# wuwuz/Pacmann

Hardware: AMD Instinct MI355X
Metric: private queries/sec + PIR-scan HBM GB/s, SIFT1M d=128 at 1/2/4/8 GPUs (higher is better)
Workload: dtype u64

## Files before the change

pacmann_amd/csrc/pm_ctx.cpp:

```cpp
#include "pm_host.h"

static thread_local std::string g_err;
namespace pmh {
int fail(int code, const std::string& msg) { g_err = msg; return code; }
}

extern "C" const char* pm_last_error(void) { return g_err.c_str(); }

static constexpr AesTables kAes{};
extern "C" int pm_expand_key(const uint8_t key[16], uint32_t rk[44]) {
  uint8_t w[176];
  memcpy(w, key, 16);
  uint8_t rcon = 1;
  for (int i = 16; i < 176; i += 4) {
    uint8_t t[4] = {w[i - 4], w[i - 3], w[i - 2], w[i - 1]};
    if (i % 16 == 0) {
      uint8_t u = t[0];
      t[0] = kAes.sbox[t[1]] ^ rcon; t[1] = kAes.sbox[t[2]]; t[2] = kAes.sbox[t[3]]; t[3] = kAes.sbox[u];
      rcon = AesTables::gmul(rcon, 2);
    }
    for (int k = 0; k < 4; ++k) w[i + k] = w[i - 16 + k] ^ t[k];
  }
  memcpy(rk, w, 176);
  return 0;
}


extern "C" int pm_ctx_create(int device, pm_ctx** out) {
  if (!out) return fail(PM_EINVAL, "out is NULL");
  int n = 0;
  HIPCHK(hipGetDeviceCount(&n));
  if (device < 0 || device >= n) return fail(PM_EINVAL, "no such HIP device " + std::to_string(device));
  HIPCHK(hipSetDevice(device));
  (void)hipSetDeviceFlags(hipDeviceScheduleSpin);
  (void)hipGetLastError();
  pm_ctx* c = new pm_ctx();
  c->device = device;
  const char* dbg = getenv("PM_DEBUG_SYNC");
  c->debug_sync = dbg && dbg[0] == '1';
  const char* nf = getenv("PM_NO_FUSE");
  c->no_fuse = nf && nf[0] == '1';
  const char* ns = getenv("PM_NO_SPLIT");
  c->no_split = ns && ns[0] == '1';
  const char* ls = getenv("PM_LOG_STEPS");
  c->log_steps = ls && ls[0] == '1';
  const char* dc = getenv("PM_DEBUG_CACHE");
  c->debug_cache = dc && dc[0] == '1';
  const char* vr = getenv("PM_VERIFY_ROWS");
  c->verify_rows = vr && vr[0] == '1';
  if (const char* rc = getenv("PM_ROWS_CHECK")) c->rows_check = atoi(rc);
  c->hash_mult.resize(pmk::step_max_e());
  for (size_t w = 0; w < c->hash_mult.size(); ++w) c->hash_mult[w] = row_hash_mult(w);
  if (const char* pw = getenv("PM_PUBLISH_WAIT")) c->publish_wait = pw[0] != '0';
  if (c->publish_wait) {
    for (auto& e : c->done_ring)
      if (hipEventCreateWithFlags(&e, hipEventDisableTiming | hipEventReleaseToSystem) != hipSuccess) {
        delete c;
        return fail(PM_EHIP, "hipEventCreateWithFlags(step completion) failed");
      }
    c->done_ev = c->done_ring[0];
  }
  if (const char* rs = getenv("PM_REPL_SIDE")) c->repl_side = rs[0] != '0';
  const char* ng = getenv("PM_NO_GUESS");
  c->no_guess = ng && ng[0] == '1';
  const char* sr = getenv("PM_STEP_SPEC");
  c->step_spec = sr && sr[0] == '1';
  hipError_t e = hipStreamCreateWithFlags(&c->stream, hipStreamNonBlocking);
  if (e != hipSuccess) { delete c; return fail(PM_EHIP, hipGetErrorString(e)); }
  *out = c;
  return 0;
}
extern "C" void pm_ctx_destroy(pm_ctx* c) { if (c) { (void)hipSetDevice(c->device); delete c; } }
extern "C" int pm_ctx_sync(pm_ctx* c) { HIPCHK(hipStreamSynchronize(c->stream)); HIPCHK(hipGetLastError()); return 0; }
extern "C" int pm_ctx_mem_info(pm_ctx* c, uint64_t* free_b, uint64_t* total_b) {
  if (!c) return fail(PM_EINVAL, "ctx is NULL");
  HIPCHK(hipSetDevice(c->device));
  size_t f = 0, t = 0;
  HIPCHK(hipMemGetInfo(&f, &t));
  if (free_b) *free_b = f;
  if (total_b) *total_b = t;
  return 0;
}
static std::mutex g_tl_mu;
static hipEvent_t g_tl_base = nullptr;
extern "C" int pm_timing_enable(pm_ctx* c, int on) {
  c->timing = on;
  if (on >= 2) {
    std::lock_guard<std::mutex> lk(g_tl_mu);
    if (!g_tl_base) {
      HIPCHK(hipEventCreate(&g_tl_base));
      HIPCHK(hipEventRecord(g_tl_base, c->stream));
    }
  }
  return 0;
}
extern "C" int pm_timing_timeline(pm_ctx* c, const char* path) {
  if (!c || !path) return fail(PM_EINVAL, "NULL argument");
  HIPCHK(hipStreamSynchronize(c->stream));
  std::lock_guard<std::mutex> lk(g_tl_mu);
  if (!g_tl_base) return fail(PM_EINVAL, "no timeline (kernel timing level 2 never enabled)");
  FILE* f = fopen(path, "a");
  if (!f) return fail(PM_EINVAL, std::string("cannot open ") + path);
  for (auto& t : c->launches) {
    float a = 0, b = 0;
    if (hipEventElapsedTime(&a, g_tl_base, t.a) != hipSuccess || hipEventElapsedTime(&b, g_tl_base, t.b) != hipSuccess)
      continue;
    fprintf(f, "%s,%.3f,%.3f,%p\n", t.name.c_str(), a * 1e3, b * 1e3, (void*)c);
  }
  fclose(f);
  return 0;
}
namespace pmh {
std::atomic<int> g_verify_records{0};
std::atomic<int> g_device_loop{-1};
std::atomic<int> g_rccl_timeout_s{-1};
std::atomic<int> g_fault_drl_query{-1};
}
extern "C" int pm_set_option(const char* name, int value) {
  if (!name) return fail(PM_EINVAL, "NULL argument");
  if (!strcmp(name, "verify_records")) { g_verify_records.store(value < 0 ? 0 : value); return 0; }
  if (!strcmp(name, "rccl_timeout_s")) { g_rccl_timeout_s.store(value); return 0; }
  if (!strcmp(name, "device_loop")) { g_device_loop.store(value < 0 ? -1 : value); return 0; }
  if (!strcmp(name, "fault_drl_query")) { g_fault_drl_query.store(value); return 0; }
  if (!strcmp(name, "stream_upload_only")) { g_stream_upload_only.store(value > 0 ? 1 : 0); return 0; }
  if (!strcmp(name, "aes_bs")) { pmk::set_aes_bs(value); return 0; }
  if (!strcmp(name, "fold_rot")) {
    if (value < -1 || value > 1) return fail(PM_EINVAL, "fold_rot takes 1, 0 or -1");
    pmk::set_fold_rot(value);
    return 0;
  }
  if (!strcmp(name, "fold_pack")) {
    if (value < -1 || value > 1) return fail(PM_EINVAL, "fold_pack takes 1, 0 or -1");
    pmk::set_fold_pack(value);
    return 0;
  }
  if (!strcmp(name, "answer_pack")) {
    if (value < -1 || value > 1) return fail(PM_EINVAL, "answer_pack takes 1, 0 or -1");
    pmk::set_answer_pack(value);
    return 0;
  }
  if (!strcmp(name, "step_help") && value != -2 && (value < 0 || value > 3))
    return fail(PM_EINVAL, "step_help takes 0..3 or -2");
  if (!strcmp(name, "step_help_spoil") && value != -2 && (value < 0 || value > 7))
    return fail(PM_EINVAL, "step_help_spoil takes a mask 0..7 or -2");
  if (pmk::set_option(name, value)) return fail(PM_EINVAL, std::string("unknown option ") + name);
  return 0;
}
extern "C" int pm_step_plan(const pm_step_shape* in, pm_step_forms* out) {
  if (!in || !out) return fail(PM_EINVAL, "NULL argument");
  if (in->kind > (uint32_t)pmk::STEP_DEVICE || in->nsub == 0 || in->np == 0) return fail(PM_EINVAL, "bad step shape");
  pmk::StepShape s{};
  s.np = in->np; s.nsub = in->nsub; s.np_live = in->np_live; s.max_per_part = in->max_per_part;
  s.maxPH = in->maxPH; s.maxSS = in->maxSS; s.E = in->E; s.ph8 = in->ph8 != 0;
  s.of_caller((int)in->kind, true);
  s.unfused = in->no_fuse != 0; s.no_split = in->no_split != 0; s.no_guess = in->no_guess != 0;
  const pmk::StepPlan p = pmk::step_plan(s, pmk::step_opts());
  static_assert(sizeof out->counter / sizeof out->counter[0] == pmk::STAGE_COUNT, "one slot per launch of a plan");
  *out = pm_step_forms{};
  for (int i = 0; i < pmk::STAGE_COUNT; ++i) {
    const pmk::StepLaunch& l = p.at[i];
    if (l.form < 0) continue;
    out->counter[i] = kHostTimerName[pm_ctx::step_counter(i, l.form)];
    out->grid_x[i] = l.gx; out->grid_y[i] = l.gy; out->block[i] = l.block;
  }
  out->nhelp = p.nhelp; out->nsplit = p.nsplit; out->qw = p.qw; out->np_live = p.np_live; out->cblk = p.cblk;
  out->no_guess = p.no_guess; out->qset = p.qset; out->args_valid = s.args_valid;
  return 0;
}
extern "C" int pm_fold_image_map(uint32_t cs, uint32_t ss, uint32_t E, uint32_t dim, int packed, uint64_t x0,
                                 uint64_t n, uint64_t* row, uint32_t* word, uint8_t* is_packed, uint64_t* nitems,
                                 uint32_t* npk_out) {
  if ((n && (!row || !word || !is_packed)) || !nitems || !npk_out) return fail(PM_EINVAL, "NULL argument");
  if ((cs != 512 && cs != 1024) || ss == 0 || ss % 4 || E < 4 || E % 2) return fail(PM_EINVAL, "not a fold image shape");
  const uint32_t npk = packed ? pmk::fold_pack_shape(E, dim) : 0;
  if (packed && (!npk || cs != 512)) return fail(PM_EINVAL, "these entries have no packed fold image");
  *nitems = pmk::fold_image_words(ss, E, cs, npk) / 2;
  *npk_out = npk;
  if (x0 > *nitems || n > *nitems - x0) return fail(PM_EINVAL, "items past the image");
  pmk::fold_image_map(cs, ss, npk, x0, n, row, word, is_packed);
  return 0;
}
extern "C" int pm_timing_reset(pm_ctx* c) {
  HIPCHK(hipStreamSynchronize(c->stream));
  for (auto& t : c->launches) { c->pool.push_back(t.a); c->pool.push_back(t.b); }
  c->launches.clear();
  for (int i = 0; i < HT_COUNT; ++i) { c->host_n[i] = 0; c->host_ms[i] = 0; }
  return 0;
}
extern "C" int pm_timing_get(pm_ctx* c, const char* name, uint64_t* launches, double* total_ms,
                             double* bytes) {
  HIPCHK(hipStreamSynchronize(c->stream));
  uint64_t n = 0; double ms = 0, by = 0;
  if (strncmp(name, "host_", 5) == 0) {
    for (int i = 0; i < HT_COUNT; ++i)
      if (strcmp(name, kHostTimerName[i]) == 0) { n = c->host_n[i]; ms = c->host_ms[i]; }
    if (launches) *launches = n;
    if (total_ms) *total_ms = ms;
    if (bytes) *bytes = 0;
    return 0;
  }
  for (auto& t : c->launches) {
    if (t.name != name) continue;
    float x = 0;
    HIPCHK(hipEventElapsedTime(&x, t.a, t.b));
    ++n; ms += x; by += t.bytes;
  }
  if (launches) *launches = n;
  if (total_ms) *total_ms = ms;
  if (bytes) *bytes = by;
  return 0;
}

#if defined(PM_STEP_STAMPS) || defined(PM_MR_STAMPS) || defined(PM_ANSWER_STAMPS)
namespace pmh {
int dump_stamps(hipStream_t st, const char* path, const void* hdr, size_t hdr_bytes, const DevBuf& buf, uint64_t count) {
  HIPCHK(hipStreamSynchronize(st));
  std::vector<uint64_t> t(count);
  HIPCHK(hipMemcpy(t.data(), buf.p, count * 8, hipMemcpyDeviceToHost));
  static std::mutex mu;
  std::lock_guard<std::mutex> lk(mu);
  if (FILE* f = fopen(path, "ab")) {
    fwrite(hdr, 1, hdr_bytes, f);
    fwrite(t.data(), 8, count, f);
    fclose(f);
  }
  return 0;
}
}
#endif

extern "C" int pm_prf_batch(pm_ctx* c, const uint32_t rk[44], const uint64_t* tags, const uint64_t* xs,
                            uint64_t n, uint64_t* out) {
  if (n == 0) return 0;
  DevBuf drk, dt, dx, dout;
  CHK(drk.reserve(176)); CHK(dt.reserve(n * 8)); CHK(dx.reserve(n * 8)); CHK(dout.reserve(n * 8));
  hipStream_t st = c->stream;
  HIPCHK(hipMemcpyAsync(drk.p, rk, 176, hipMemcpyHostToDevice, st));
  HIPCHK(hipMemcpyAsync(dt.p, tags, n * 8, hipMemcpyHostToDevice, st));
  HIPCHK(hipMemcpyAsync(dx.p, xs, n * 8, hipMemcpyHostToDevice, st));
  c->timed("prf", (double)n, [&] { pmk::prf_batch(st, drk.as<uint32_t>(), dt.as<uint64_t>(), dx.as<uint64_t>(), n, dout.as<uint64_t>()); });
  HIPCHK(hipGetLastError());
  HIPCHK(hipMemcpyAsync(out, dout.p, n * 8, hipMemcpyDeviceToHost, st));
  HIPCHK(hipStreamSynchronize(st));
  return 0;
}
extern "C" int pm_l2_batch(pm_ctx* c, const float* q, const float* rows, uint64_t nrows, uint64_t dim,
                           float* out) {
  if (nrows == 0) return 0;
  if (dim == 0) return fail(PM_EINVAL, "dim must be > 0");
  DevBuf dq, dr, dout;
  CHK(dq.reserve(dim * 4)); CHK(dr.reserve(nrows * dim * 4)); CHK(dout.reserve(nrows * 4));
  hipStream_t st = c->stream;
  HIPCHK(hipMemcpyAsync(dq.p, q, dim * 4, hipMemcpyHostToDevice, st));
  HIPCHK(hipMemcpyAsync(dr.p, rows, nrows * dim * 4, hipMemcpyHostToDevice, st));
  c->timed("l2_rows", (double)nrows * dim * 4, [&] {
    pmk::l2_rows(st, dr.as<float>(), dim, nrows, nullptr, dq.as<float>(), (uint32_t)dim, dout.as<float>());
  });
  HIPCHK(hipGetLastError());
  HIPCHK(hipMemcpyAsync(out, dout.p, nrows * 4, hipMemcpyDeviceToHost, st));
  HIPCHK(hipStreamSynchronize(st));
  return 0;
}
extern "C" int pm_ip_batch(pm_ctx* c, const uint32_t* q, const uint32_t* rows, uint64_t nrows, uint64_t dim,
                           uint32_t* per_row, uint32_t* sum) {
  if (dim == 0) return fail(PM_EINVAL, "dim must be > 0");
  DevBuf dq, dr, dpr, ds;
  CHK(dq.reserve(dim * 4)); CHK(dr.reserve(std::max<uint64_t>(1, nrows * dim * 4)));
  CHK(dpr.reserve(std::max<uint64_t>(4, nrows * 4))); CHK(ds.reserve(4));
  hipStream_t st = c->stream;
  HIPCHK(hipMemcpyAsync(dq.p, q, dim * 4, hipMemcpyHostToDevice, st));
  if (nrows) HIPCHK(hipMemcpyAsync(dr.p, rows, nrows * dim * 4, hipMemcpyHostToDevice, st));
  HIPCHK(hipMemsetAsync(ds.p, 0, 4, st));
  c->timed("ip_scan", (double)nrows * dim * 4, [&] {
    pmk::ip_rows(st, dr.as<uint32_t>(), nrows, dq.as<uint32_t>(), (uint32_t)dim, per_row ? dpr.as<uint32_t>() : nullptr,
                 ds.as<uint32_t>());
  });
  HIPCHK(hipGetLastError());
  if (per_row && nrows) HIPCHK(hipMemcpyAsync(per_row, dpr.p, nrows * 4, hipMemcpyDeviceToHost, st));
  uint32_t s = 0;
  HIPCHK(hipMemcpyAsync(&s, ds.p, 4, hipMemcpyDeviceToHost, st));
  HIPCHK(hipStreamSynchronize(st));
  if (sum) *sum = s;
  return 0;
}
extern "C" int pm_ip_bench(pm_ctx* c, uint64_t N, uint64_t D, uint32_t* sum, double* scan_ms) {
  return pm_ip_bench_shard(c, N, D, 0, N, sum, scan_ms);
}
extern "C" int pm_ip_bench_shard(pm_ctx* c, uint64_t Ntot, uint64_t D, uint64_t r0, uint64_t N, uint32_t* sum,
                                 double* scan_ms) {
  if (!c) return fail(PM_EINVAL, "NULL context");
  if (D == 0 || D % 4 || D > 4096) return fail(PM_EINVAL, "D must be a multiple of 4 and <= 4096");
  if (r0 > Ntot || N > Ntot - r0) return fail(PM_EINVAL, "shard rows past the fill's N");
  if (N == 0) {
    if (sum) *sum = 0;
    if (scan_ms) *scan_ms = 0.0;
    return 0;
  }
  DevBuf dv, dq, ds;
  CHK(dv.reserve(N * D * 4)); CHK(dq.reserve(D * 4)); CHK(ds.reserve(4));
  std::vector<uint32_t> q(D);
  for (uint64_t j = 0; j < D; ++j) q[j] = (uint32_t)j;
  hipStream_t st = c->stream;
  HIPCHK(hipMemcpyAsync(dq.p, q.data(), D * 4, hipMemcpyHostToDevice, st));
  HIPCHK(hipMemsetAsync(ds.p, 0, 4, st));
  pmk::ip_fill(st, dv.as<uint32_t>(), N, (uint32_t)D, r0);
  hipEvent_t a, b;
  HIPCHK(hipEventCreate(&a)); HIPCHK(hipEventCreate(&b));
  HIPCHK(hipEventRecord(a, st));
  c->timed("ip_scan", (double)N * D * 4, [&] { pmk::ip_rows(st, dv.as<uint32_t>(), N, dq.as<uint32_t>(), (uint32_t)D, nullptr, ds.as<uint32_t>()); });
  HIPCHK(hipEventRecord(b, st));
  HIPCHK(hipGetLastError());
  uint32_t s = 0;
  HIPCHK(hipMemcpyAsync(&s, ds.p, 4, hipMemcpyDeviceToHost, st));
  HIPCHK(hipStreamSynchronize(st));
  float ms = 0;
  HIPCHK(hipEventElapsedTime(&ms, a, b));
  (void)hipEventDestroy(a); (void)hipEventDestroy(b);
  if (sum) *sum = s;
  if (scan_ms) *scan_ms = ms;
  return 0;
}
```

pacmann_amd/csrc/pm_engine.cpp:

```cpp
#include "pm_engine.h"

static void derive_key(uint64_t seed, uint64_t part, uint64_t epoch, uint8_t key[16]) {
  uint64_t r1 = hash4(seed, DOM_KEY, part, epoch, 0), r2 = hash4(seed, DOM_KEY, part, epoch, 1);
  memcpy(key, &r1, 8);
  memcpy(key + 8, &r2, 8);
}

static void part_params(PartHost& ph, uint64_t N, uint64_t F) {
  uint64_t target = (uint64_t)(2 * std::sqrt((double)N));
  uint64_t cs = 1;
  while (cs < target) cs *= 2;
  uint64_t ss = (uint64_t)std::ceil((double)N / (double)cs);
  ss = (ss + 3) / 4 * 4;
  const uint64_t thr = 8;
  uint64_t maxq = (uint64_t)(std::sqrt((double)N) * std::log((double)N));
  uint64_t k = (uint64_t)std::ceil(std::log(2.0) * (double)(F + 1));
  uint64_t phn = (k * cs + thr - 1) / thr * thr;
  uint64_t qpc = 3 * (uint64_t)((double)maxq / (double)ss);
  qpc = (qpc + thr - 1) / thr * thr;
  ph.d.N = N;
  ph.d.CS = (uint32_t)cs;
  uint32_t lg = 0; while ((1ull << lg) < cs) ++lg;
  ph.d.log2CS = lg;
  ph.d.SS = (uint32_t)ss;
  ph.d.PH = (uint32_t)phn;
  ph.d.Qpc = (uint32_t)qpc;
  ph.d.H = (uint32_t)(phn + ss * qpc);
  ph.maxq64 = maxq;
  ph.d.MaxQ = (uint32_t)std::min<uint64_t>(maxq, 0xffffffffu);
}

static double part_storage(const PartHost& p, uint64_t Ebytes) {
  double s = 0;
  s = s + (double)p.d.PH * 8;
  s = s + (double)p.d.PH * (double)Ebytes;
  s = s + (double)p.d.PH * 8;
  double tb = (double)p.d.SS * (double)p.d.Qpc;
  s = s + tb * 8;
  s = s + tb * (double)Ebytes;
  s = s + tb * 8;
  s = s + tb * (double)Ebytes;
  return s;
}
static double part_comm(const PartHost& p, uint64_t E) { return (double)((uint64_t)p.d.SS * 4 + E * 8); }

namespace pmh {
int engine_create(pm_ctx* ctx, Engine* g, uint64_t N, uint64_t Ebytes, uint64_t B,
                         const uint64_t* rawDB, uint64_t F, uint64_t seed, bool batch,
                         uint32_t shard, uint32_t nshards, const Engine* server,
                         const DbGen* gen, uint32_t coord_words, bool remote) {
  if (nshards == 0 || shard >= nshards) return fail(PM_EINVAL, "shard must be < nshards");
  if (!ctx) return fail(PM_EINVAL, "ctx is NULL");
  if (!rawDB && N && !server && !gen && !remote) return fail(PM_EINVAL, "rawDB is NULL");
  if (gen && gen->kind == 1 && (uint64_t)(gen->dim + gen->m) * 4 != Ebytes)
    return fail(PM_EINVAL, "graph entry size must be 4 * (dim + m)");
  if (server && server->ctx->device != ctx->device) return fail(PM_EINVAL, "a client shares the server DB of its own device only");
  if (N == 0) return fail(PM_EINVAL, "DBSize must be > 0");
  if (Ebytes < 8) return fail(PM_EINVAL, "DBEntryByteNum must be >= 8");
  HIPCHK(hipSetDevice(ctx->device));
  g->ctx = ctx; g->is_batch = batch;
  g->N = N; g->Ebytes = Ebytes; g->E = Ebytes / 8; g->F = F; g->seed = seed;
  g->remote = remote;
  if (batch) {
    g->B = B;
    g->P = B / 2;
    if (g->P == 0) return fail(PM_EINVAL, "BatchSize must be >= 2");
    g->PS = (N + g->P - 1) / g->P;
    if (g->PS > 1 && g->PS < (1ull << 32)) g->ps_magic = ~0ull / g->PS + 1;
  } else {
    g->P = 1; g->PS = N;
  }
  g->parts.resize(g->P);
  if (g->E > pmk::step_max_e()) return fail(PM_EINVAL, "DBEntrySize above the step kernel's LDS limit");
  g->shard = shard; g->nshards = nshards;
  uint64_t off_tag = 0, off_pp = 0, off_par = 0, off_ridx = 0, off_rval = 0, off_hist = 0, off_ar = 0,
           off_tab = 0, off_tabT = 0, off_cur = 0, off_db = 0;
  for (uint64_t i = 0; i < g->P; ++i) {
    PartHost& ph = g->parts[i];
    uint64_t start = i * g->PS, end = std::min((i + 1) * g->PS, N);
    if (end <= start) return fail(PM_EINVAL, "empty partition (DBSize too small for BatchSize)");
    part_params(ph, end - start, F);
    ph.owned = i % nshards == shard;
    if (!ph.owned) {
      ph.d.seed = seed; ph.d.idx = i;
      continue;
    }
    g->owned_list.push_back((uint32_t)i);
    if (ph.d.CS > 32768) return fail(PM_EINVAL, "ChunkSize > 32768 unsupported (16-bit prep offsets)");
    if (ph.d.SS > pmk::step_max_ss()) return fail(PM_EINVAL, "SetSize above the step kernel's LDS limit");
    if ((uint64_t)ph.d.H >= (1ull << 29)) return fail(PM_EINVAL, "tag space >= 2^29 (util.go:161)");
    ph.d.row0 = off_db; off_db += end - start;
    ph.d.seed = seed; ph.d.idx = i;
    g->maxH = std::max(g->maxH, ph.d.H);
    g->maxCS = std::max(g->maxCS, ph.d.CS);
    g->minCS = std::min(g->minCS, ph.d.CS);
    g->maxPH = std::max(g->maxPH, ph.d.PH);
    g->ph8 = g->ph8 && ph.d.PH % 8 == 0;
    g->maxSS = std::max(g->maxSS, ph.d.SS);
    g->maxRepl = std::max(g->maxRepl, ph.d.SS * ph.d.Qpc);
    ph.d.tag = (uint32_t*)(uintptr_t)off_tag; off_tag += ph.d.H;
    ph.d.pp = (uint32_t*)(uintptr_t)off_pp; off_pp += ph.d.PH;
    ph.d.parity = (uint64_t*)(uintptr_t)off_par; off_par += (uint64_t)ph.d.H * g->E;
    ph.d.ridx = (uint32_t*)(uintptr_t)off_ridx; off_ridx += (uint64_t)ph.d.SS * ph.d.Qpc;
    ph.d.rval = (uint64_t*)(uintptr_t)off_rval; off_rval += (uint64_t)ph.d.SS * ph.d.Qpc * g->E;
    ph.d.hist = (uint32_t*)(uintptr_t)off_hist; off_hist += ph.d.SS;
    ph.d.arena = (uint64_t*)(uintptr_t)off_ar; off_ar += (uint64_t)ph.d.MaxQ * g->E;
    ph.d.tab = (uint16_t*)(uintptr_t)off_tab; off_tab += (uint64_t)ph.d.H * ph.d.SS;
    ph.d.curk = cur_k(ph.d.PH, ph.d.SS);
    ph.d.cur = (uint16_t*)(uintptr_t)off_cur; off_cur += cur_words(ph.d.PH, ph.d.SS, ph.d.curk);
    ph.d.tabT = (uint16_t*)(uintptr_t)off_tabT; off_tabT += tabT_words(ph.d.H, ph.d.SS);
    ph.cache.reserve(ph.d.MaxQ);
  }
  CHK(g->zero16.reserve(64));
  HIPCHK(hipMemset(g->zero16.p, 0, 64));
  if (server) g->db = server->db;
  else if (!remote) CHK(g->db->reserve(std::max<uint64_t>(8, off_db * g->E * 8)));
  for (uint32_t i : server || remote ? std::vector<uint32_t>{} : g->owned_list) {
    const uint64_t start = (uint64_t)i * g->PS, rows = g->parts[i].d.N;
    uint64_t* dst = g->db->as<uint64_t>() + g->parts[i].d.row0 * g->E;
    if (gen && gen->kind == 0)
      pmk::db_synth(ctx->stream, dst, start, rows, (uint32_t)g->E, gen->seed);
    else if (gen)
      pmk::graph_synth(ctx->stream, dst, start, rows, N, gen->dim, gen->m, gen->seed);
    else
      HIPCHK(hipMemcpy(dst, rawDB + start * g->E, rows * g->E * 8, hipMemcpyHostToDevice));
  }
  if (gen) {
    HIPCHK(hipGetLastError());
    HIPCHK(hipStreamSynchronize(ctx->stream));
  }
  uint64_t off_img = 0;
  const bool fold_img = !remote && !g->owned_list.empty() && pmk::fold_image_ok(g->minCS, g->maxCS, (uint32_t)g->E);
  const uint32_t want_npk = !server && fold_img ? pmk::fold_pack_slices(g->minCS, g->maxCS, (uint32_t)g->E, coord_words) : 0;
  const uint32_t want_apk = !server && !remote && !g->owned_list.empty() ? pmk::answer_pack_segs((uint32_t)g->E, coord_words) : 0;
  bool low_zero = false;
  if (want_npk || want_apk) {
    DevBuf flag;
    CHK(flag.reserve(64));
    low_zero = pmk::coord_low_zero(ctx->stream, g->db->as<uint64_t>(), off_db, (uint32_t)g->E, coord_words, flag.as<uint32_t>());
    HIPCHK(hipGetLastError());
  }
  if (fold_img) {
    if (server) g->img_npk = server->img_npk;
    else if (low_zero) g->img_npk = want_npk;
    for (uint32_t i : g->owned_list) {
      PmPart& d = g->parts[i].d;
      d.img = (const uint64_t*)(uintptr_t)off_img;
      off_img += pmk::fold_image_words(d.SS, (uint32_t)g->E, (uint32_t)g->maxCS, g->img_npk);
    }
    size_t free_b = 0, total_b = 0;
    if (!server && hipMemGetInfo(&free_b, &total_b) == hipSuccess && off_img * 8 > free_b / 4) {
      for (uint32_t i : g->owned_list) g->parts[i].d.img = nullptr;
      off_img = 0;
    } else if (server && !server->img->p) {
      for (uint32_t i : g->owned_list) g->parts[i].d.img = nullptr;
      off_img = 0;
    }
    if (!off_img) g->img_npk = 0;
  }
  if (off_img) {
    if (server) {
      g->img = server->img;
    } else {
      CHK(g->img->reserve(off_img * 8));
      for (uint32_t i : g->owned_list) {
        const PmPart& d = g->parts[i].d;
        pmk::fold_image(ctx->stream, g->img->as<uint64_t>() + (uintptr_t)d.img, g->db->as<uint64_t>() + d.row0 * g->E,
                        d.N, d.SS, (uint32_t)g->E, (uint32_t)g->maxCS, g->img_npk);
      }
      HIPCHK(hipGetLastError());
      HIPCHK(hipStreamSynchronize(ctx->stream));
    }
  }
  if (server) {
    g->apk = server->apk; g->apk_nseg = server->apk_nseg; g->apk_cseg = server->apk_cseg;
  } else if (want_apk && low_zero) {
    const uint64_t bytes = off_db * want_apk * 16;
    size_t free_b = 0, total_b = 0;
    if (hipMemGetInfo(&free_b, &total_b) != hipSuccess || bytes <= free_b / 4) {
      CHK(g->apk->reserve(bytes));
      pmk::answer_pack_image(ctx->stream, g->apk->as<uint64_t>(), g->db->as<uint64_t>(), off_db, (uint32_t)g->E, coord_words);
      HIPCHK(hipGetLastError());
      HIPCHK(hipStreamSynchronize(ctx->stream));
      g->apk_nseg = want_apk; g->apk_cseg = coord_words / 8;
    }
  }
  CHK(g->tag.reserve(off_tag * 4));
  CHK(g->pp.reserve(off_pp * 4));
  CHK(g->parity.reserve(off_par * 8));
  CHK(g->ridx.reserve(off_ridx * 4));
  CHK(g->rval.reserve(off_rval * 8));
  CHK(g->hist.reserve(off_hist * 4));
  CHK(g->fqn.reserve(g->P * 4));
  CHK(g->arena.reserve(std::max<uint64_t>(8, off_ar * 8)));
  const bool need_tab = !remote && pmk::fold_needs_tab(g->minCS, g->maxCS, (uint32_t)g->E, off_img != 0);
  if (need_tab) CHK(g->tab.reserve(off_tab * 2));
  CHK(g->tabT.reserve(off_tabT * 2));
  CHK(g->cur.reserve(std::max<uint64_t>(2, off_cur * 2)));
  CHK(g->done.reserve(4 * (3 + 16 * 4096)));
  {
    const uint32_t init[3] = {1u << 31, 0, 0};
    HIPCHK(hipMemcpy(g->done.p, init, sizeof init, hipMemcpyHostToDevice));
  }
  {
    g->gran_words = (g->maxPH + 63) / 64;
    const size_t n = (size_t)kArgSubs * (8 + 64 + 2 * g->gran_words + 8) * 8;
    CHK(g->gran.reserve(n));
    HIPCHK(hipMemset(g->gran.p, 0, n));
    CHK(g->err_h.reserve(64));
    memset(g->err_h.p, 0, 64);
  }
  CHK(g->parts_d.reserve(g->P * sizeof(PmPart)));
  CHK(g->owned_d.reserve(std::max<size_t>(1, g->owned_list.size()) * sizeof(PmPart)));
  CHK(g->parts_stage.reserve((g->P + g->owned_list.size()) * sizeof(PmPart)));
  for (uint64_t i = 0; i < g->P; ++i) {
    PmPart& d = g->parts[i].d;
    if (!g->parts[i].owned) continue;
    d.tag = g->tag.as<uint32_t>() + (uintptr_t)d.tag;
    d.pp = g->pp.as<uint32_t>() + (uintptr_t)d.pp;
    d.parity = g->parity.as<uint64_t>() + (uintptr_t)d.parity;
    d.ridx = g->ridx.as<uint32_t>() + (uintptr_t)d.ridx;
    d.rval = g->rval.as<uint64_t>() + (uintptr_t)d.rval;
    d.hist = g->hist.as<uint32_t>() + (uintptr_t)d.hist;
    d.fqn = g->fqn.as<uint32_t>() + i;
    d.arena = g->arena.as<uint64_t>() + (uintptr_t)d.arena;
    d.tabT = g->tabT.as<uint16_t>() + (uintptr_t)d.tabT;
    d.tab = need_tab ? g->tab.as<uint16_t>() + (uintptr_t)d.tab : nullptr;
    d.cur = g->cur.as<uint16_t>() + (uintptr_t)d.cur;
    d.img = off_img ? g->img->as<uint64_t>() + (uintptr_t)d.img : nullptr;
  }
  HIPCHK(hipMemsetAsync(g->fqn.p, 0, g->P * 4, ctx->stream));
  HIPCHK(hipMemsetAsync(g->hist.p, 0, off_hist * 4, ctx->stream));
  HIPCHK(hipStreamSynchronize(ctx->stream));
  return 0;
}
}

static int upload_parts(Engine* g) {
  std::vector<PmPart> v(g->P), w;
  for (uint64_t i = 0; i < g->P; ++i) v[i] = g->parts[i].d;
  for (uint32_t i : g->owned_list) w.push_back(g->parts[i].d);
  HIPCHK(hipMemcpyAsync(g->parts_d.p, v.data(), g->P * sizeof(PmPart), hipMemcpyHostToDevice,
                        g->ctx->stream));
  if (!w.empty())
    HIPCHK(hipMemcpyAsync(g->owned_d.p, w.data(), w.size() * sizeof(PmPart), hipMemcpyHostToDevice,
                          g->ctx->stream));
  HIPCHK(hipStreamSynchronize(g->ctx->stream));
  return 0;
}

static int upload_parts_async(Engine* g, hipStream_t st) {
  if (g->ctx->stream != st && hipStreamQuery(g->ctx->stream) != hipSuccess) {
    if (!g->order_ev) HIPCHK(hipEventCreateWithFlags(&g->order_ev, hipEventDisableTiming));
    HIPCHK(hipEventRecord(g->order_ev, g->ctx->stream));
    HIPCHK(hipStreamWaitEvent(st, g->order_ev, 0));
  }
  const size_t no = g->owned_list.size();
  if (g->stage_ev) HIPCHK(hipEventSynchronize(g->stage_ev));
  else HIPCHK(hipEventCreateWithFlags(&g->stage_ev, hipEventDisableTiming));
  CHK(g->parts_stage.reserve((g->P + no) * sizeof(PmPart)));
  PmPart* h = g->parts_stage.as<PmPart>();
  for (uint64_t i = 0; i < g->P; ++i) h[i] = g->parts[i].d;
  for (size_t i = 0; i < no; ++i) h[g->P + i] = g->parts[g->owned_list[i]].d;
  HIPCHK(hipMemcpyAsync(g->parts_d.p, h, g->P * sizeof(PmPart), hipMemcpyHostToDevice, st));
  if (no) HIPCHK(hipMemcpyAsync(g->owned_d.p, h + g->P, no * sizeof(PmPart), hipMemcpyHostToDevice, st));
  HIPCHK(hipEventRecord(g->stage_ev, st));
  return 0;
}

namespace pmh {
int ensure_host_cache(Engine* g) {
  if (!g->cache_on_dev) return 0;
  const uint64_t cap = (uint64_t)g->dcache_cmask + 1;
  std::vector<uint64_t> t(g->P * cap);
  HIPCHK(hipSetDevice(g->ctx->device));
  HIPCHK(hipMemcpy(t.data(), g->dcache.p, t.size() * 8, hipMemcpyDeviceToHost));
  for (uint64_t p = 0; p < g->P; ++p) {
    FlatMap& c = g->parts[p].cache;
    c.clear();
    for (uint64_t i = 0; i < cap; ++i)
      if (const uint64_t e = t[p * cap + i]) c.put((uint32_t)e - 1u, (uint32_t)(e >> 32));
  }
  g->cache_on_dev = false;
  g->dcache_valid = false;
  return 0;
}

int engine_prep_host(Engine* g, uint64_t p0, uint64_t p1, std::vector<uint64_t>& todo,
                            hipStream_t st) {
  if (p1 - p0 > 1 && !(p0 == 0 && p1 == g->P)) return fail(PM_EINVAL, "engine_prep: unsupported range");
  const bool all = p0 == 0 && p1 == g->P;
  if (g->cache_on_dev && !all) CHK(ensure_host_cache(g));
  if (all) { g->cache_on_dev = false; g->dcache_valid = false; }
  todo.clear();
  for (uint64_t i = p0; i < p1; ++i)
    if (g->parts[i].owned) todo.push_back(i);
  if (todo.empty()) return 0;
  for (uint64_t i : todo) {
    PartHost& ph = g->parts[i];
    uint8_t key[16];
    derive_key(g->seed, i, ph.epoch_ctr, key);
    ph.d.epoch = ph.epoch_ctr++;
    pm_expand_key(key, ph.d.rk);
    ph.fqn = 0;
    ph.cache.clear();
    ph.shadow.clear();
  }
  CHK(st ? upload_parts_async(g, st) : upload_parts(g));
  g->prep_gen++;
  return 0;
}
int engine_prep_launch(pm_ctx* c, const Engine* g, const PmPart* dp, int np, const PmPart* host_parts,
                              uint32_t clients, bool sync) {
  hipStream_t st = c->stream;
  c->timed("prep_init", 0, [&] { pmk::prep_init(st, dp, np, g->maxH, g->maxRepl, (uint32_t)g->E, g->skipPrep); });
  double aes = 0, fold = 0, repl = 0;
  uint32_t minH = ~0u;
  for (int i = 0; i < np; ++i) {
    const PmPart& d = host_parts[i];
    minH = std::min(minH, d.H);
    aes += (double)d.H * d.SS;
    fold += ((double)d.PH + (double)(d.SS - 1) * d.Qpc) * d.SS * (double)g->E * 8;
    repl += (double)d.SS * d.Qpc * g->E * 8 * 2;
  }
  const bool side = !g->skipPrep && c->repl_side && !c->timing && !c->debug_sync;
  std::unique_lock<std::mutex> side_lk(c->side_mu, std::defer_lock);
  if (side) {
    side_lk.lock();
    if (!c->side) {
      HIPCHK(hipStreamCreateWithFlags(&c->side, hipStreamNonBlocking));
      for (auto& e : c->side_ev) HIPCHK(hipEventCreateWithFlags(&e, hipEventDisableTiming));
    }
    HIPCHK(hipEventRecord(c->side_ev[0], st));
    HIPCHK(hipStreamWaitEvent(c->side, c->side_ev[0], 0));
    pmk::prep_repl(c->side, dp, np, g->maxRepl, g->db->as<uint64_t>(), (uint32_t)g->E);
    HIPCHK(hipEventRecord(c->side_ev[1], c->side));
  }
  c->timed("prep_offsets", aes, [&] { pmk::prep_offsets(st, dp, np, g->maxH, g->maxSS); });
  if (g->skipPrep) {
    for (int i = 0; i < np; ++i) {
      const PmPart& d = host_parts[i];
      HIPCHK(hipMemsetAsync(d.parity, 0, (uint64_t)d.H * g->E * 8, st));
      HIPCHK(hipMemsetAsync(d.rval, 0, (uint64_t)d.SS * d.Qpc * g->E * 8, st));
    }
  } else {
    int kind = pmk::FOLD_GATHER;
    c->timed("prep_fold", fold, [&] { kind = pmk::prep_fold(st, dp, np, g->maxH, g->db->as<uint64_t>(), (uint32_t)g->E, g->minCS,
                                                      g->maxCS, g->zero16.as<uint64_t>(), clients, g->img->p != nullptr, minH,
                                                      g->img_npk); });
    if (kind == pmk::FOLD_ROT512 || kind == pmk::FOLD_ROT512P || kind == pmk::FOLD_ROT1024) {
      c->host_add(kind == pmk::FOLD_ROT512 ? HT_FOLD_ROT512 : kind == pmk::FOLD_ROT512P ? HT_FOLD_ROT512P : HT_FOLD_ROT1024, 0.0);
    } else {
      c->host_add(HT_FOLD_OTHER, 0.0);
      c->host_add(kind == pmk::FOLD_PIPE ? HT_FOLD_PIPE : kind == pmk::FOLD_BLK ? HT_FOLD_BLK : HT_FOLD_GATHER, 0.0);
    }
    if (side) HIPCHK(hipStreamWaitEvent(st, c->side_ev[1], 0));
    else c->timed("prep_repl", repl, [&] { pmk::prep_repl(st, dp, np, g->maxRepl, g->db->as<uint64_t>(), (uint32_t)g->E); });
  }
  HIPCHK(hipGetLastError());
  if (sync) HIPCHK(hipStreamSynchronize(st));
  return 0;
}
}
static int engine_prep(Engine* g, uint64_t p0, uint64_t p1) {
  std::vector<uint64_t> todo;
  CHK(engine_prep_host(g, p0, p1, todo));
  if (todo.empty()) return 0;
  const PmPart* dp = p1 - p0 == 1 ? g->parts_d.as<PmPart>() + p0 : g->owned_d.as<PmPart>();
  std::vector<PmPart> hp;
  for (uint64_t i : todo) hp.push_back(g->parts[i].d);
  return engine_prep_launch(g->ctx, g, dp, (int)todo.size(), hp.data());
}


namespace pmh {
int wait_done(pm_ctx* sc, uint64_t seq) {
  if (sc->done_seen.load(std::memory_order_acquire) >= seq) return 0;
  auto t0 = Clock::now();
  for (uint64_t spin = 0;; ++spin) {
    if (sc->done_seen.load(std::memory_order_acquire) >= seq) return 0;
    if (sc->done_mu.try_lock()) {
      std::lock_guard<std::mutex> lk(sc->done_mu, std::adopt_lock);
      if (sc->done_seen.load(std::memory_order_acquire) >= seq) return 0;
      const uint64_t rec = seq;
      if (sc->done_rec.load(std::memory_order_acquire) < seq)
        return fail(PM_EHIP, "step completion: waited for a step that was not recorded");
      for (uint64_t k = 0;; ++k) {
        const hipError_t e = hipEventQuery(sc->done_ring[seq % pm_ctx::kDoneRing]);
        if (e == hipSuccess) break;
        if (e != hipErrorNotReady) return fail(PM_EHIP, std::string("step completion: ") + hipGetErrorString(e));
        if ((k & 0xfff) == 0xfff && ms_since(t0) > 5000.0) {
          HIPCHK(hipStreamSynchronize(sc->stream));
          HIPCHK(hipGetLastError());
          break;
        }
      }
      uint64_t prev = sc->done_seen.load(std::memory_order_relaxed);
      while (prev < rec && !sc->done_seen.compare_exchange_weak(prev, rec, std::memory_order_release)) {}
      return 0;
    }
    if ((spin & 0xffff) == 0xffff && ms_since(t0) > 10000.0) return fail(PM_EHIP, "step completion wait timed out");
  }
}

int poll_done(pm_ctx* sc, uint64_t seq, bool* ready) {
  *ready = !(sc->publish_wait && sc->done_ev && seq) || sc->done_seen.load(std::memory_order_acquire) >= seq;
  if (*ready || !sc->done_mu.try_lock()) return 0;
  std::lock_guard<std::mutex> lk(sc->done_mu, std::adopt_lock);
  if (sc->done_seen.load(std::memory_order_acquire) >= seq) { *ready = true; return 0; }
  if (sc->done_rec.load(std::memory_order_acquire) < seq)
    return fail(PM_EHIP, "step completion: polled a step that was not recorded");
  const hipError_t e = hipEventQuery(sc->done_ring[seq % pm_ctx::kDoneRing]);
  if (e == hipErrorNotReady) return 0;
  if (e != hipSuccess) return fail(PM_EHIP, std::string("step completion: ") + hipGetErrorString(e));
  uint64_t prev = sc->done_seen.load(std::memory_order_relaxed);
  while (prev < seq && !sc->done_seen.compare_exchange_weak(prev, seq, std::memory_order_release)) {}
  *ready = true;
  return 0;
}

int wait_step(pm_ctx* c, const PmOutHdr* hdr, uint32_t nsub, uint32_t token, const char* rows,
                     size_t row_bytes, size_t pf_off, size_t pf_len, uint64_t seq, pm_ctx* sc) {
  if (!sc) sc = c;
  hipStream_t stream = sc->stream;
  const bool ordered = sc->publish_wait && sc->done_ev && seq;
  const size_t w0 = pf_off / 8, w1 = (pf_off + pf_len + 7) / 8;
  auto row_hash = [&](uint32_t s) {
    const volatile uint64_t* rw = (const volatile uint64_t*)(rows + s * row_bytes);
    uint64_t x = token * kCsumMix;
    for (size_t w = w0; w < w1; ++w) x += rw[w] * c->hash_mult[w];
    return x;
  };
  if (c->debug_sync) {
    HIPCHK(hipStreamSynchronize(stream));
  } else if (ordered && !c->timing) {
    for (uint32_t s = 0; s < nsub; ++s) {
      __builtin_prefetch(&hdr[s]);
      if (c->rows_check)
        for (size_t w = w0; w < w1; w += 8) __builtin_prefetch(rows + s * row_bytes + w * 8);
    }
    CHK(wait_done(sc, seq));
    std::atomic_thread_fence(std::memory_order_acquire);
  } else {
    const volatile uint32_t* tok = &hdr[0].token;
    const size_t stride = sizeof(PmOutHdr) / sizeof(uint32_t);
    for (uint32_t s = 0; s < nsub; ++s) {
      __builtin_prefetch(&hdr[s]);
      if (c->rows_check)
        for (size_t w = w0; w < w1; w += 8) __builtin_prefetch(rows + s * row_bytes + w * 8);
    }
    auto t0 = Clock::now();
    uint32_t s = 0;
    bool first_look = true;
    for (uint64_t spin = 0; s < nsub; ++spin) {
      if (tok[s * stride] == token) {
        if (c->timing && s == 0 && first_look) c->host_add(HT_WAIT_FIRST, ms_since(t0));
        std::atomic_thread_fence(std::memory_order_acquire);
        if (c->rows_check) {
          const bool match = row_hash(s) == *(const volatile uint64_t*)&hdr[s].csum;
          if (first_look) {
            c->host_add(HT_ROWS_SEEN, 0);
            if (!match) c->host_add(HT_ROWS_TORN, 0);
          }
          if (!match && !ordered) {
            first_look = false;
            if (c->rows_check == 1)
              return fail(PM_EHIP, "step result row " + std::to_string(s) + " does not match its header checksum");
            if ((spin & 0xffff) == 0xffff && ms_since(t0) > 5000.0)
              return fail(PM_EHIP, "step results incomplete (sub-query " + std::to_string(s) + ")");
            continue;
          }
        }
        if (c->timing && s + 1 == nsub) c->host_add(HT_WAIT_ALL, ms_since(t0));
        ++s;
        first_look = true;
        continue;
      }
      if ((spin & 0xffff) == 0xffff && ms_since(t0) > 5000.0) {
        HIPCHK(hipStreamSynchronize(stream));
        HIPCHK(hipGetLastError());
        break;
      }
    }
    if (ordered) {
      auto td = Clock::now();
      CHK(wait_done(sc, seq));
      if (c->timing) c->host_add(HT_WAIT_DONE, ms_since(td));
    }
    std::atomic_thread_fence(std::memory_order_acquire);
  }
  for (uint32_t s = 0; s < nsub; ++s)
    if (hdr[s].token != token) return fail(PM_EHIP, "step results not published (sub-query " + std::to_string(s) + ")");
  if (ordered && c->rows_check)
    for (uint32_t s = 0; s < nsub; ++s)
      if (row_hash(s) != hdr[s].csum)
        return fail(PM_EHIP, "step result row " + std::to_string(s) + " does not match its header after completion");
  return 0;
}
}

static int wait_and_post(Engine* g, const PmStep& S, uint32_t nsub, Clock::time_point) {
  pm_ctx* c = g->ctx;
  const uint64_t E = g->E;
  auto t_wait = Clock::now();
  CHK(wait_step(c, S.hdr_h, nsub, S.token, (const char*)S.rows_h, E * 8, (size_t)S.pf_w0 * 8,
                (size_t)(S.pf_w1 - S.pf_w0) * 8, g->step_seq));
  c->host_add(HT_STEP_WAIT, ms_since(t_wait));

  if (c->verify_rows) {
    std::vector<uint64_t> seen((const uint64_t*)S.rows_h, (const uint64_t*)S.rows_h + (uint64_t)nsub * E);
    std::vector<PmOutHdr> hseen(S.hdr_h, S.hdr_h + nsub);
    HIPCHK(hipStreamSynchronize(c->stream));
    for (uint32_t s = 0; s < nsub; ++s) {
      const bool rd = memcmp(seen.data() + (uint64_t)s * E, (const uint64_t*)S.rows_h + (uint64_t)s * E, E * 8) != 0;
      const bool hd = memcmp(&hseen[s], &S.hdr_h[s], sizeof(PmOutHdr)) != 0;
      if (rd || hd)
        fprintf(stderr, "[pm] verify: token %u sub %u status %u: %s%s changed after the token was seen\n", S.token, s,
                S.hdr_h[s].status, rd ? "row " : "", hd ? "header " : "");
    }
  }
  auto t_post = Clock::now();
  post_results(g, S.hdr_h, S.rows_h, nsub, 0, S.token);
  c->host_add(HT_STEP_POST, ms_since(t_post));
  return 0;
}

namespace pmh {
void post_results(Engine* g, PmOutHdr* hdr, uint64_t* rows, uint32_t nsub, uint32_t base,
                         uint32_t token) {
  pm_ctx* c = g->ctx;
  const uint64_t E = g->E;
  g->hdr = hdr + base;
  g->rows = rows + (uint64_t)base * E;
  PmStep S{};
  S.token = token;
  if (c->log_steps) {
    for (uint32_t s = 0; s < nsub; ++s)
      fprintf(stderr, "[pm] step %p tok %u s %u part %u kind %u idx %lu -> st %u ref %u row0 %016lx\n", (void*)g,
              S.token, s, g->subs[s].part, g->subs[s].kind, (unsigned long)g->subs[s].idx, g->hdr[s].status,
              g->hdr[s].ref, (unsigned long)g->rows[(uint64_t)s * E]);
  }
  if (c->debug_cache) {
    for (uint32_t s = 0; s < nsub; ++s) {
      const PmOutHdr& h = g->hdr[s];
      PartHost& ph = g->parts[g->subs[s].part];
      const uint64_t* row = g->rows + (uint64_t)s * E;
      if (h.status == ST_OK) ph.shadow[h.ref].assign(row, row + E);
      if (h.status == ST_CACHED) {
        auto it = ph.shadow.find(h.ref);
        if (it == ph.shadow.end() || memcmp(it->second.data(), row, E * 8) != 0) {
          (void)hipStreamSynchronize(c->stream);
          std::vector<uint64_t> dev(E);
          (void)hipMemcpy(dev.data(), ph.d.arena + (uint64_t)h.ref * E, E * 8, hipMemcpyDeviceToHost);
          const bool dev_ok = it != ph.shadow.end() && memcmp(it->second.data(), dev.data(), E * 8) == 0;
          fprintf(stderr, "[pm] cache: token %u sub %u part %u idx %lu slot %u: row differs from the slot's answer%s; "
                  "device arena now %s the slot's answer; row[0] %016lx shadow[0] %016lx arena[0] %016lx\n",
                  S.token, s, g->subs[s].part, (unsigned long)g->subs[s].idx, h.ref,
                  it == ph.shadow.end() ? " (no answer recorded)" : "", dev_ok ? "equals" : "differs from",
                  (unsigned long)row[0], (unsigned long)(it == ph.shadow.end() ? 0 : it->second[0]), (unsigned long)dev[0]);
        }
      }
    }
  }
  for (uint32_t s = 0; s < nsub; ++s) {
    const PmOutHdr& h = g->hdr[s];
    if (h.status == ST_OK) {
      PartHost& ph = g->parts[g->subs[s].part];
      ph.fqn++;
      ph.cache.put(g->subs[s].idx, h.ref);
    } else if (h.status == ST_DUP) {
      const uint32_t r = h.ref - base;
      memcpy(g->rows + (uint64_t)s * E, g->rows + (uint64_t)r * E, E * 8);
      g->hdr[s].dist = g->hdr[r].dist;
    }
  }
#ifdef PM_STAMPS
  {
    std::vector<uint64_t> t(64);
    (void)hipMemcpy(t.data(), g->buf.stamps.p, 64 * 8, hipMemcpyDeviceToHost);
    g->stamp_sum.resize(64, 0.0);
    for (int i = 1; i < 64; ++i)
    {
      const uint64_t base = i >= 48 ? t[48] : i >= 41 ? t[41] : t[0];
      if (t[i] && base && i != 41 && i != 48) g->stamp_sum[i] += (double)(t[i] - base);
    }
    g->stamp_n++;
  }
#endif
}

#if defined(PM_STEP_STAMPS) || defined(PM_MR_STAMPS) || defined(PM_ANSWER_STAMPS)
struct LaunchStamps {
  const char* file = nullptr;
  uint64_t words = 0;
  int begin(const char* f, std::atomic<int>* first, hipStream_t st, StepBufs& B, PmStep& S, uint64_t n) {
    if (!f || (first && first->fetch_add(1) >= 40)) return 0;
    CHK(B.stamps.reserve(n * 8));
    HIPCHK(hipMemsetAsync(B.stamps.p, 0, n * 8, st));
    S.stamps = B.stamps.as<uint64_t>();
    file = f; words = n;
    return 0;
  }
  int end(hipStream_t st, const StepBufs& B, PmStep& S, const void* hdr, size_t hdr_bytes) {
    if (!file) return 0;
    S.stamps = nullptr;
    return dump_stamps(st, file, hdr, hdr_bytes, B.stamps, words);
  }
};
#endif

int step_chain(pm_ctx* c, StepBufs& B, PmStep& S, const pmk::StepShape& shape, uint32_t nreal, double ans_bytes,
               const std::function<int()>& after_resolve) {
  hipStream_t st = c->stream;
  if (shape.desc_shared != (S.subs == S.subs_h && S.sb == S.sb_h))
    return fail(PM_EINVAL, "step_chain: the descriptor is not where the step's shape says");
  const pmk::StepPlan plan = pmk::step_plan(shape, pmk::step_opts());
  S.args_valid = shape.args_valid ? 1u : 0u;
  S.nsplit = plan.nsplit; S.qw = plan.qw; S.np_live = plan.np_live; S.cblk = plan.cblk; S.nhelp = plan.nhelp; S.no_guess = plan.no_guess;
  S.help_spoil = plan.help_spoil;
  const uint32_t nsub = S.nsub;
  if (plan.qset) {
    CHK(B.qset.reserve((uint64_t)nsub * plan.qw * 2));
    S.qset = B.qset.as<uint16_t>();
  }
  if (plan.nsplit > 1) {
    CHK(B.part_x.reserve((uint64_t)nsub * plan.nsplit * (S.E & ~3u) * 8));
    S.part_x = B.part_x.as<uint64_t>();
  }
  const bool fused = plan.at[pmk::STAGE_FUSED].form >= 0;
  if (fused) {
    if (plan.nhelp && !B.helpg.p) {
      const size_t nh = (size_t)kArgSubs * kStepHelpMax * kHelpGran * 8;
      CHK(B.helpg.reserve(nh));
      HIPCHK(hipMemsetAsync(B.helpg.p, 0, nh, st));
    }
    S.helpg = B.helpg.as<uint64_t>();
  }
  B.spec_nsub = 0;
  if (fused && c->step_spec) {
    CHK(B.specrec.reserve(kArgSubs * 4));
    HIPCHK(hipMemsetAsync(B.specrec.p, 0, kArgSubs * 4, st));
    S.specrec = B.specrec.as<uint32_t>();
    B.spec_nsub = nsub;
  }
  auto run = [&](int stage, const char* name, double bytes) {
    const int form = plan.at[stage].form;
    if (form < 0) return;
    c->timed_ext(name, bytes, [&](pmk::PmEvents ev) { pmk::step_launch(st, S, plan, stage, ev); }, 2);
    c->host_add(pm_ctx::step_counter(stage, form), stage == pmk::STAGE_FUSED ? plan.nhelp : 0.0);
    if (pmk::step_answer_packed(S, plan, stage)) c->host_add(HT_ANSWER_PACKED, 0.0);
  };
#ifdef PM_STEP_STAMPS
  LaunchStamps ss;
  const uint32_t sh[4] = {plan.at[pmk::STAGE_FUSED].gx, nsub, pmk::step_match_blocks(shape.maxPH), S.np};
// ... 800 lines not shown
```

pacmann_amd/csrc/pm_engine.h:

```cpp
#pragma once
#include "pm_host.h"

#include <functional>

struct DbGen;
struct Engine;
struct pm_graph;
struct StepGroup;
struct StepBufs;
struct ShardComb;

namespace pmh {
int engine_create(pm_ctx* ctx, Engine* g, uint64_t N, uint64_t Ebytes, uint64_t B,
                  const uint64_t* rawDB, uint64_t F, uint64_t seed, bool batch,
                  uint32_t shard = 0, uint32_t nshards = 1, const Engine* server = nullptr,
                  const DbGen* gen = nullptr, uint32_t coord_words = 0, bool remote = false);
int ensure_host_cache(Engine* g);
int engine_prep_host(Engine* g, uint64_t p0, uint64_t p1, std::vector<uint64_t>& todo,
                     hipStream_t st = nullptr);
int engine_prep_launch(pm_ctx* c, const Engine* g, const PmPart* dp, int np, const PmPart* host_parts,
                       uint32_t clients = 1, bool sync = true);
int wait_done(pm_ctx* sc, uint64_t seq);
int poll_done(pm_ctx* sc, uint64_t seq, bool* ready);
int wait_step(pm_ctx* c, const PmOutHdr* hdr, uint32_t nsub, uint32_t token, const char* rows,
              size_t row_bytes, size_t pf_off, size_t pf_len, uint64_t seq, pm_ctx* sc = nullptr);
void post_results(Engine* g, PmOutHdr* hdr, uint64_t* rows, uint32_t nsub, uint32_t base,
                  uint32_t token);
constexpr int kChainStop = 1 << 30;
int step_chain(pm_ctx* c, StepBufs& B, PmStep& S, const pmk::StepShape& shape, uint32_t nreal, double ans_bytes,
               const std::function<int()>& after_resolve = {});
int engine_step(Engine* g, const float* q_dev, uint32_t dim);
int client_guard(const Engine* g);
int db_guard(const Engine* g);
void print_stamps(const Engine& e);
void record_stats(Engine* g, double t);
int batch_prep(Engine* g);
int batch_query(Engine* g, const uint64_t* idx, uint64_t n, uint64_t* out, const float* q_dev,
                uint32_t dim, float* dist_out, const uint64_t** rows_out = nullptr,
                uint8_t* ok = nullptr);
int bq_prepare(Engine* g, const uint64_t* idx, uint64_t n, bool* fast);
void bq_emit_fast(Engine* g, const uint64_t* idx, uint64_t n, uint64_t* out, float* dist_out,
                  const uint64_t** rows_out, uint8_t* ok);
int bq_tail(Engine* g, uint64_t n);
int batch_query_impl(Engine* g, const uint64_t* idx, uint64_t n, uint64_t* out, const float* q_dev,
                     uint32_t dim, float* dist_out, const uint64_t** rows_out, uint8_t* ok);
int check_session(const pm_graph* g);
int graph_start_set(pm_graph* g);
int gvi_pre(pm_graph* g, bool with_q, bool* fast);
int gvi_post(pm_graph* g, bool with_q, bool fast);
void knn_reset(pm_graph* g);
void knn_begin_finish(pm_graph* g, int parallel, int benchmarking, const float* sdh = nullptr);
void knn_batch(pm_graph* g, int parallel, int benchmarking);
void knn_update(pm_graph* g, int step);
void knn_end(pm_graph* g, int k, int64_t* ids_out, int64_t* steps_out);
int group_step_launch(StepGroup& G, PmStep& S, int kind, uint32_t max_per_part, uint32_t nreal, double ans_bytes);
int prep_clients(pm_ctx* c, DevBuf& pbuf, const std::vector<uint32_t>& lp, const std::vector<Engine*>& who,
                 const std::vector<double*>* mt, HostBuf* stage = nullptr, hipEvent_t* stage_ev = nullptr);
int team_init(StepGroup& G, pm_graph** gs, uint32_t S);
void team_release(pm_graph** gs, uint32_t S);
int run_batched_team(pm_graph** gs, uint32_t S, const float* queries, uint64_t q, int k, int step,
                     int parallel, uint32_t T, int64_t* answers, double* mt_out, ShardComb* comb = nullptr,
                     uint32_t team = 0);
hipStream_t team_stream(int dev, uint32_t t);
int run_batched_pool(pm_graph** gs, uint32_t S, const float* queries, uint64_t q, int k, int step, int parallel,
                     uint32_t NG, uint32_t T, int64_t* answers, double* mt_out);
int check_loop_sessions(pm_graph** gs, uint32_t S, bool sharded);
using TeamFn = std::function<int(uint32_t g, uint32_t s0, uint32_t s1, uint32_t Tg)>;
int run_teams(pm_graph** gs, uint32_t S, uint32_t NG, uint32_t TT, const TeamFn& fn);
}

struct FlatMap {
  struct Slot { uint64_t key; uint32_t val, gen; };
  std::vector<Slot> slot;
  uint32_t cur = 1, count = 0, mask = 0;
  explicit FlatMap(uint32_t cap_pow2 = 256) { rehash(cap_pow2); }
  static uint64_t mix(uint64_t x) { x ^= x >> 33; x *= 0xff51afd7ed558ccdULL; x ^= x >> 33; return x; }
  void rehash(uint32_t cap) {
    std::vector<Slot> s0;
    s0.swap(slot);
    slot.assign(cap, Slot{0, 0, 0});
    mask = cap - 1; count = 0;
    const uint32_t old = cur; cur = 1;
    for (const Slot& x : s0) if (x.gen == old) put(x.key, x.val);
  }
  void clear() { if (++cur == 0) { for (Slot& x : slot) x.gen = 0; cur = 1; } count = 0; }
  void reserve(uint32_t n) { uint32_t c = (uint32_t)slot.size(); while (c < 2 * n) c *= 2; if (c != slot.size()) rehash(c); }
  void prefetch(uint64_t k) const { __builtin_prefetch(&slot[(uint32_t)mix(k) & mask]); }
  uint32_t* find(uint64_t k) {
    for (uint32_t i = (uint32_t)mix(k) & mask;; i = (i + 1) & mask) {
      Slot& x = slot[i];
      if (x.gen != cur) return nullptr;
      if (x.key == k) return &x.val;
    }
  }
  void put(uint64_t k, uint32_t v) {
    if (2 * (count + 1) > slot.size()) rehash((uint32_t)slot.size() * 2);
    for (uint32_t i = (uint32_t)mix(k) & mask;; i = (i + 1) & mask) {
      Slot& x = slot[i];
      if (x.gen != cur) { x.gen = cur; x.key = k; x.val = v; ++count; return; }
      if (x.key == k) { x.val = v; return; }
    }
  }
  bool emplace(uint64_t k, uint32_t v) {
    if (find(k)) return false;
    put(k, v);
    return true;
  }
  template <class F> void for_each(F&& f) const {
    for (const Slot& x : slot) if (x.gen == cur) f(x.key, x.val);
  }
};

struct StepBufs {
  DevBuf subs_d, sb_d, bits, cand, meta, spec, res_d, ans, part_x, stamps;
  DevBuf qset;
  DevBuf helpg;
  DevBuf specrec;
  uint32_t spec_nsub = 0;
  HostBuf desc_h, out_h;
  int reserve(uint32_t nsub, uint32_t np, uint32_t words, uint32_t cblk, uint64_t E) {
    CHK(subs_d.reserve(nsub * sizeof(PmSub)));
    CHK(sb_d.reserve((np + 1) * 4));
    CHK(bits.reserve((uint64_t)nsub * words * 8));
    CHK(cand.reserve((uint64_t)nsub * cblk * 6 * 4));
    CHK(meta.reserve((uint64_t)nsub * 2 * 4));
    CHK(spec.reserve((uint64_t)nsub * 64 * 4));
    CHK(res_d.reserve(nsub * sizeof(PmRes)));
    CHK(ans.reserve((uint64_t)nsub * E * 8));
    return 0;
  }
  void fill(PmStep& S, uint32_t words, uint32_t cblk) const {
    S.subs = subs_d.as<PmSub>();
    S.sb = sb_d.as<uint32_t>();
    S.bits = bits.as<uint64_t>();
    S.cand = cand.as<uint32_t>();
    S.meta = meta.as<uint32_t>();
    S.spec = spec.as<uint32_t>();
    S.res = res_d.as<PmRes>();
    S.ans = ans.as<uint64_t>();
    S.words = words;
    S.cblk = cblk;
  }
};
static inline size_t step_out_bytes(uint32_t nsub, uint64_t E) { return nsub * sizeof(PmOutHdr) + (size_t)nsub * E * 8; }
static inline void step_out(PmStep& S, void* out, uint32_t nsub) {
  S.hdr_h = (PmOutHdr*)out;
  S.rows_h = (uint64_t*)((char*)out + nsub * sizeof(PmOutHdr));
}
static inline uint32_t next_token(uint32_t& token) {
  if (++token == 0) ++token;
  return token;
}
static inline void step_read_window(PmStep& S, size_t pf_off, size_t pf_len, uint64_t E) {
  const size_t off = std::min<size_t>(pf_off, E * 8);
  const size_t end = std::min<size_t>(E * 8, off + std::min<size_t>(pf_len, E * 8));
  S.pf_w0 = (uint32_t)(off / 8);
  S.pf_w1 = (uint32_t)((end + 7) / 8);
}
static inline uint32_t host_rows_partial(const pm_ctx* c, bool partial) {
  return partial && !c->verify_rows && !c->debug_cache ? 1u : 0u;
}
struct PartHost {
  PmPart d{};
  bool owned = true;
  uint64_t epoch_ctr = 0, fqn = 0, dummy_ctr = 0;
  uint64_t maxq64 = 0;
  FlatMap cache;
  std::unordered_map<uint64_t, std::vector<uint64_t>> shadow;
};

struct Engine {
  pm_ctx* ctx = nullptr;
  static uint64_t next_uid() { static std::atomic<uint64_t> n{0}; return ++n; }
  const uint64_t uid = next_uid();
  bool is_batch = false;
  uint64_t N = 0, E = 0, Ebytes = 0, F = 0, seed = 0;
  uint64_t B = 0, P = 1, PS = 0;
  uint64_t ps_magic = 0;
  uint64_t part_of(uint64_t id) const {
    return ps_magic && id < (1ull << 32) ? (uint64_t)(((unsigned __int128)id * ps_magic) >> 64) : id / PS;
  }
  uint32_t shard = 0, nshards = 1;
  bool skipPrep = false;
  uint64_t FBN = 0, QMIP = 0, Support = 0, prepCount = 0;
  double prepTime = 0, storage = 0, commOn = 0, commOff = 0;

  std::shared_ptr<DevBuf> db = std::make_shared<DevBuf>();
  std::shared_ptr<DevBuf> img = std::make_shared<DevBuf>();
  uint32_t img_npk = 0;
  std::shared_ptr<DevBuf> apk = std::make_shared<DevBuf>();
  uint32_t apk_nseg = 0, apk_cseg = 0;
  void step_db(PmStep& S) const {
    S.db = db->as<uint64_t>();
    S.dbp = apk_nseg ? apk->as<uint64_t>() : nullptr;
    S.pk_nseg = apk_nseg; S.pk_cseg = apk_cseg;
  }
  DevBuf zero16, parts_d, owned_d, tag, pp, parity, ridx, rval, hist, fqn, arena, tab, tabT, cur, done, gran;
  HostBuf parts_stage;
  hipEvent_t stage_ev = nullptr;
  hipEvent_t order_ev = nullptr;
  uint32_t gran_words = 0;
  std::vector<uint32_t> owned_list;
  DevBuf qoffs, ans_srv;
  DevBuf srv_parts;
  bool srv_parts_up = false;
  struct SplitQuery {
    bool open = false;
    PmStep S{};
    uint64_t nq = 0;
    std::vector<uint64_t> ids;
    std::vector<uint32_t> map;
    DevBuf sets_d, ans_d, map_d;
    HostBuf sets_h;
  } split;
  bool remote = false, prepared = false, prep_due = false;
  struct PrepStream {
    bool open = false;
    std::vector<std::vector<char>> got;
    uint64_t missing = 0;
    HostBuf stage[2];
    DevBuf win[2];
    hipEvent_t ev[2] = {};
    bool busy[2] = {};
    uint64_t slot_bytes = 0;
    uint32_t next = 0;
    std::chrono::steady_clock::time_point t0;
  } pstream;
  StepBufs buf;
  std::vector<double> stamp_sum;
  uint64_t stamp_n = 0;
  uint32_t step_token = 0;
  uint64_t step_seq = 0;
  size_t pf_off = 0, pf_len = ~size_t(0);
  bool rows_partial = false;
  HostBuf err_h, src_h;
  HostBuf stage_h;
  hipEvent_t dev_ev = nullptr;
  ~Engine() {
    if (dev_ev) (void)hipEventDestroy(dev_ev);
    if (stage_ev) (void)hipEventDestroy(stage_ev);
    if (order_ev) (void)hipEventDestroy(order_ev);
    for (hipEvent_t e : pstream.ev) if (e) (void)hipEventDestroy(e);
  }
  std::vector<PartHost> parts;
  uint32_t maxH = 0, maxPH = 0, maxSS = 0, maxRepl = 0, maxCS = 0, minCS = ~0u;
  bool ph8 = true;

  std::vector<PmSub> subs;
  std::vector<uint32_t> sb;
  std::vector<uint64_t> sub_gid;
  PmOutHdr* hdr = nullptr;
  uint64_t* rows = nullptr;
  std::vector<std::vector<uint64_t>> pq;
  FlatMap resp_map;
  std::vector<uint64_t> resp_rows;
  std::vector<float> resp_dist;
  std::vector<uint8_t> resp_ok;
  std::vector<char> slow;
  uint64_t qn = 0;
  uint64_t prep_gen = 0;
  std::vector<uint64_t> zero_row;
  DevBuf dcache;
  uint32_t dcache_cmask = 0;
  bool cache_on_dev = false, dcache_valid = false;
};

static inline double answer_bytes(const PmPart& d, uint64_t E) {
  const double rows = std::min((double)d.SS, (double)d.N / (double)d.CS);
  return rows * (double)E * 8 + 4.0 * d.SS + 8.0 * E;
}

struct DbGen { int kind; uint64_t seed; uint32_t dim, m; };

struct pm_batchpir { Engine e; ~pm_batchpir() { print_stamps(e); } };

struct SplitMix {
  uint64_t s;
  uint64_t next() { s += 0x9e3779b97f4a7c15ULL; uint64_t z = s;
    z = (z ^ (z >> 30)) * 0xbf58476d1ce4e5b9ULL; z = (z ^ (z >> 27)) * 0x94d049bb133111ebULL;
    return z ^ (z >> 31); }
  uint64_t intn(uint64_t n) { return next() % n; }
};
struct VD { float dist; int64_t id; };

struct pm_graph {
  pm_ctx* ctx = nullptr;
  uint64_t n = 0, dim = 0, m = 0;
  bool nonprivate = false, skipPrep = false;
  uint64_t pir_seed = 0;
  SplitMix rng{0};
  std::shared_ptr<const std::vector<float>> vec_own;
  std::shared_ptr<const std::vector<uint32_t>> graph_own;
  const float* vectors = nullptr;
  const uint32_t* graph = nullptr;
  std::shared_ptr<DevBuf> dvec = std::make_shared<DevBuf>();
  std::shared_ptr<DevBuf> dgraph = std::make_shared<DevBuf>();
  uint32_t shard = 0, nshards = 1;
  bool synth = false;
  uint64_t data_seed = 0;
  DevBuf dstartvec;
  std::vector<uint8_t> okv;
  const uint32_t* true_nb(uint64_t id, uint32_t* tmp) const {
    if (!synth) return graph + id * m;
    const uint64_t kg = sm64(data_seed + DOM_SYNTH_NB);
    for (uint32_t k = 0; k < m; ++k) tmp[k] = graph_synth_nb(kg, n, id, (uint32_t)m, k);
    return tmp;
  }
  pm_batchpir* server = nullptr;
  DevBuf dq, dids, ddist;
  float* q_shared = nullptr;
  float* qdev() { return q_shared ? q_shared : dq.as<float>(); }
  HostBuf stage_h;
  pm_batchpir* pir = nullptr;
  std::vector<uint64_t> start;
  DevBuf dstart;
  uint64_t total = 0, succ = 0;
  std::vector<int64_t> batch;
  std::vector<uint64_t> qids;
  std::vector<const uint64_t*> rowp;
  std::vector<float> dist, start_d;
  std::vector<uint32_t> nb;
  FlatMap known;
  std::vector<uint32_t> known_nb;
  std::vector<float> known_dist;
  std::vector<int64_t> known_id, known_reach;
  std::vector<VD> heap, all;
  std::vector<std::pair<VD, uint32_t>> fs;
  Clock::time_point t_init;
  DevBuf kb_q, kb_ids, kb_steps, kb_flags;
  int graph_ids_ok = -1;
  std::string lost;
  ~pm_graph() { delete pir; }
};

struct ShardComb;
struct StepGroup {
  pm_ctx* c = nullptr;
  uint32_t S = 0, P = 0, maxPH = 0, maxSS = 0, E = 0, dim = 0;
  std::vector<uint32_t> lp;
  uint32_t Pl = 0;
  bool ph8 = false;
  StepBufs buf;
  DevBuf parts_d, done, prep_parts, desc_d;
  uint32_t token = 0, pf_w0 = 0, pf_w1 = 0;
  uint64_t seq = 0;
  std::vector<PmSub> subs;
  std::vector<uint32_t> sb, base;
  uint32_t nsub = 0;
  struct alignas(64) SessStage {
    uint64_t step = ~0ull;
    uint32_t n = 0, nreal = 0, maxpp = 0, live = 0;
    double bytes = 0;
    bool ok = false;
    std::vector<uint32_t> pc;
  };
  bool stage_on = false;
  uint32_t stride = 0;
  uint64_t nstep = 0;
  HostBuf stage_h;
  std::vector<SessStage> stg;
  std::vector<uint64_t> gen;
  std::vector<Engine*> es;
  std::vector<const float*> qv;
  bool rows_partial = false;
  uint32_t ns = 0;
  DevBuf qbuf, start_ids, start_dist, start_vec;
  HostBuf qstage;
  ShardComb* comb = nullptr;
  uint32_t team = 0;
  uint64_t round = 0;
  std::vector<pm_graph*> gs;
  uint32_t npos = 0, W = 0, w0 = 0, nb_off = 0;
  DevBuf out_d, map_d, ids_d, rec_own;
  uint64_t* rec_d = nullptr;
  std::atomic<bool> peer_failed{false};
  uint32_t verify_every = 0;
  bool combine_dead = false;
  DevBuf st_d;
  HostBuf map_h, ids_h, slow_h, rec_h;
  std::vector<char> slow;
};

struct StreamSwap {
  pm_ctx* c = nullptr;
  hipStream_t old = nullptr;
  void swap_in(pm_ctx* ctx, hipStream_t st) {
    if (!st) return;
    c = ctx; old = ctx->stream;
    (void)hipStreamSynchronize(old);
    ctx->stream = st;
  }
  ~StreamSwap() {
    if (!c) return;
    (void)hipStreamSynchronize(c->stream);
    c->stream = old;
  }
};
```

pacmann_amd/csrc/pm_host.h:

```cpp
#define PM_HOST_TU 1
#pragma once
#include "pm_internal.h"
#include "pm_aes.h"
#include "../../include/pacmann.h"

#include <dlfcn.h>
#include <hip/hip_runtime.h>
#include <rccl/rccl.h>

#include <algorithm>
#include <atomic>
#include <cstdio>
#include <cstdlib>
#include <chrono>
#include <condition_variable>
#include <cmath>
#include <cstring>
#include <memory>
#include <string>
#include <mutex>
#include <thread>
#include <unordered_map>
#include <vector>

using namespace pm;

struct DevBuf;

namespace pmh {
int fail(int code, const std::string& msg);
extern std::atomic<int> g_verify_records;
extern std::atomic<int> g_device_loop;
extern std::atomic<int> g_rccl_timeout_s;
extern std::atomic<int> g_fault_drl_query;
extern std::atomic<int> g_stream_upload_only;
int dump_stamps(hipStream_t st, const char* path, const void* hdr, size_t hdr_bytes, const DevBuf& buf, uint64_t count);
}
using namespace pmh;

#define HIPCHK(x)                                                                         \
  do {                                                                                    \
    hipError_t e_ = (x);                                                                  \
    if (e_ != hipSuccess)                                                                 \
      return fail(PM_EHIP, std::string(#x) + ": " + hipGetErrorString(e_));               \
  } while (0)
#define CHK(x)            \
  do {                    \
    int r_ = (x);         \
    if (r_ != 0) return r_; \
  } while (0)

struct DevBuf {
  void* p = nullptr;
  size_t n = 0;
  ~DevBuf() { if (p) (void)hipFree(p); }
  int reserve(size_t bytes) {
    if (bytes <= n) return 0;
    if (p) { (void)hipFree(p); p = nullptr; n = 0; }
    if (bytes == 0) return 0;
    hipError_t e = hipMalloc(&p, bytes);
    if (e != hipSuccess) return fail(PM_ENOMEM, "hipMalloc(" + std::to_string(bytes) + "): " + hipGetErrorString(e));
    n = bytes;
    return 0;
  }
  template <class T> T* as() const { return (T*)p; }
};
struct HostBuf {
  void* p = nullptr;
  size_t n = 0;
  ~HostBuf() { if (p) (void)hipHostFree(p); }
  int reserve(size_t bytes) {
    if (bytes <= n) return 0;
    if (p) { (void)hipHostFree(p); p = nullptr; n = 0; }
    hipError_t e = hipHostMalloc(&p, bytes, hipHostMallocCoherent | hipHostMallocMapped);
    if (e != hipSuccess) return fail(PM_ENOMEM, std::string("hipHostMalloc: ") + hipGetErrorString(e));
    memset(p, 0, bytes);
    n = bytes;
    return 0;
  }
  template <class T> T* as() const { return (T*)p; }
};

enum HostTimer : int { HT_STEP_LAUNCH, HT_STEP_WAIT, HT_STEP_POST, HT_BATCH_QUERY, HT_GVI_PARSE, HT_SEARCH_KNN, HT_KNN_INIT, HT_KNN_BATCH, HT_KNN_UPDATE, HT_KNN_FINAL, HT_WAIT_FIRST, HT_WAIT_ALL, HT_ROWS_SEEN, HT_ROWS_TORN, HT_WAIT_DONE, HT_COMBINE, HT_COMBINE_TURN, HT_PATH_MATCH, HT_PATH_MATCH_PART, HT_PATH_MATCH_PART8, HT_PREP_SETS, HT_REC_VERIFIED, HT_REC_BAD, HT_REC_DROPPED, HT_REC_FAILED, HT_REC_PEER, HT_REC_UNEXPLAINED, HT_FOLD_ROT512, HT_FOLD_ROT1024, HT_FOLD_OTHER, HT_FOLD_PIPE, HT_FOLD_BLK, HT_FOLD_GATHER, HT_FOLD_ROT512P, HT_DEV_STEPS, HT_DEV_QUERIES, HT_KNN_BATCH_FALLBACK, HT_PATH_STEP, HT_PATH_RESOLVE_LDS, HT_PATH_RESOLVE_G, HT_PATH_MR_S2, HT_PATH_MR_S4, HT_PATH_MR_GENERAL, HT_PATH_GATHER, HT_PATH_ANSWER_P5, HT_PATH_ANSWER_P, HT_PATH_ANSWER_S, HT_PATH_ANSWER_G, HT_ANSWER_PACKED, HT_GVI_GROUP, HT_GVI_GROUP_STEPS, HT_SERVER_ANSWER_PACKED, HT_CLIENT_BEGIN, HT_CLIENT_FINISH, HT_PREP_STREAM, HT_PREP_STREAM_WINDOWS, HT_COUNT };
static const char* const kHostTimerName[HT_COUNT] = {"host_step_launch", "host_step_wait", "host_step_post", "host_batch_query", "host_gvi_parse", "host_search_knn", "host_knn_init", "host_knn_batch", "host_knn_update", "host_knn_final", "host_wait_first_token", "host_wait_all_tokens", "host_rows_seen", "host_rows_torn", "host_wait_done", "host_combine", "host_combine_turn", "host_path_match", "host_path_match_part", "host_path_match_part8", "host_prep_sets", "host_records_verified", "host_records_bad", "host_records_dropped", "host_records_failed", "host_records_peer", "host_records_unexplained", "host_fold_rot512", "host_fold_rot1024", "host_fold_other", "host_fold_pipe", "host_fold_blk", "host_fold_gather", "host_fold_rot512p", "host_dev_steps", "host_dev_queries", "host_knn_batch_fallback", "host_path_step", "host_path_resolve_lds", "host_path_resolve_g", "host_path_mr_s2", "host_path_mr_s4", "host_path_mr_general", "host_path_gather", "host_path_answer_p5", "host_path_answer_p", "host_path_answer_s", "host_path_answer_g", "host_answer_packed", "host_gvi_group", "host_gvi_group_steps", "host_server_answer_packed", "host_client_begin", "host_client_finish", "host_prep_stream", "host_prep_stream_windows"};
static_assert(HT_PATH_ANSWER_G - HT_PATH_STEP + 1 == pmk::FORM_COUNT, "one counter per step form, in the order of pmk::FORM_*");

struct TimedLaunch { std::string name; hipEvent_t a, b; double bytes; };

struct pm_ctx {
  int device = 0;
  hipStream_t stream = nullptr;
  int timing = 0;
  bool sample_now = true;
  uint64_t sample_ctr = 0;
  bool no_fuse = false;
  bool no_split = false;
  bool no_guess = false;
  bool step_spec = false;
  bool verify_rows = false;
  bool debug_cache = false;
  bool log_steps = false;
  bool debug_sync = false;
  bool repl_side = true;
  hipStream_t side = nullptr;
  hipEvent_t side_ev[2] = {};
  std::mutex side_mu;
  int rows_check = 2;
  std::vector<uint64_t> hash_mult;
  bool publish_wait = true;
  static constexpr uint32_t kDoneRing = 64;
  hipEvent_t done_ev = nullptr;
  hipEvent_t done_ring[kDoneRing] = {};
  std::atomic<uint64_t> done_rec{0}, done_seen{0};
  std::mutex done_mu, rec_mu;
  uint64_t record_done(hipStream_t st) {
    if (!publish_wait) return 0;
    std::lock_guard<std::mutex> lk(rec_mu);
    const uint64_t seq = done_rec.load(std::memory_order_relaxed) + 1;
    (void)hipEventRecord(done_ring[seq % kDoneRing], st);
    done_rec.store(seq, std::memory_order_release);
    return seq;
  }
  std::string last_kernel;
  uint64_t host_n[HT_COUNT] = {};
  double host_ms[HT_COUNT] = {};
  void host_add(HostTimer t, double ms) { host_n[t]++; host_ms[t] += ms; }
  static HostTimer step_counter(int stage, int form) {
    if (stage != pmk::STAGE_MATCH) return (HostTimer)(HT_PATH_STEP + form);
    return form == pmk::MATCH_PART8 ? HT_PATH_MATCH_PART8 : form == pmk::MATCH_PART ? HT_PATH_MATCH_PART : HT_PATH_MATCH;
  }
  std::vector<TimedLaunch> launches;
  std::vector<hipEvent_t> pool;
  hipEvent_t ev() {
    if (!pool.empty()) { hipEvent_t e = pool.back(); pool.pop_back(); return e; }
    hipEvent_t e; (void)hipEventCreate(&e); return e;
  }
  template <class F> void timed(const char* name, double bytes, F&& f, int level = 1) {
    last_kernel = name;
    if (debug_sync) {
      f();
      hipError_t e = hipStreamSynchronize(stream);
      if (e != hipSuccess) fprintf(stderr, "[pm] kernel %s failed: %s\n", name, hipGetErrorString(e));
      return;
    }
    if (timing < level) { f(); return; }
    TimedLaunch t{name, ev(), ev(), bytes};
    (void)hipEventRecord(t.a, stream);
    f();
    (void)hipEventRecord(t.b, stream);
    launches.push_back(t);
  }
  template <class F> void timed_ext(const char* name, double bytes, F&& f, int level) {
    last_kernel = name;
    if (debug_sync) { timed(name, bytes, [&] { f(pmk::PmEvents{}); }, level); return; }
    if (timing < level || (timing == 3 && level == 2 && !sample_now)) { f(pmk::PmEvents{}); return; }
    TimedLaunch t{name, ev(), ev(), bytes};
    f(pmk::PmEvents{t.a, t.b});
    launches.push_back(t);
  }
  ~pm_ctx() {
    for (auto& t : launches) { (void)hipEventDestroy(t.a); (void)hipEventDestroy(t.b); }
    for (auto e : pool) (void)hipEventDestroy(e);
    for (auto e : done_ring) if (e) (void)hipEventDestroy(e);
    for (auto e : side_ev) if (e) (void)hipEventDestroy(e);
    if (side) (void)hipStreamDestroy(side);
    if (stream) (void)hipStreamDestroy(stream);
  }
};
struct KnnDev {
  DevBuf x, xb, xl, xn, mx;
  uint32_t dp = 0;
};
struct KnnOut {
  DevBuf cand, out, dist, len, tau, list, nlist, pref, eps;
  bool stages = false;
  uint64_t nl = 0;
};
extern const char* const kWideDimText;
bool wide_dim_ok(uint64_t dim);
int knn_upload(pm_ctx* c, const float* v, uint64_t n, uint32_t dim, KnnDev& d, bool exact, bool wide = false,
               hipMemcpyKind kind = hipMemcpyHostToDevice);
int knn_device(pm_ctx* c, const KnnDev& B, uint64_t n, const KnnDev& Q, uint64_t nq, uint32_t dim, uint32_t K,
               bool self_base, bool want_dist, bool exact, KnnOut& o, uint64_t* fallback,
               uint32_t top = pmk::knn_top());

using Clock = std::chrono::steady_clock;
static inline double ms_since(Clock::time_point t) {
  return std::chrono::duration<double, std::milli>(Clock::now() - t).count();
}
```

pacmann_amd/csrc/pm_internal.h:

```cpp
#pragma once
#include <hip/hip_runtime.h>
#include <stdint.h>

#include <string>

#if defined(__HIP_DEVICE_COMPILE__) && !defined(PM_HOST_TU)
#define PM_G __attribute__((address_space(1)))
#else
#define PM_G
#endif

namespace pm {

constexpr uint32_t kDefaultProgramPoint = 0x7fffffffu;
constexpr uint64_t kDefaultValue = 0xdeadbeefULL;
constexpr uint16_t kSkip = 0xffffu;
constexpr int kBlock = 256;

enum : uint64_t { DOM_KEY = 1, DOM_REPL = 2, DOM_DUMMY = 3, DOM_SYNTH_DB = 9, DOM_SYNTH_VEC = 10, DOM_SYNTH_NB = 11 };
__host__ __device__ inline uint64_t sm64(uint64_t x) {
  uint64_t z = x + 0x9e3779b97f4a7c15ULL;
  z = (z ^ (z >> 30)) * 0xbf58476d1ce4e5b9ULL;
  z = (z ^ (z >> 27)) * 0x94d049bb133111ebULL;
  return z ^ (z >> 31);
}
__host__ __device__ inline uint64_t hash4(uint64_t seed, uint64_t dom, uint64_t a, uint64_t b,
                                          uint64_t c) {
  uint64_t h = sm64(seed + dom);
  h = sm64(h ^ a);
  h = sm64(h ^ b);
  return sm64(h ^ c);
}

__host__ __device__ inline float graph_synth_vec(uint64_t kv, uint64_t v, uint32_t dim, uint32_t j) {
  return (float)(sm64(kv ^ (v * dim + j)) >> 40) * 0x1.0p-24f;
}
__host__ __device__ inline uint32_t graph_synth_nb(uint64_t kg, uint64_t n, uint64_t v, uint32_t m, uint32_t k) {
  const uint64_t c = v * m + k;
  uint64_t x = sm64(kg ^ c) % n;
  for (uint64_t a = 1; x == v; ++a) x = sm64(kg ^ c ^ (a << 56)) % n;
  return (uint32_t)x;
}
__host__ __device__ inline uint32_t graph_synth_elem(uint64_t kv, uint64_t kg, uint64_t n, uint32_t dim, uint32_t m,
                                                     uint64_t v, uint32_t e) {
  if (e < dim) return __builtin_bit_cast(uint32_t, graph_synth_vec(kv, v, dim, e));
  return graph_synth_nb(kg, n, v, m, e - dim);
}

struct PmPart {
  uint64_t N;
  uint64_t row0;
  uint64_t seed;
  uint64_t epoch;
  uint64_t idx;
  uint32_t CS, log2CS, SS, PH, Qpc, H, MaxQ, curk;
  uint32_t rk[44];
  PM_G uint32_t* tag;
  PM_G uint32_t* pp;
  PM_G uint64_t* parity;
  PM_G uint32_t* ridx;
  PM_G uint64_t* rval;
  PM_G uint32_t* hist;
  PM_G uint32_t* fqn;
  PM_G uint64_t* arena;
  PM_G uint16_t* tab;
  PM_G uint16_t* tabT;
  PM_G uint16_t* cur;
  const PM_G float* qv;
  const PM_G uint64_t* img;
};
struct PmSrvPart {
  uint64_t N;
  uint64_t row0;
  uint32_t CS, SS;
};

__host__ __device__ inline uint64_t tabT_index(uint32_t H, uint32_t t, uint32_t c) {
  return ((uint64_t)(c >> 3) * H + t) * 8 + (c & 7);
}
struct FoldImageSrc { uint64_t row; uint32_t word; bool packed; };
__host__ __device__ inline uint64_t tabT_words(uint32_t H, uint32_t SS) { return (uint64_t)((SS + 7) / 8) * 8 * H; }

#ifndef PM_CUR_K
#define PM_CUR_K 0
#endif
__host__ __device__ inline uint32_t cur_k(uint32_t PH, uint32_t SS) {
  return PM_CUR_K ? PM_CUR_K : ((uint64_t)PH * 2 > (uint64_t)SS * 128 ? 1u : 2u);
}
__host__ __device__ inline uint32_t cur_blocks(uint32_t PH) { return (PH + 7) >> 3; }
__host__ __device__ inline uint64_t cur_index(uint32_t PH, uint32_t K, uint32_t c, uint32_t h) {
  return K == 2 ? (((uint64_t)(c >> 1) * cur_blocks(PH) + (h >> 3)) * 2 + (c & 1)) * 8 + (h & 7)
                : (((uint64_t)(c / K) * cur_blocks(PH) + (h >> 3)) * K + (c % K)) * 8 + (h & 7);
}
__host__ __device__ inline uint64_t cur_row(uint32_t PH, uint32_t K, uint32_t c) { return cur_index(PH, K, c, 0); }
__host__ __device__ inline uint32_t cur_row_off(uint32_t K, uint32_t h) { return (h >> 3) * 8 * K + (h & 7); }
__host__ __device__ inline uint64_t cur_words(uint32_t PH, uint32_t SS, uint32_t K) {
  return (uint64_t)((SS + K - 1) / K) * cur_blocks(PH) * 8 * K;
}

enum : uint32_t { SUB_NONE = 0, SUB_REAL = 1, SUB_DUMMY = 2, SUB_HOSTCACHE = 3 };
enum : uint32_t {
  ST_OK = 0, ST_EBUDGET = 1, ST_ECHUNK = 2, ST_ENOHIT = 3, ST_ERANGE = 4,
  ST_DUMMY = 8, ST_CACHED = 9, ST_DUP = 10, ST_SKIP = 11
};
struct PmSub {
  uint32_t part, kind;
  uint64_t idx;
};
struct PmRes {
  uint32_t status, hit, chunk, ing;
  uint32_t tag, pp;
  uint32_t slot;
  uint32_t flags;
};
constexpr uint64_t kCsumMix = 0x9E3779B97F4A7C15ull;
__host__ __device__ inline uint64_t row_hash_mult(uint64_t w) { return sm64(w ^ 0x5851F42D4C957F2Dull) | 1ull; }
struct alignas(16) PmOutHdr {
  uint32_t status, ref;
  float dist;
  uint32_t token;
  uint64_t csum, pad;
};
#ifndef PM_KARG_SUBS
#define PM_KARG_SUBS 112
#endif
constexpr uint32_t kArgSubs = PM_KARG_SUBS, kArgParts = PM_KARG_SUBS > 1 ? 32 : 1;
constexpr uint32_t kStepHelpMax = 3, kHelpWords = 256, kHelpGran = 2 * kHelpWords + 8;
struct PmStep {
  const PM_G PmPart* parts;
  const PM_G PmSub* subs_h;
  const PM_G uint32_t* sb_h;
  PM_G PmSub* subs;
  PM_G uint32_t* sb;
  PM_G uint64_t* bits;
  PM_G uint32_t* cand;
  PM_G PmRes* res;
  PM_G uint64_t* ans;
  PM_G uint32_t* done;
  const PM_G uint64_t* db;
  const PM_G uint64_t* dbp;
  uint32_t pk_nseg, pk_cseg;
  const PM_G float* q;
  PM_G PmOutHdr* hdr_h;
  PM_G uint64_t* rows_h;
  PM_G uint64_t* stamps;
  PM_G uint32_t* meta;
  PM_G uint32_t* spec;
  PM_G uint64_t* recg;
  PM_G uint64_t* specg;
  PM_G uint64_t* bitsg;
  PM_G uint64_t* resg;
  PM_G uint64_t* helpg;
  uint32_t nhelp;
  uint32_t help_spoil;
  PM_G uint32_t* specrec;
  PM_G uint32_t* err_h;
  uint32_t words, E, dim, nsub, np, cblk;
  uint32_t np_live;
  uint32_t pf_w0, pf_w1;
  uint32_t rows_partial;
  uint32_t no_guess;
  uint32_t nsplit;
  PM_G uint64_t* part_x;
  PM_G uint16_t* qset;
  uint32_t qw;
  uint32_t args_valid;
  uint32_t token;
  uint32_t sb_a[kArgParts + 1];
  PmSub subs_a[kArgSubs];
};

__host__ __device__ inline uint32_t step_spec_word(uint32_t gmode, bool helped, bool help_ok, bool kept, bool redo,
                                                   uint32_t mode) {
  return (gmode & 7u) | (helped ? 8u : 0u) | (help_ok ? 16u : 0u) | (kept ? 32u : 0u) | (redo ? 64u : 0u) |
         ((mode & 7u) << 8) | 0x80000000u;
}

__host__ __device__ inline uint32_t drl_hash(uint32_t k) {
  uint64_t x = k;
  x ^= x >> 33; x *= 0xff51afd7ed558ccdULL; x ^= x >> 33;
  return (uint32_t)x;
}
struct DrlSess {
  uint64_t rng;
  uint64_t succ;
  uint32_t nknown, nheap;
  uint32_t pad0, pad1;
};
enum : uint32_t { DRL_BEGIN = 0, DRL_MID = 1, DRL_END = 2 };
struct DrlArgs {
  uint32_t S, P, qn, n, m, parallel, k, E, dim, kcap, cmask, ns, mode, q, qi, seq;
  uint32_t vec16;
  uint64_t N, PS;
  const PmOutHdr* hdr;
  const uint64_t* rows;
  PmSub* subs;
  uint64_t* gid;
  const uint32_t* graph;
  const float* start_dist;
  const uint32_t* start_ids;
  DrlSess* sess;
  uint64_t* dummy;
  uint32_t* batch;
  uint64_t* heap;
  uint64_t* ktab;
  uint32_t* knb;
  float* kdist;
  uint32_t* kid;
  uint64_t* const* ctab;
  int64_t* answers;
  const double* part_bytes;
  double* step_bytes;
  uint32_t* step_real;
  uint64_t* stamps;
};

struct KnbArgs {
  const float* vec;
  const uint32_t* graph;
  const uint32_t* start;
  const float* queries;
  uint32_t nq, ns, dim, m, k, max_step, parallel, kcap;
  int64_t* ids;
  int64_t* steps;
  uint32_t* needs_host;
};

}

namespace pmk {
using namespace pm;
void prep_init(hipStream_t st, const PmPart* dparts, int nparts, uint32_t maxH, uint32_t maxRepl,
               uint32_t E, bool zero_state);
void prep_offsets(hipStream_t st, const PmPart* dparts, int nparts, uint32_t maxH, uint32_t maxSS);
void set_aes_bs(int v);
enum : int { FOLD_GATHER = 0, FOLD_ROT512 = 1, FOLD_ROT1024 = 2, FOLD_PIPE = 3, FOLD_BLK = 4, FOLD_ROT512P = 5 };
int fold_form(uint32_t minCS, uint32_t maxCS, uint32_t E, bool have_img, uint32_t npk = 0);
void set_fold_rot(int v);
int prep_fold(hipStream_t st, const PmPart* dparts, int nparts, uint32_t maxH, const uint64_t* db,
              uint32_t E, uint32_t minCS, uint32_t maxCS, const uint64_t* zero16, uint32_t clients = 1,
              bool have_img = false, uint32_t minH = 0, uint32_t npk = 0);
void prep_repl(hipStream_t st, const PmPart* dparts, int nparts, uint32_t maxRepl,
               const uint64_t* db, uint32_t E);
void stream_fold(hipStream_t st, const PmPart* parts, uint32_t part, uint32_t H, const uint64_t* win, uint32_t c0,
                 uint32_t nc, uint32_t nrows, uint32_t E);
void stream_repl(hipStream_t st, const PmPart* parts, uint32_t part, uint32_t Qpc, const uint64_t* win, uint32_t c0,
                 uint32_t nc, uint32_t nrows, uint32_t E);
bool fold_image_ok(uint32_t minCS, uint32_t maxCS, uint32_t E);
bool fold_needs_tab(uint32_t minCS, uint32_t maxCS, uint32_t E, bool have_img);
uint64_t fold_image_words(uint32_t SS, uint32_t E, uint32_t CS, uint32_t npk = 0);
void fold_image(hipStream_t st, uint64_t* img, const uint64_t* part_rows, uint64_t N, uint32_t SS, uint32_t E,
                uint32_t CS, uint32_t npk = 0);
void set_fold_pack(int v);
uint32_t fold_pack_shape(uint32_t E, uint32_t dim);
uint32_t fold_pack_slices(uint32_t minCS, uint32_t maxCS, uint32_t E, uint32_t dim);
bool coord_low_zero(hipStream_t st, const uint64_t* rows, uint64_t nrows, uint32_t E, uint32_t dim, uint32_t* flag);
void set_answer_pack(int v);
uint32_t answer_pack_shape(uint32_t E, uint32_t dim);
uint32_t answer_pack_segs(uint32_t E, uint32_t dim);
void answer_pack_image(hipStream_t st, uint64_t* img, const uint64_t* rows, uint64_t nrows, uint32_t E, uint32_t dim);
void fold_image_map(uint32_t CS, uint32_t SS, uint32_t npk, uint64_t x0, uint64_t n, uint64_t* row, uint32_t* word,
                    uint8_t* packed);
struct PmEvents { hipEvent_t a = nullptr, b = nullptr; };
int set_option(const char* name, int value);
struct StepOpts { int match_part, match_part8, match_resolve, answer_waves, answer_nt, answer_pair, gather_split, step_help, step_help_spoil; };
StepOpts step_opts();
uint32_t step_match_blocks(uint32_t maxPH);
enum : int { STEP_ENGINE = 0, STEP_SHARED = 1, STEP_DEVICE = 2 };
inline bool step_args_fit(uint32_t nsub, uint32_t np) { return nsub <= kArgSubs && np <= kArgParts; }
struct StepShape {
  uint32_t np, nsub, np_live, max_per_part, maxPH, maxSS, E;
  bool ph8;
  bool args_valid;
  bool desc_shared;
  bool granules;
  bool unfused;
  bool no_split, no_guess;
  void of_caller(int kind, bool have_granules) {
    args_valid = kind != STEP_DEVICE && step_args_fit(nsub, np);
    desc_shared = kind == STEP_DEVICE || (kind == STEP_SHARED && !args_valid);
    granules = kind == STEP_ENGINE && have_granules;
  }
};
enum : int { MATCH_SUB = 0, MATCH_PART = 1, MATCH_PART8 = 2 };
enum : int { FORM_STEP = 0, FORM_RESOLVE_LDS, FORM_RESOLVE_G, FORM_MR_S2, FORM_MR_S4, FORM_MR_GENERAL,
             FORM_GATHER, FORM_ANSWER_P5, FORM_ANSWER_P, FORM_ANSWER_S, FORM_ANSWER_G, FORM_COUNT };
enum : int { STAGE_FUSED = 0, STAGE_MR, STAGE_MATCH, STAGE_RESOLVE, STAGE_GATHER, STAGE_ANSWER, STAGE_COUNT };
struct StepLaunch { int form = -1; uint32_t gx = 0, gy = 1, block = 0; };
struct StepPlan {
  StepLaunch at[STAGE_COUNT];
  uint32_t nhelp, nsplit, qw, np_live, cblk, no_guess;
  uint32_t help_spoil;
  bool qset;
};
StepPlan step_plan(const StepShape& s, const StepOpts& O);
void step_launch(hipStream_t st, const PmStep& S, const StepPlan& plan, int stage, PmEvents ev = {});
inline bool step_answer_packed(const PmStep& S, const StepPlan& plan, int stage) {
  const int form = plan.at[stage].form;
  return stage == STAGE_ANSWER && (form == FORM_ANSWER_P5 || form == FORM_ANSWER_P) && S.dbp != nullptr;
}
uint32_t step_max_sub_per_part();
uint32_t step_max_ss();
uint32_t step_max_e();
void client_sets(hipStream_t st, const PmStep& S, uint32_t* sets, uint32_t* modes, uint32_t qw);
void client_finish(hipStream_t st, const PmStep& S, const uint64_t* answers, const uint32_t* map);
bool client_mode_sends(uint32_t mode);
bool client_mode_reads(uint32_t mode);
uint32_t client_max_ss();
uint32_t client_max_e();
void server_answer(hipStream_t st, const PmPart* dpart, const uint32_t* offs, uint32_t nq,
                   uint32_t SS, const uint64_t* db, uint32_t E, uint64_t* out);
void server_answer_parts(hipStream_t st, const PmSrvPart* sp, const uint32_t* qpart, const uint32_t* offs,
                         uint32_t nq, uint32_t stride, const uint64_t* db, const uint64_t* dbp, uint32_t pk_nseg,
                         uint32_t pk_cseg, uint32_t E, uint64_t* out);
void l2_rows(hipStream_t st, const float* rows, uint64_t row_stride_floats, uint64_t nrows,
             const uint32_t* row_ids, const float* q, uint32_t dim, float* out, uint64_t seglen = 0);
void ip_rows(hipStream_t st, const uint32_t* rows, uint64_t nrows, const uint32_t* q, uint32_t dim,
             uint32_t* per_row, uint32_t* sum);
void ip_fill(hipStream_t st, uint32_t* rows, uint64_t N, uint32_t D, uint64_t r0 = 0);
void db_synth(hipStream_t st, uint64_t* dst, uint64_t r0, uint64_t rows, uint32_t E, uint64_t db_seed);
void gather_rows(hipStream_t st, const uint64_t* const* src, uint64_t n, uint32_t E, uint64_t* out);
void graph_synth(hipStream_t st, uint64_t* dst, uint64_t r0, uint64_t rows, uint64_t n, uint32_t dim, uint32_t m,
                 uint64_t seed);
void graph_synth_vecs(hipStream_t st, const uint64_t* ids, uint64_t nids, uint32_t dim, uint64_t seed, float* out);
void pack_records(hipStream_t st, const int32_t* map, uint32_t nrec, const PmOutHdr* hdr, const uint64_t* rows,
                  uint32_t E, uint32_t w0, uint32_t W, uint64_t* rec, uint32_t nsub, uint32_t* st2, uint64_t errw);
void synth_records(hipStream_t st, const int32_t* map, const uint64_t* ids, uint32_t nrec, uint32_t npos,
                   const float* qbuf, uint32_t dim, uint32_t m, uint64_t n, uint64_t seed, uint32_t w0, uint32_t W,
                   uint64_t* rec);
void prf_batch(hipStream_t st, const uint32_t* rk, const uint64_t* tags, const uint64_t* xs,
               uint64_t n, uint64_t* out);
void team_round(hipStream_t st, const DrlArgs& A, PmEvents ev = {});
uint32_t team_round_lds(uint32_t kcap, uint32_t n, uint32_t m);
constexpr uint32_t kDrlMaxKcap = 4096, kDrlMaxN = 256, kDrlMaxNM = 8192, kDrlMaxParallel = 8;
constexpr uint32_t kKnbMaxBatch = 256, kKnbMaxM = 64, kKnbMaxLds = 160 * 1024 - 512;
uint32_t knn_batch_kcap(uint64_t parallel, uint64_t max_step, uint64_t m);
uint64_t knn_batch_lds(uint32_t kcap, uint32_t dim, uint32_t nb, uint32_t ns);
bool knn_batch_ok(uint64_t dim, uint64_t m, uint64_t ns, uint64_t max_step, uint64_t parallel);
void knn_batch(hipStream_t st, const KnbArgs& A);
inline unsigned gcdiv(uint64_t a, uint64_t b) { return (unsigned)((a + b - 1) / b); }
inline unsigned gclamp(uint64_t blocks) { return (unsigned)(blocks < (1u << 20) ? blocks : (1u << 20)); }
uint32_t knn_pad_dim(uint32_t dim);
uint32_t knn_pad_dim_wide(uint32_t dim);
bool knn_wide(uint32_t width);
uint32_t knn_top();
uint32_t knn_top_k128();
uint32_t prune_max_list();
uint32_t prune_max_dim();
uint32_t prune_max_m();
void to_bf16(hipStream_t st, const float* rows, uint64_t n, uint32_t dim, uint32_t dp, void* out, float* norms);
void knn_prefilter(hipStream_t st, const void* X, const float* xn, uint64_t N, const void* Q, const float* qn,
                   uint64_t M, uint32_t dp, uint32_t* out, uint32_t* out_hi = nullptr);
void knn_rerank(hipStream_t st, const float* X, uint64_t N, uint32_t dim, const float* Q, uint64_t M,
                const uint32_t* cand, uint32_t K, bool self_base, uint32_t* out, float* dist, uint32_t* len);
void to_bf16x2(hipStream_t st, const float* rows, uint64_t n, uint32_t dim, uint32_t dp, void* hi, void* lo,
               float* norms, uint32_t* maxnorm);
void knn_prefilter_x3(hipStream_t st, const void* Xh, const void* Xl, const float* xn, uint64_t N, const void* Qh,
                      const void* Ql, const float* qn, uint64_t M, uint32_t dp, uint32_t top, uint32_t* out,
                      float* tau, uint32_t* out_hi = nullptr);
float knn_cert_rel(uint32_t dp);
void knn_rerank_cert(hipStream_t st, const float* X, uint64_t N, uint32_t dim, const float* Q, uint64_t M,
                     const uint32_t* cand, uint32_t K, bool self_base, uint32_t* out, float* dist, uint32_t* len,
                     const float* qn, const float* tau, const uint32_t* maxnorm, uint32_t dp, uint32_t top,
                     uint64_t* list, uint64_t* nlist, float* eps_out = nullptr);
void knn_brute(hipStream_t st, const float* X, uint64_t N, uint32_t dim, uint32_t top, const float* Q,
               const uint64_t* list, uint64_t nlist, uint32_t K, bool self_base, uint32_t* out, float* dist,
               uint32_t* len);
void prune(hipStream_t st, const float* X, uint32_t dim, bool wide, const uint32_t* verts, uint64_t nverts,
           const uint64_t* offs, uint64_t stride, const uint32_t* lens, const uint32_t* ids, uint32_t m,
           float alpha, uint32_t* out, uint32_t* out_len, uint32_t* err, const uint32_t* sorted_pos = nullptr,
           const float* dist_g = nullptr);
void cand_dist(hipStream_t st, const float* X, uint32_t dim, const uint32_t* verts, uint64_t nverts,
               const uint64_t* offs, const uint32_t* lens, const uint32_t* ids, float* dist_g);
uint32_t knn_u8_max_dim();
uint32_t knn_u8_pad_dim(uint32_t dim);
void u8_bias(hipStream_t st, const uint8_t* rows, uint64_t n, uint32_t dim, uint32_t dp, void* out, int32_t* cst);
void u8_to_f32(hipStream_t st, const uint8_t* rows, uint64_t count, float* out);
void knn_i8(hipStream_t st, const void* X, const int32_t* xc, uint64_t N, const void* Q, const int32_t* qc, uint64_t M,
            uint32_t dp, uint32_t K, bool self_base, uint32_t* out, float* dist, uint32_t* len);
struct ScanWork {
  uint64_t r0, r1;
  uint32_t q, pad;
};
constexpr uint32_t kKmeansPartials = 16;
size_t cluster_sort_temp(uint64_t n, uint64_t nc);
hipError_t cluster_sort(hipStream_t st, void* temp, size_t temp_bytes, const uint32_t* labels, uint64_t n, uint64_t nc,
                        uint64_t* keys, uint64_t* keys_out, uint32_t* order, uint64_t* offs);
void kmeans_update(hipStream_t st, const float* rows, uint32_t dim, const uint32_t* order, const uint64_t* offs,
                   uint64_t nc, float* centroids);
void kmeans_moved(hipStream_t st, const uint32_t* cur, const uint32_t* prev, uint64_t n, uint64_t* count);
void cluster_gather(hipStream_t st, const float* rows, uint64_t n, uint32_t dim, const uint32_t* order, float* out);
void cluster_scan(hipStream_t st, const float* S, const uint32_t* order, uint32_t dim, const float* Q,
                  const ScanWork* work, uint64_t nwork, uint32_t K, uint64_t* lists);
void cluster_merge(hipStream_t st, const uint64_t* lists, const uint64_t* woff, uint64_t nq, uint32_t K, uint32_t* out,
                   float* dist, uint32_t* len);
}
```

pacmann_amd/csrc/pm_kernels.hip:

```cpp
#include <atomic>
#include "pm_aes.h"
#include "pm_aes_bs.h"
#include "pm_internal.h"

namespace pm {
#ifndef PM_PREP_NT
#define PM_PREP_NT 0
#endif


__device__ __forceinline__ uint32_t xor3(uint32_t a, uint32_t b, uint32_t c) {
  return __builtin_amdgcn_bitop3_b32(a, b, c, 0x96);
}
__device__ __forceinline__ uint4 xor4(uint4 a, uint4 b) {
  return make_uint4(a.x ^ b.x, a.y ^ b.y, a.z ^ b.z, a.w ^ b.w);
}

#ifndef PM_OFFS_CHUNKS
#define PM_OFFS_CHUNKS 8
#endif
constexpr int kOffsChunksPerBlock = PM_OFFS_CHUNKS;
constexpr int kOffsBlock = 1024;

#ifndef PM_OFFS_TILES
// ... 159 lines not shown
    } else {
      if ((q & 1) == 0) continue;
#pragma unroll
      for (int j = 0; j < 32; ++j) T[j] = 0xffffffffu;
    }
    uint32_t* tt = reinterpret_cast<uint32_t*>(P.tabT + tabT_index(H, h0, c));
    if (h0 + 32 <= H) {
#pragma unroll
      for (int j = 0; j < 32; ++j) tt[4 * j] = T[j];
    } else {
#pragma unroll
      for (int j = 0; j < 32; ++j)
        if (h0 + j < H) tt[4 * j] = T[j];
    }
    if (c >= SS) continue;
#pragma unroll
    for (int jb = 0; jb < 4; ++jb) {
      const uint32_t hb = h0 + 8 * jb;
      uint4 wlo, whi;
      wlo.x = __builtin_amdgcn_perm(T[8 * jb + 1], T[8 * jb + 0], 0x05040100u);
      wlo.y = __builtin_amdgcn_perm(T[8 * jb + 3], T[8 * jb + 2], 0x05040100u);
      wlo.z = __builtin_amdgcn_perm(T[8 * jb + 5], T[8 * jb + 4], 0x05040100u);
      wlo.w = __builtin_amdgcn_perm(T[8 * jb + 7], T[8 * jb + 6], 0x05040100u);
      whi.x = __builtin_amdgcn_perm(T[8 * jb + 1], T[8 * jb + 0], 0x07060302u);
      whi.y = __builtin_amdgcn_perm(T[8 * jb + 3], T[8 * jb + 2], 0x07060302u);
      whi.z = __builtin_amdgcn_perm(T[8 * jb + 5], T[8 * jb + 4], 0x07060302u);
      whi.w = __builtin_amdgcn_perm(T[8 * jb + 7], T[8 * jb + 6], 0x07060302u);
      if (hb < PH) {
        *reinterpret_cast<uint4*>(P.cur + cur_index(PH, P.curk, c, hb)) = wlo;
        *reinterpret_cast<uint4*>(P.cur + cur_index(PH, P.curk, c + 1, hb)) = whi;
      }
      if (P.tab && hb < H) {
        *reinterpret_cast<uint4*>(P.tab + (uint64_t)c * H + hb) = wlo;
        *reinterpret_cast<uint4*>(P.tab + (uint64_t)(c + 1) * H + hb) = whi;
      }
    }
  }
}

#ifndef PM_FOLD_NT
#define PM_FOLD_NT 1
#endif
template <int W>
__global__ void __launch_bounds__(kBlock) k_prep_fold(const PmPart* __restrict__ parts,
                                                      const uint64_t* __restrict__ db, uint32_t E) {
  const PmPart& P = parts[blockIdx.y];
  const uint32_t EX = E & ~3u, NSEG = EX / W;
  const uint64_t e = (uint64_t)blockIdx.x * kBlock + threadIdx.x;
  const uint32_t H = P.H;
  if (NSEG == 0) {
    if (e < (uint64_t)H * E) P.parity[e] = 0;
    return;
  }
  const uint32_t h = (uint32_t)(e / NSEG), seg = (uint32_t)(e % NSEG);
  if (h >= H) return;
  const uint64_t* base = db + (P.row0 * E) + (uint64_t)seg * W;
  const uint32_t CS = P.CS, SS = P.SS;
  const uint64_t N = P.N;
  uint64_t a0 = 0, a1 = 0;
  uint32_t c = 0;
  for (; c + 4 <= SS; c += 4) {
    const uint64_t t4 = *reinterpret_cast<const uint64_t*>(P.tabT + tabT_index(H, h, c));
    uint16_t v[4];
#pragma unroll
    for (int u = 0; u < 4; ++u) v[u] = (uint16_t)(t4 >> (16 * u));
#pragma unroll
    for (int u = 0; u < 4; ++u) {
      const uint64_t r = (uint64_t)(c + u) * CS + v[u];
      if (v[u] != kSkip && r < N) {
        const uint64_t* p = base + r * E;
        if (W == 2) {
          typedef uint32_t u32x4 __attribute__((ext_vector_type(4)));
          const u32x4 x = PM_FOLD_NT ? __builtin_nontemporal_load(reinterpret_cast<const u32x4*>(p))
                                     : *reinterpret_cast<const u32x4*>(p);
          a0 ^= ((uint64_t)x.y << 32) | x.x;
          a1 ^= ((uint64_t)x.w << 32) | x.z;
        } else {
          a0 ^= PM_FOLD_NT ? __builtin_nontemporal_load(p) : *p;
        }
      }
    }
  }
  for (; c < SS; ++c) {
    uint16_t v = P.tabT[tabT_index(H, h, c)];
    const uint64_t r = (uint64_t)c * CS + v;
    if (v != kSkip && r < N) {
      const uint64_t* p = base + r * E;
      a0 ^= p[0];
      if (W == 2) a1 ^= p[1];
    }
  }
  uint64_t* dst = P.parity + (uint64_t)h * E + (uint64_t)seg * W;
  dst[0] = a0;
  if (W == 2) dst[1] = a1;
  if (seg == 0)
    for (uint32_t w = EX; w < E; ++w) P.parity[(uint64_t)h * E + w] = 0;
}

constexpr int kFoldThreads = 1024, kFoldHPT = 7;
constexpr int kFoldHPTBlk = 4;
constexpr uint32_t kFoldMaxItems = 4;
typedef __attribute__((address_space(3))) void lds_void_t;
typedef __attribute__((address_space(1))) const void g_cvoid_t;

__device__ __forceinline__ void lds_dma16(const void* src, const void* lds_wave_base) {
  const uint32_t m = __builtin_amdgcn_readfirstlane((uint32_t)(uintptr_t)(lds_void_t*)lds_wave_base);
  asm volatile("s_nop 0\n\tglobal_load_lds_dwordx4 %0, off" ::"v"(src), "{m0}"(m) : "memory");
}

template <int SW>
__global__ void __launch_bounds__(kFoldThreads) k_prep_fold_blk(const PmPart* __restrict__ parts,
                                                                const uint64_t* __restrict__ db,
                                                                const uint64_t* __restrict__ zero16,
                                                                uint32_t E, uint32_t w0) {
  extern __shared__ __attribute__((aligned(16))) uint64_t fold_lds[];
  typedef uint64_t u64x2 __attribute__((ext_vector_type(2)));
  constexpr uint32_t IPE = SW / 2;
  const PmPart& P = parts[blockIdx.z];
  const uint32_t H = P.H, CS = P.CS, SS = P.SS, tid = threadIdx.x;
  const uint32_t ng = (H + kFoldThreads * kFoldHPTBlk - 1) / (kFoldThreads * kFoldHPTBlk);
  if (blockIdx.x >= ng) return;
  const uint32_t hb = (H + ng - 1) / ng, h0 = blockIdx.x * hb, h1 = min(H, h0 + hb);
  const uint32_t w = w0 + blockIdx.y * SW;
  const uint64_t N = P.N;
  const PM_G uint64_t* base = (const PM_G uint64_t*)db + P.row0 * E + w;
  const PM_G uint16_t* tab = P.tab;
  const uint32_t rowWords = (CS + 1) * SW, items = CS * IPE;
  const uint32_t wave_item0 = tid & ~63u;
  uint32_t hk[kFoldHPTBlk];
  uint64_t acc[kFoldHPTBlk][SW];
#pragma unroll
  for (int k = 0; k < kFoldHPTBlk; ++k) {
    hk[k] = h0 + tid + k * kFoldThreads;
#pragma unroll
    for (int x = 0; x < SW; ++x) acc[k][x] = 0;
  }
  uint32_t v[kFoldHPTBlk], nv[kFoldHPTBlk];
  auto stage = [&](uint32_t c, uint32_t buf) {
    uint64_t* L = fold_lds + buf * rowWords;
#pragma unroll
    for (uint32_t i = 0; i < kFoldMaxItems; ++i) {
      const uint32_t it = tid + i * kFoldThreads;
      if (i * kFoldThreads + wave_item0 < items && it < items) {
        const uint64_t r = (uint64_t)c * CS + it / IPE;
        const PM_G uint64_t* src = r < N ? base + r * E + (it % IPE) * 2 : (const PM_G uint64_t*)zero16;
        __builtin_amdgcn_global_load_lds((g_cvoid_t*)src, (lds_void_t*)(L + (i * kFoldThreads + wave_item0) * 2),
                                         16, 0, 0);
      }
    }
  };
  auto load_tab = [&](uint32_t c, uint32_t* out) {
#pragma unroll
    for (int k = 0; k < kFoldHPTBlk; ++k) out[k] = hk[k] < h1 ? tab[(uint64_t)c * H + hk[k]] : kSkip;
  };
  stage(0, 0);
  load_tab(0, v);
  for (uint32_t x = tid; x < 2 * SW; x += kFoldThreads) fold_lds[(x / SW) * rowWords + CS * SW + x % SW] = 0;
  asm volatile("s_waitcnt vmcnt(0)" ::: "memory");
  __syncthreads();
  for (uint32_t c = 0; c < SS; ++c) {
    const bool more = c + 1 < SS;
    if (more) { stage(c + 1, (c + 1) & 1); load_tab(c + 1, nv); }
    const uint64_t* L = fold_lds + (c & 1) * rowWords;
#pragma unroll
    for (int k = 0; k < kFoldHPTBlk; ++k) {
      const uint32_t o = v[k] == kSkip ? CS : v[k];
      const uint64_t* row = L + o * SW;
#pragma unroll
      for (int x = 0; x < SW; x += 2) {
        const u64x2 y = *reinterpret_cast<const u64x2*>(row + x);
        acc[k][x] ^= y.x;
        acc[k][x + 1] ^= y.y;
      }
    }
    asm volatile("s_waitcnt vmcnt(0)" ::: "memory");
    __syncthreads();
#pragma unroll
    for (int k = 0; k < kFoldHPTBlk; ++k) v[k] = nv[k];
  }
#pragma unroll
  for (int k = 0; k < kFoldHPTBlk; ++k) {
    if (hk[k] >= h1) continue;
    PM_G uint64_t* dst = P.parity + (uint64_t)hk[k] * E + w;
#pragma unroll
    for (int x = 0; x < SW; x += 2) *reinterpret_cast<PM_G u64x2*>(dst + x) = u64x2{acc[k][x], acc[k][x + 1]};
    if (w == 0)
      for (uint32_t t = E & ~3u; t < E; ++t) P.parity[(uint64_t)hk[k] * E + t] = 0;
  }
}

constexpr uint32_t kPipeTabWords = kFoldThreads * kFoldHPT / 4;

__device__ __forceinline__ void wait_vmcnt(uint32_t n) {
  switch (__builtin_amdgcn_readfirstlane(n)) {
#define PM_VMC(i) case i: asm volatile("s_waitcnt vmcnt(" #i ")" ::: "memory"); break;
    PM_VMC(1) PM_VMC(2) PM_VMC(3) PM_VMC(4) PM_VMC(5) PM_VMC(6) PM_VMC(7) PM_VMC(8)
    PM_VMC(9) PM_VMC(10) PM_VMC(11) PM_VMC(12) PM_VMC(13) PM_VMC(14) PM_VMC(15)
#undef PM_VMC
    default: asm volatile("s_waitcnt vmcnt(0)" ::: "memory");
  }
}

template <int SW, int G, int NB, int D = 1>
__global__ void __launch_bounds__(kFoldThreads) k_prep_fold_pipe(const PmPart* __restrict__ parts,
                                                                 const uint64_t* __restrict__ db,
                                                                 const uint64_t* __restrict__ zero16,
                                                                 uint32_t E, uint32_t ngmax, uint32_t nsl,
                                                                 uint32_t npg, uint32_t K) {
  extern __shared__ __attribute__((aligned(16))) uint64_t fold_lds[];
  typedef uint64_t u64x2 __attribute__((ext_vector_type(2)));
  constexpr uint32_t IPE = SW / 2, CS = G * kFoldThreads / IPE;
  constexpr uint32_t LW = 16 / SW;
  const uint32_t ngl = (nsl + LW - 1) / LW, per_pg = K * ngl * LW;
  const uint32_t xcd = blockIdx.x % 8, k = blockIdx.x / 8;
  const uint32_t pg = xcd + 8 * (k / per_pg), r = k % per_pg;
  const uint32_t client = (r / LW) % K, slice = (r / (K * LW)) * LW + r % LW;
  if (pg >= npg || slice >= nsl) return;
  const PmPart& P = parts[(pg / ngmax) * K + client];
  const uint32_t H = P.H, SS = P.SS, tid = threadIdx.x;
  const uint32_t ng = (H + kFoldThreads * kFoldHPT - 1) / (kFoldThreads * kFoldHPT);
  const uint32_t grp = pg % ngmax;
  if (grp >= ng) return;
  const uint32_t hb = (((H + ng - 1) / ng) + 7) & ~7u, h0 = grp * hb, h1 = min(H, h0 + hb);
  const uint32_t w = slice * SW;
  const uint64_t N = P.N;
  const PM_G uint64_t* base = (const PM_G uint64_t*)db + P.row0 * E + w;
  const PM_G uint16_t* tab = P.tab;
  constexpr uint32_t TABW = (CS + 1) * SW, BUFW = TABW + kPipeTabWords;
  const uint32_t wave_item0 = tid & ~63u;
  const bool tab_wave = tid < kPipeTabWords / 2;
  uint32_t hk[kFoldHPT];
  uint64_t acc[kFoldHPT][SW];
#pragma unroll
  for (int k = 0; k < kFoldHPT; ++k) {
    hk[k] = h0 + tid + k * kFoldThreads;
#pragma unroll
    for (int x = 0; x < SW; ++x) acc[k][x] = 0;
  }
  auto stage = [&](uint32_t c, uint32_t buf) {
    uint64_t* L = fold_lds + buf * BUFW;
#pragma unroll
    for (uint32_t i = 0; i < (uint32_t)G; ++i) {
      const uint32_t it = tid + i * kFoldThreads;
      const uint64_t r = (uint64_t)c * CS + it / IPE;
      const PM_G uint64_t* src = r < N ? base + r * E + (it % IPE) * 2 : (const PM_G uint64_t*)zero16;
      __builtin_amdgcn_global_load_lds((g_cvoid_t*)src, (lds_void_t*)(L + (i * kFoldThreads + wave_item0) * 2),
                                       16, 0, 0);
    }
    if (tab_wave) {
      const uint32_t hh = h0 + tid * 8;
      const PM_G uint64_t* src = hh < h1 ? (const PM_G uint64_t*)(tab + (uint64_t)c * H + hh)
                                         : (const PM_G uint64_t*)zero16;
      __builtin_amdgcn_global_load_lds((g_cvoid_t*)src, (lds_void_t*)(L + TABW + wave_item0 * 2), 16, 0, 0);
    }
  };
  for (uint32_t x = tid; x < NB * SW; x += kFoldThreads) fold_lds[(x / SW) * BUFW + CS * SW + x % SW] = 0;
  static_assert(NB > D, "fold pipeline: more buffers than chunks per barrier");
  for (uint32_t c = 0; c + D < (uint32_t)NB && c < SS; ++c) stage(c, c);
  const uint32_t ops = G + (tab_wave ? 1 : 0);
  auto wait_chunks = [&](uint32_t next, uint32_t issued) {
    const uint32_t need = min(SS, next + D);
    wait_vmcnt(issued > need ? (issued - need) * ops : 0);
    asm volatile("s_waitcnt lgkmcnt(0)" ::: "memory");
    __builtin_amdgcn_s_barrier();
  };
  wait_chunks(0, min(SS, (uint32_t)(NB - D)));
  const uint32_t fl = SW == 4 ? ((tid & 1u) << 1) : 0u;
  for (uint32_t c0 = 0; c0 < SS; c0 += D) {
#pragma unroll
    for (int j = 0; j < D; ++j)
      if (c0 + NB - D + j < SS) stage(c0 + NB - D + j, (c0 + NB - D + j) % NB);
#pragma unroll
    for (int j = 0; j < D; ++j) {
    const uint32_t c = c0 + j;
    if (D > 1 && c >= SS) break;
    const uint64_t* L = fold_lds + (c % NB) * BUFW;
    const uint16_t* T = reinterpret_cast<const uint16_t*>(L + TABW);
#pragma unroll
    for (int k = 0; k < kFoldHPT; ++k) {
      const uint32_t t = hk[k] < h1 ? T[hk[k] - h0] : kSkip;
      const uint64_t* row = L + (t == kSkip ? CS : t) * SW;
#pragma unroll
      for (int x = 0; x < SW; x += 2) {
        const u64x2 y = *reinterpret_cast<const u64x2*>(row + (x ^ fl));
        acc[k][x] ^= y.x;
        acc[k][x + 1] ^= y.y;
      }
    }
    }
    if (c0 + D < SS) wait_chunks(c0 + D, min(SS, c0 + NB));
  }
#pragma unroll
  for (int k = 0; k < kFoldHPT; ++k) {
    if (hk[k] >= h1) continue;
    PM_G uint64_t* dst = P.parity + (uint64_t)hk[k] * E + w;
#pragma unroll
    for (int x = 0; x < SW; x += 2)
      *reinterpret_cast<PM_G u64x2*>(dst + (x ^ fl)) = u64x2{acc[k][x], acc[k][x + 1]};
    if (w == 0)
      for (uint32_t t = E & ~3u; t < E; ++t) P.parity[(uint64_t)hk[k] * E + t] = 0;
  }
}

#ifndef PM_ROT_HPL
#define PM_ROT_HPL 5
#endif
#ifndef PM_ROT_GB
#define PM_ROT_GB 4
#endif
#ifndef PM_ROT_SB
#define PM_ROT_SB 8
#endif
#ifndef PM_ROT_HPL2
#define PM_ROT_HPL2 7
#endif
constexpr int kRotHPL = PM_ROT_HPL;
__host__ __device__ constexpr int rot_hpl(uint32_t cs) { return cs == 512 ? kRotHPL : PM_ROT_HPL2; }
constexpr uint32_t kRotBufBytes = 512 * 128;
__host__ __device__ constexpr uint32_t rot_nch(uint32_t cs) { return cs == 512 ? 4 : 2; }
template <int CS>
__global__ void __launch_bounds__(kFoldThreads) k_prep_fold_rot(const PmPart* __restrict__ parts, uint32_t E,
                                                                uint32_t nvg, uint32_t nsl, uint32_t npv,
                                                                uint32_t npk_arg, uint32_t K, uint32_t ngc) {
  constexpr uint32_t NCH = rot_nch(CS), LINE = NCH * 8, BUFW = (CS + 1) * LINE;
  constexpr int HPL = rot_hpl(CS);
  static_assert(CS == 512 || CS == 1024, "4 chunks of 512 rows or 2 of 1,024 per block");
  static_assert(CS * LINE * 4 == kRotBufBytes, "64 KB blocks");
  __shared__ __attribute__((aligned(16))) uint32_t rot_lds[2 * BUFW];
  constexpr uint32_t ITEMS = CS * NCH * 2;
  static_assert(ITEMS % kFoldThreads == 0, "whole staging items per thread");
  constexpr uint32_t G = ITEMS / kFoldThreads;
  constexpr uint32_t HB = kFoldThreads * HPL;
  const uint32_t npk = CS == 512 ? npk_arg : 0u;
  const uint32_t xcd = blockIdx.x % 8, kq = blockIdx.x / 8;
  constexpr uint32_t GB = PM_ROT_GB, SB = PM_ROT_SB;
  const uint32_t nsb = (nsl + SB - 1) / SB, ngb = (npv + GB - 1) / GB;
  const uint32_t T = (kq / (GB * SB)) * 8 + xcd, wt = kq % (GB * SB);
  if (T >= ngb * nsb) return;
  const uint32_t gsup = T / (8 * nsb), m = min(8u, ngb - gsup * 8), r = T - gsup * 8 * nsb;
  const uint32_t pgv = (gsup * 8 + r % m) * GB + wt % GB;
  const uint32_t slice = (r / m) * SB + wt / GB;
  if (pgv >= npv || slice >= nsl) return;
  const uint32_t part = pgv / nvg, vg = pgv % nvg;
  const PmPart& P = parts[part * K];
  const uint32_t H = P.H, SS = P.SS, tid = threadIdx.x;
  const uint32_t vend = K * H;
  uint32_t v0, v1;
  if (ngc == 0) {
    v0 = vg * HB;
    if (v0 >= vend) return;
    v1 = min(v0 + HB, vend);
  } else {
    const uint32_t c = vg / ngc, g = vg % ngc;
    if (c >= K || g * HB >= H) return;
    v0 = c * H + g * HB;
    v1 = min(v0 + HB, (c + 1) * H);
  }
  const uint32_t cA = v0 / H, cB = min(cA + 1, K - 1), vb = (cA + 1) * H;
  const PmPart& PA = parts[part * K + cA];
  const PmPart& PB = parts[part * K + cB];
  const PM_G uint16_t* const tabA = PA.tabT;
  const PM_G uint16_t* const tabB = PB.tabT;
  const uint32_t hA = cA * H;
  const uint32_t w = slice < npk ? slice * 8 : (slice + npk) * 4;
  const uint32_t nbuf = SS / NCH;
  const PM_G char* img = (const PM_G char*)P.img + (uint64_t)slice * nbuf * kRotBufBytes;
  const uint32_t lane = tid & 63, j = (lane / NCH) & 1, ks = lane & (NCH - 1);
  const uint32_t vl = v0 + tid;
  uint32_t acc[HPL][8];
#pragma unroll
  for (int k = 0; k < HPL; ++k)
#pragma unroll
    for (int t = 0; t < 8; ++t) acc[k][t] = 0;
  const uint32_t wave_item0 = tid & ~63u;
  auto stage = [&](uint32_t b, uint32_t buf) {
    uint32_t* L = rot_lds + buf * BUFW;
    const PM_G char* src = img + (uint64_t)b * kRotBufBytes;
#pragma unroll
    for (uint32_t i = 0; i < G; ++i)
      lds_dma16(src + (tid + i * kFoldThreads) * 16u, L + (i * kFoldThreads + wave_item0) * 4);
  };
  typedef uint32_t u32x2 __attribute__((ext_vector_type(2)));
  using Tile = std::conditional_t<NCH == 4, u32x2, uint32_t>;
  auto load_tab = [&](uint32_t b, Tile* out) {
#pragma unroll
    for (int k = 0; k < HPL; ++k) {
      const uint32_t v = min(vl + k * kFoldThreads, vend - 1);
      const bool inB = v >= vb;
      const PM_G char* src = (const PM_G char*)(inB ? tabB : tabA) + (uint32_t)tabT_index(H, v - (inB ? vb : hA), NCH * b) * 2u;
      out[k] = *reinterpret_cast<const PM_G Tile*>(src);
    }
  };
  for (uint32_t x = tid; x < 2 * LINE; x += kFoldThreads) rot_lds[(x / LINE) * BUFW + CS * LINE + x % LINE] = 0;
  Tile tv[HPL], tn[HPL];
  stage(0, 0);
  auto skip_idle = [&](Tile* t) {
#pragma unroll
    for (int k = 0; k < HPL; ++k)
      if (vl + k * kFoldThreads >= v1) t[k] = ~Tile{};
  };
  load_tab(0, tv);
  asm volatile("s_waitcnt vmcnt(0)" ::: "memory");
  __syncthreads();
  skip_idle(tv);
  const char* lds0 = reinterpret_cast<const char*>(rot_lds);
  for (uint32_t b = 0; b < nbuf; ++b) {
    if (b + 1 < nbuf) { stage(b + 1, (b + 1) & 1); load_tab(b + 1, tn); }
    const uint32_t lb = (b & 1) * BUFW * 4;
    uint32_t cso[NCH], psel[NCH];
#pragma unroll
    for (uint32_t ph = 0; ph < NCH; ++ph) {
      const uint32_t sl = (ks + ph) & (NCH - 1);
      cso[ph] = lb + sl * 32 + 16 * j;
      psel[ph] = 0x0c0c0000u | ((2 * sl + 1) << 8) | (2 * sl);
    }
#pragma unroll
    for (int k = 0; k < HPL; ++k) {
#pragma unroll
      for (uint32_t p0 = 0; p0 < NCH; p0 += 2) {
        uint32_t v[2][8];
#pragma unroll
        for (uint32_t pp = 0; pp < 2; ++pp) {
          const uint32_t ph = p0 + pp;
          uint32_t o;
          if constexpr (NCH == 4) o = __builtin_amdgcn_perm(tv[k].y, tv[k].x, psel[ph]);
          else o = __builtin_amdgcn_perm(0u, tv[k], psel[ph]);
          o = min(o, (uint32_t)CS);
          const uint32_t a = o * (LINE * 4) + cso[ph];
          const uint4 x0 = *reinterpret_cast<const uint4*>(lds0 + a);
          const uint4 x1 = *reinterpret_cast<const uint4*>(lds0 + (a ^ 16u));
          v[pp][0] = x0.x; v[pp][1] = x0.y; v[pp][2] = x0.z; v[pp][3] = x0.w;
          v[pp][4] = x1.x; v[pp][5] = x1.y; v[pp][6] = x1.z; v[pp][7] = x1.w;
        }
#pragma unroll
        for (int t = 0; t < 8; ++t)
          acc[k][t] = xor3(acc[k][t], v[0][t], v[1][t]);
      }
    }
    asm volatile("s_waitcnt vmcnt(0)" ::: "memory");
    __syncthreads();
#pragma unroll
    for (int k = 0; k < HPL; ++k) tv[k] = tn[k];
    skip_idle(tv);
  }
#pragma unroll
  for (int k = 0; k < HPL; ++k) {
    const uint32_t v = vl + k * kFoldThreads;
    if (v >= v1) continue;
    const bool inB = v >= vb;
    PM_G uint64_t* const par = (inB ? PB.parity : PA.parity) + (uint64_t)(v - (inB ? vb : hA)) * E;
    PM_G uint32_t* dst = reinterpret_cast<PM_G uint32_t*>(par + w);
    if (slice < npk) {
      typedef uint32_t u32x4 __attribute__((ext_vector_type(4)));
#pragma unroll
      for (int t = 0; t < 8; t += 2) {
        PM_G u32x4* const d = reinterpret_cast<PM_G u32x4*>(dst + 8 * (j ^ (t >> 2)) + 2 * (t & 3));
        const u32x4 x = {acc[k][t] << 16, acc[k][t] & 0xffff0000u, acc[k][t + 1] << 16, acc[k][t + 1] & 0xffff0000u};
        if (PM_PREP_NT) __builtin_nontemporal_store(x, d);
        else *d = x;
      }
    } else {
#pragma unroll
      for (int t = 0; t < 8; ++t) {
        PM_G uint32_t* const d = dst + 4 * (j ^ (t >> 2)) + (t & 3);
        if (PM_PREP_NT) __builtin_nontemporal_store(acc[k][t], d);
        else *d = acc[k][t];
      }
    }
    if (w == 0)
      for (uint32_t t = E & ~3u; t < E; ++t) par[t] = 0;
  }
}

__host__ __device__ inline FoldImageSrc fold_image_src(uint64_t x, uint32_t nbuf, uint32_t CS, uint32_t npk) {
  const uint32_t lg = CS == 512 ? 2 : 1;
  const uint32_t it = (uint32_t)(x % (kRotBufBytes / 16));
  const uint64_t blk = x / (kRotBufBytes / 16);
  const uint32_t b = (uint32_t)(blk % nbuf), s = (uint32_t)(blk / nbuf);
  FoldImageSrc o;
  o.row = (uint64_t)((b << lg) + ((it >> 1) & ((1u << lg) - 1))) * CS + (it >> (lg + 1));
  o.packed = s < npk;
  o.word = o.packed ? 16 * s + 8 * (it & 1) : 8 * (s + npk) + 4 * (it & 1);
  return o;
}
__global__ void __launch_bounds__(kBlock) k_fold_image(uint4* __restrict__ img, const uint64_t* __restrict__ rows,
                                                      uint64_t N, uint32_t nbuf, uint32_t E, uint64_t nitems,
                                                      uint32_t CS, uint32_t npk) {
  for (uint64_t x = (uint64_t)blockIdx.x * kBlock + threadIdx.x; x < nitems; x += (uint64_t)gridDim.x * kBlock) {
    const FoldImageSrc src = fold_image_src(x, nbuf, CS, npk);
    uint4 v = make_uint4(0, 0, 0, 0);
    if (src.row < N) {
      const uint4* const p = reinterpret_cast<const uint4*>(reinterpret_cast<const uint32_t*>(rows + src.row * E) + src.word);
      v = p[0];
      if (src.packed) {
        const uint4 u = p[1];
        v = make_uint4((v.x >> 16) | (v.y & 0xffff0000u), (v.z >> 16) | (v.w & 0xffff0000u),
                       (u.x >> 16) | (u.y & 0xffff0000u), (u.z >> 16) | (u.w & 0xffff0000u));
      }
    }
    img[x] = v;
  }
}
__global__ void __launch_bounds__(kBlock) k_answer_pack_image(uint4* __restrict__ img, const uint64_t* __restrict__ rows,
                                                             uint64_t nitems, uint32_t E, uint32_t nseg, uint32_t cseg) {
  for (uint64_t x = (uint64_t)blockIdx.x * kBlock + threadIdx.x; x < nitems; x += (uint64_t)gridDim.x * kBlock) {
    const uint64_t r = x / nseg;
    const uint32_t s = (uint32_t)(x - r * nseg);
    const uint32_t* const row = reinterpret_cast<const uint32_t*>(rows + r * E);
    uint4 v;
    if (s < cseg) {
      const uint4* const p = reinterpret_cast<const uint4*>(row + 8 * s);
      const uint4 a = p[0], u = p[1];
      v = make_uint4((a.x >> 16) | (a.y & 0xffff0000u), (a.z >> 16) | (a.w & 0xffff0000u),
                     (u.x >> 16) | (u.y & 0xffff0000u), (u.z >> 16) | (u.w & 0xffff0000u));
    } else {
      v = *reinterpret_cast<const uint4*>(row + 8 * cseg + 4 * (s - cseg));
    }
    img[x] = v;
  }
}
__global__ void __launch_bounds__(kBlock) k_coord_low_or(const uint64_t* __restrict__ rows, uint64_t nrows, uint32_t E,
                                                        uint32_t dim, uint32_t* __restrict__ out) {
  const uint32_t per = dim / 4;
  const uint64_t nitems = nrows * per;
  uint32_t acc = 0;
  for (uint64_t x = (uint64_t)blockIdx.x * kBlock + threadIdx.x; x < nitems; x += (uint64_t)gridDim.x * kBlock) {
    const uint64_t r = x / per;
    const uint4 v = reinterpret_cast<const uint4*>(rows + r * E)[x - r * per];
    acc |= v.x | v.y | v.z | v.w;
  }
  if (acc & 0xffffu) atomicOr(out, 1u);
}

constexpr uint32_t kReplRows = 32, kReplIt = (kReplRows * 1024 / 16 + kBlock - 1) / kBlock;
template <int W>
__global__ void __launch_bounds__(kBlock) k_prep_repl(const PmPart* __restrict__ parts,
                                                      const uint64_t* __restrict__ db, uint32_t E) {
  typedef uint64_t vec __attribute__((ext_vector_type(W)));
  __shared__ uint32_t rrow[kReplRows];
  const PmPart& P = parts[blockIdx.y];
  const uint32_t nslot = P.SS * P.Qpc;
  const uint32_t s0 = blockIdx.x * kReplRows;
  if (s0 >= nslot) return;
  const uint32_t ns = min(kReplRows, nslot - s0);
  if (threadIdx.x < ns) {
    const uint32_t slot = s0 + threadIdx.x, c = slot / P.Qpc;
    const uint64_t off = hash4(P.seed, DOM_REPL, P.idx, P.epoch, slot) & (P.CS - 1);
    const uint64_t r = (uint64_t)c * P.CS + off;
    P.ridx[slot] = (uint32_t)r;
    rrow[threadIdx.x] = r < P.N ? (uint32_t)r : ~0u;
  }
  __syncthreads();
  const uint32_t nseg = E / W, tot = ns * nseg;
  const uint64_t* const src = db + P.row0 * E;
  uint64_t* const dst = P.rval + (uint64_t)s0 * E;
  for (uint32_t x0 = 0; x0 < tot; x0 += kReplIt * kBlock) {
    vec v[kReplIt];
    uint32_t at[kReplIt];
#pragma unroll
    for (uint32_t u = 0; u < kReplIt; ++u) {
      const uint32_t x = x0 + u * kBlock + threadIdx.x;
      at[u] = ~0u;
      v[u] = vec{};
      if (x < tot) {
        const uint32_t i = x / nseg, sg = x - i * nseg, r = rrow[i];
        at[u] = i * E + sg * W;
        if (r != ~0u) v[u] = *reinterpret_cast<const vec*>(src + (uint64_t)r * E + sg * W);
      }
    }
#pragma unroll
    for (uint32_t u = 0; u < kReplIt; ++u)
      if (at[u] != ~0u) *reinterpret_cast<vec*>(dst + at[u]) = v[u];
  }
}

__global__ void __launch_bounds__(kBlock) k_prep_init(const PmPart* __restrict__ parts) {
  const PmPart& P = parts[blockIdx.y];
  const uint32_t i = blockIdx.x * kBlock + threadIdx.x;
  if (i < P.H) P.tag[i] = i;
  if (i < P.PH) P.pp[i] = kDefaultProgramPoint;
  if (i < P.SS) P.hist[i] = 0;
  if (i < P.SS * P.Qpc) P.ridx[i] = kDefaultProgramPoint;
  if (i == 0) *P.fqn = 0;
}

template <int W>
__global__ void __launch_bounds__(kBlock) k_server_answer(const PmPart* __restrict__ parts,
                                                          const uint32_t* __restrict__ qoffs,
                                                          uint32_t maxSS,
                                                          const uint64_t* __restrict__ db, uint32_t E,
                                                          uint64_t* __restrict__ ans) {
  __shared__ uint64_t red[kBlock * 2];
  const uint32_t s = blockIdx.x;
  const PmPart& P = parts[0];
  const uint32_t EX = E & ~3u, NSEG = EX / W;
  const uint32_t* qo = qoffs + (uint64_t)s * maxSS;
  const uint64_t* base = db + P.row0 * E;
  uint64_t* out = ans + (uint64_t)s * E;
  for (uint32_t seg0 = 0; seg0 < NSEG; seg0 += kBlock) {
    const uint32_t nseg = min(NSEG - seg0, (uint32_t)kBlock);
    const uint32_t nsl = kBlock / nseg;
    const uint32_t sl = threadIdx.x / nseg, seg = seg0 + threadIdx.x % nseg;
    uint64_t a0 = 0, a1 = 0;
    if (sl < nsl) {
      for (uint32_t i = sl; i < P.SS; i += nsl) {
        const uint64_t r = (uint64_t)i * P.CS + qo[i];
        if (r < P.N) {
          const uint64_t* p = base + r * E + (uint64_t)seg * W;
          if (W == 2) {
            uint4 x = *reinterpret_cast<const uint4*>(p);
            a0 ^= ((uint64_t)x.y << 32) | x.x;
            a1 ^= ((uint64_t)x.w << 32) | x.z;
          } else {
            a0 ^= *p;
          }
        }
      }
    }
    red[threadIdx.x * 2] = a0;
    red[threadIdx.x * 2 + 1] = a1;
    __syncthreads();
    if (threadIdx.x < nseg) {
      uint64_t x0 = 0, x1 = 0;
      for (uint32_t k = 0; k < nsl; ++k) {
        x0 ^= red[(k * nseg + threadIdx.x) * 2];
        x1 ^= red[(k * nseg + threadIdx.x) * 2 + 1];
      }
      out[(uint64_t)seg * W] = x0;
      if (W == 2) out[(uint64_t)seg * W + 1] = x1;
    }
    __syncthreads();
  }
  for (uint32_t w = EX + threadIdx.x; w < E; w += kBlock) out[w] = 0;
}

constexpr uint32_t kSrvFlight = 4;
template <int W, bool PK>
__global__ void __launch_bounds__(kBlock) k_server_answer_parts(const PmSrvPart* __restrict__ sp,
                                                                const uint32_t* __restrict__ qpart,
                                                                const uint32_t* __restrict__ qoffs, uint32_t stride,
                                                                const uint64_t* __restrict__ rows, uint32_t rw,
                                                                uint32_t NSEG, uint32_t cseg, uint32_t E,
                                                                uint64_t* __restrict__ ans) {
  static_assert(!PK || W == 2, "packed rows are whole 16-B segments");
  __shared__ uint64_t red[kBlock * 2];
  const uint32_t s = blockIdx.x;
  const PmSrvPart P = sp[qpart[s]];
  const uint32_t* qo = qoffs + (uint64_t)s * stride;
  const uint64_t* base = rows + P.row0 * rw;
  uint64_t* out = ans + (uint64_t)s * E;
  for (uint32_t seg0 = 0; seg0 < NSEG; seg0 += kBlock) {
    const uint32_t nseg = min(NSEG - seg0, (uint32_t)kBlock);
    const uint32_t nsl = kBlock / nseg;
    const uint32_t sl = threadIdx.x / nseg, seg = seg0 + threadIdx.x % nseg;
    uint64_t a0 = 0, a1 = 0;
    if (sl < nsl) {
      for (uint32_t i0 = sl; i0 < P.SS; i0 += kSrvFlight * nsl) {
        uint64_t x0[kSrvFlight], x1[kSrvFlight];
#pragma unroll
        for (uint32_t u = 0; u < kSrvFlight; ++u) {
          const uint32_t i = i0 + u * nsl;
          x0[u] = 0; x1[u] = 0;
          if (i >= P.SS) continue;
          const uint64_t r = (uint64_t)i * P.CS + qo[i];
          if (r >= P.N) continue;
          const uint64_t* p = base + r * rw + (uint64_t)seg * W;
          if (W == 2) {
            const uint4 x = *reinterpret_cast<const uint4*>(p);
            x0[u] = ((uint64_t)x.y << 32) | x.x;
            x1[u] = ((uint64_t)x.w << 32) | x.z;
          } else {
            x0[u] = *p;
          }
        }
#pragma unroll
        for (uint32_t u = 0; u < kSrvFlight; ++u) { a0 ^= x0[u]; a1 ^= x1[u]; }
      }
    }
    red[threadIdx.x * 2] = a0;
    red[threadIdx.x * 2 + 1] = a1;
    __syncthreads();
    if (threadIdx.x < nseg) {
      uint64_t x0 = 0, x1 = 0;
      for (uint32_t k = 0; k < nsl; ++k) {
        x0 ^= red[(k * nseg + threadIdx.x) * 2];
        x1 ^= red[(k * nseg + threadIdx.x) * 2 + 1];
      }
      if (PK && seg < cseg) {
        const uint32_t v[4] = {(uint32_t)x0, (uint32_t)(x0 >> 32), (uint32_t)x1, (uint32_t)(x1 >> 32)};
#pragma unroll
        for (uint32_t k = 0; k < 4; ++k)
          out[4 * seg + k] = ((uint64_t)(v[k] & 0xffff0000u) << 32) | (uint64_t)(uint32_t)(v[k] << 16);
      } else if (PK) {
        out[4 * cseg + 2 * (seg - cseg)] = x0;
        out[4 * cseg + 2 * (seg - cseg) + 1] = x1;
      } else {
        out[(uint64_t)seg * W] = x0;
        if (W == 2) out[(uint64_t)seg * W + 1] = x1;
      }
    }
    __syncthreads();
  }
  for (uint32_t w = (E & ~3u) + threadIdx.x; w < E; w += kBlock) out[w] = 0;
}

__global__ void __launch_bounds__(kBlock) k_l2_rows(const float* __restrict__ rows,
                                                    uint64_t stride, uint64_t nrows,
                                                    const uint32_t* __restrict__ ids,
                                                    const float* __restrict__ q, uint32_t dim,
                                                    float* __restrict__ out, uint64_t seglen) {
  const uint64_t g = ((uint64_t)blockIdx.x * kBlock + threadIdx.x) >> 3;
  const uint32_t k = threadIdx.x & 7;
  const bool live = g < nrows;
  const float* r = rows + (live ? (ids ? (uint64_t)ids[g] : g) : 0) * stride;
  if (seglen && live) q += (g / seglen) * dim;
  const uint32_t dimS = dim & ~7u;
  float acc = 0.0f;
  if (live)
    for (uint32_t t = k; t < dimS; t += 8) {
      const float d = __fsub_rn(r[t], q[t]);
      acc = __fadd_rn(acc, __fmul_rn(d, d));
    }
  acc = __fadd_rn(acc, __shfl_xor(acc, 1));
  acc = __fadd_rn(acc, __shfl_xor(acc, 2));
  acc = __fadd_rn(acc, __shfl_xor(acc, 4));
  if (live && k == 0) {
    float d = dimS ? acc : 0.0f;
    for (uint32_t i = dimS; i < dim; ++i) {
      const float t = __fsub_rn(r[i], q[i]);
      d = __fadd_rn(d, __fmul_rn(t, t));
    }
    out[g] = d;
  }
}

__global__ void __launch_bounds__(kBlock) k_ip_rows(const uint32_t* __restrict__ rows, uint64_t nrows,
                                                    const uint32_t* __restrict__ q, uint32_t dim,
                                                    uint32_t* __restrict__ per_row,
                                                    uint32_t* __restrict__ sum) {
  const uint64_t g = ((uint64_t)blockIdx.x * kBlock + threadIdx.x) >> 4;
  const uint32_t l = threadIdx.x & 15;
  uint32_t acc = 0;
  if (g < nrows) {
    const uint32_t* r = rows + g * dim;
    for (uint32_t j = l; j < dim; j += 16) acc += r[j] * q[j];
  }
#pragma unroll
  for (int m = 1; m < 16; m <<= 1) acc += __shfl_xor(acc, m);
  if (g < nrows && l == 0 && per_row) per_row[g] = acc;
  uint32_t w = (l == 0 && g < nrows) ? acc : 0;
#pragma unroll
  for (int m = 16; m < 64; m <<= 1) w += __shfl_xor(w, m);
  if ((threadIdx.x & 63) == 0) atomicAdd(sum, w);
}

__global__ void __launch_bounds__(kBlock) k_ip_scan(const uint4* __restrict__ rows, uint64_t n4,
                                                    const uint32_t* __restrict__ q, uint32_t dim,
                                                    uint32_t* __restrict__ sum) {
  __shared__ uint32_t qs[4096];
  for (uint32_t j = threadIdx.x; j < dim; j += kBlock) qs[j] = q[j];
  __syncthreads();
  uint32_t acc = 0;
  const uint64_t stride = (uint64_t)gridDim.x * kBlock;
  const uint32_t dim4 = dim / 4;
  typedef unsigned int u32x4 __attribute__((ext_vector_type(4)));
  const u32x4* r4 = reinterpret_cast<const u32x4*>(rows);
  uint64_t f = (uint64_t)blockIdx.x * kBlock + threadIdx.x;
  if (stride % dim4 == 0) {
    const uint32_t j = (uint32_t)(f % dim4) * 4;
    const uint32_t q0 = qs[j], q1 = qs[j + 1], q2 = qs[j + 2], q3 = qs[j + 3];
    constexpr int kU = 8;
    for (; f + (kU - 1) * stride < n4; f += kU * stride) {
      u32x4 t[kU];
#pragma unroll
      for (int u = 0; u < kU; ++u) t[u] = __builtin_nontemporal_load(r4 + f + u * stride);
#pragma unroll
      for (int u = 0; u < kU; ++u) acc += t[u].x * q0 + t[u].y * q1 + t[u].z * q2 + t[u].w * q3;
    }
    for (; f < n4; f += stride) {
      const u32x4 t = __builtin_nontemporal_load(r4 + f);
      acc += t.x * q0 + t.y * q1 + t.z * q2 + t.w * q3;
    }
  } else {
    for (; f < n4; f += stride) {
      const u32x4 t = __builtin_nontemporal_load(r4 + f);
      const uint32_t j = (uint32_t)(f % dim4) * 4;
      acc += t.x * qs[j] + t.y * qs[j + 1] + t.z * qs[j + 2] + t.w * qs[j + 3];
    }
  }
#pragma unroll
  for (int m = 1; m < 64; m <<= 1) acc += __shfl_xor(acc, m);
  if ((threadIdx.x & 63) == 0) atomicAdd(sum, acc);
}

__global__ void __launch_bounds__(kBlock) k_ip_fill(uint4* __restrict__ rows, uint64_t n4, uint32_t dim,
                                                    uint64_t r0) {
  const uint64_t stride = (uint64_t)gridDim.x * kBlock;
  for (uint64_t f = (uint64_t)blockIdx.x * kBlock + threadIdx.x; f < n4; f += stride) {
    const uint64_t e = f * 4;
    const uint32_t i = (uint32_t)(r0 + e / dim), j = (uint32_t)(e % dim);
    rows[f] = make_uint4(i + j, i + j + 1, i + j + 2, i + j + 3);
  }
}

__global__ void __launch_bounds__(kBlock) k_db_synth(uint64_t* __restrict__ dst, uint64_t r0, uint64_t nw,
                                                     uint32_t E, uint64_t k) {
  const uint64_t stride = (uint64_t)gridDim.x * kBlock, x0 = r0 * E;
  for (uint64_t f = (uint64_t)blockIdx.x * kBlock + threadIdx.x; f < nw; f += stride)
    __builtin_nontemporal_store(sm64(k ^ (x0 + f)), dst + f);
}

__global__ void __launch_bounds__(kBlock) k_prf_batch(const uint32_t* __restrict__ rk,
                                                      const uint64_t* __restrict__ tags,
                                                      const uint64_t* __restrict__ xs, uint64_t n,
                                                      uint64_t* __restrict__ out) {
  __shared__ uint32_t te[kTeLdsWords];
  __shared__ uint32_t srk[44];
  aes_lds_init<kBlock>(te, g_aes.te0);
  if (threadIdx.x < 44) srk[threadIdx.x] = rk[threadIdx.x];
  __syncthreads();
  const AesLane A(te, threadIdx.x);
  for (uint64_t i = (uint64_t)blockIdx.x * kBlock + threadIdx.x; i < n; i += (uint64_t)gridDim.x * kBlock)
    out[i] = prf64(A, srk, tags[i], xs[i]);
}

__global__ void __launch_bounds__(kBlock) k_gather_rows(const uint64_t* const* __restrict__ src, uint32_t E,
                                                         uint64_t* __restrict__ out) {
  const uint64_t i = blockIdx.x;
  const uint64_t* r = src[i];
  uint64_t* o = out + i * (E + 1);
  for (uint32_t w = threadIdx.x; w < E; w += kBlock) o[w] = r ? r[w] : 0;
  if (threadIdx.x == 0) o[E] = r ? 1 : 0;
}

}

namespace pmk {
static inline unsigned cdiv(uint64_t a, uint64_t b) { return (unsigned)((a + b - 1) / b); }

void prep_init(hipStream_t st, const PmPart* d, int np, uint32_t maxH, uint32_t maxRepl, uint32_t,
               bool) {
  const uint32_t n = maxH > maxRepl ? maxH : maxRepl;
  hipLaunchKernelGGL(k_prep_init, dim3(cdiv(n, kBlock), np), dim3(kBlock), 0, st, d);
}
void prep_offsets_tt(hipStream_t st, const PmPart* d, int np, uint32_t maxH, uint32_t maxSS) {
  hipLaunchKernelGGL(k_prep_offsets, dim3(cdiv(maxH, kOffsBlock), cdiv(maxSS, kOffsChunksPerBlock * kOffsTiles), np),
                     dim3(kOffsBlock), 0, st, d);
}
void prep_offsets_bs(hipStream_t st, const PmPart* d, int np, uint32_t maxH, uint32_t maxSS) {
  hipLaunchKernelGGL(k_prep_offsets_bs, dim3(cdiv((uint64_t)cdiv(maxH, 32) * cdiv(maxSS, 8), kBsThreads), np),
                     dim3(kBsThreads), 0, st, d);
}
static std::atomic<int> g_aes_bs{-1};
void set_aes_bs(int v) { g_aes_bs.store(v < 0 ? -1 : (v ? 1 : 0)); }
bool prep_offsets_bitsliced() {
  static const bool env = [] { const char* e = getenv("PM_AES_BS"); return e && e[0] == '1'; }();
  const int v = g_aes_bs.load();
  return v < 0 ? env : v == 1;
}
void prep_offsets(hipStream_t st, const PmPart* d, int np, uint32_t maxH, uint32_t maxSS) {
  if (prep_offsets_bitsliced()) prep_offsets_bs(st, d, np, maxH, maxSS);
  else prep_offsets_tt(st, d, np, maxH, maxSS);
}
static std::atomic<int> g_fold_rot{-1};
void set_fold_rot(int v) { g_fold_rot.store(v < 0 ? -1 : (v ? 1 : 0)); }
static bool fold_rot_shape(uint32_t minCS, uint32_t maxCS, uint32_t E) {
  return minCS == maxCS && (maxCS == 512 || maxCS == 1024) && E % 2 == 0 && E >= 4;
}
bool fold_image_ok(uint32_t minCS, uint32_t maxCS, uint32_t E) {
  static const bool env = [] { const char* e = getenv("PM_FOLD_ROT"); return !e || e[0] != '0'; }();
  const int v = g_fold_rot.load();
  return (v < 0 ? env : v == 1) && fold_rot_shape(minCS, maxCS, E);
}
static uint32_t fold_blk_sw(uint32_t maxCS) {
  auto fits = [&](uint32_t sw) {
    return 2ull * (maxCS + 1) * sw * 8 <= 150u * 1024 &&
           (uint64_t)maxCS * (sw / 2) <= (uint64_t)kFoldMaxItems * kFoldThreads;
  };
  uint32_t sw = 8;
  while (sw > 2 && !fits(sw)) sw /= 2;
  return fits(sw) ? sw : 0;
}
int fold_form(uint32_t minCS, uint32_t maxCS, uint32_t E, bool have_img, uint32_t npk) {
  if ((E & ~3u) == 0) return FOLD_GATHER;
  if (have_img && fold_rot_shape(minCS, maxCS, E))
    return maxCS == 512 ? (npk ? FOLD_ROT512P : FOLD_ROT512) : FOLD_ROT1024;
  if (minCS == maxCS && (maxCS == 512 || maxCS == 1024 || maxCS == 2048) && E % 2 == 0) return FOLD_PIPE;
  if (E % 2 || !fold_blk_sw(maxCS)) return FOLD_GATHER;
  return FOLD_BLK;
}
bool fold_needs_tab(uint32_t minCS, uint32_t maxCS, uint32_t E, bool have_img) {
  const int form = fold_form(minCS, maxCS, E, have_img);
  return form == FOLD_PIPE || form == FOLD_BLK;
}
static std::atomic<int> g_fold_pack{-1};
void set_fold_pack(int v) { g_fold_pack.store(v < 0 ? -1 : (v ? 1 : 0)); }
uint32_t fold_pack_slices(uint32_t minCS, uint32_t maxCS, uint32_t E, uint32_t dim) {
  static const bool env = [] { const char* e = getenv("PM_FOLD_PACK"); return !e || e[0] != '0'; }();
  const int v = g_fold_pack.load();
  if (!(v < 0 ? env : v == 1) || fold_form(minCS, maxCS, E, true) != FOLD_ROT512) return 0;
  return fold_pack_shape(E, dim);
}
uint32_t fold_pack_shape(uint32_t E, uint32_t dim) {
  return dim && dim % 16 == 0 && dim / 8 <= E / 4 ? dim / 16 : 0;
}
static std::atomic<int> g_answer_pack{-1};
void set_answer_pack(int v) { g_answer_pack.store(v < 0 ? -1 : (v ? 1 : 0)); }
uint32_t answer_pack_shape(uint32_t E, uint32_t dim) {
  if (!dim || E % 4 || E > 256 || dim % 8 || dim >= 2 * E) return 0;
  const uint32_t stride = 2 * dim + 4 * (2 * E - dim);
  return stride % 16 ? 0 : stride / 16;
}
uint32_t answer_pack_segs(uint32_t E, uint32_t dim) {
  static const bool env = [] { const char* e = getenv("PM_ANSWER_PACK"); return !e || e[0] != '0'; }();
  const int v = g_answer_pack.load();
  return (v < 0 ? env : v == 1) ? answer_pack_shape(E, dim) : 0;
}
void answer_pack_image(hipStream_t st, uint64_t* img, const uint64_t* rows, uint64_t nrows, uint32_t E, uint32_t dim) {
  const uint32_t nseg = answer_pack_shape(E, dim);
  const uint64_t nitems = nrows * nseg;
  unsigned grid = cdiv(nitems, kBlock);
  if (grid > 256 * 32) grid = 256 * 32;
  if (grid) hipLaunchKernelGGL(k_answer_pack_image, dim3(grid), dim3(kBlock), 0, st, (uint4*)img, rows, nitems, E, nseg, dim / 8);
}
bool coord_low_zero(hipStream_t st, const uint64_t* rows, uint64_t nrows, uint32_t E, uint32_t dim, uint32_t* flag) {
  if (hipMemsetAsync(flag, 0, 4, st) != hipSuccess) return false;
  unsigned grid = cdiv(nrows * (dim / 4), kBlock);
  if (grid > 256 * 32) grid = 256 * 32;
  if (grid) hipLaunchKernelGGL(k_coord_low_or, dim3(grid), dim3(kBlock), 0, st, rows, nrows, E, dim, flag);
  uint32_t h = 1;
  if (hipMemcpyAsync(&h, flag, 4, hipMemcpyDeviceToHost, st) != hipSuccess || hipStreamSynchronize(st) != hipSuccess)
    return false;
  return h == 0;
}
uint64_t fold_image_words(uint32_t SS, uint32_t E, uint32_t CS, uint32_t npk) {
  return (uint64_t)(E / 4 - npk) * (SS / rot_nch(CS)) * (kRotBufBytes / 8);
}
void fold_image(hipStream_t st, uint64_t* img, const uint64_t* rows, uint64_t N, uint32_t SS, uint32_t E, uint32_t CS,
                uint32_t npk) {
  const uint64_t nitems = fold_image_words(SS, E, CS, npk) / 2;
  unsigned grid = cdiv(nitems, kBlock);
  if (grid > 256 * 32) grid = 256 * 32;
  hipLaunchKernelGGL(k_fold_image, dim3(grid), dim3(kBlock), 0, st, (uint4*)img, rows, N, SS / rot_nch(CS), E, nitems,
                     CS, npk);
}
void fold_image_map(uint32_t CS, uint32_t SS, uint32_t npk, uint64_t x0, uint64_t n, uint64_t* row, uint32_t* word,
                    uint8_t* packed) {
  for (uint64_t i = 0; i < n; ++i) {
    const FoldImageSrc s = fold_image_src(x0 + i, SS / rot_nch(CS), CS, npk);
    row[i] = s.row; word[i] = s.word; packed[i] = s.packed;
  }
}
int prep_fold(hipStream_t st, const PmPart* d, int np, uint32_t maxH, const uint64_t* db, uint32_t E,
              uint32_t minCS, uint32_t maxCS, const uint64_t* zero16, uint32_t clients, bool have_img,
               uint32_t minH, uint32_t npk) {
  const int form = fold_form(minCS, maxCS, E, have_img, npk);
  const uint32_t EX = E & ~3u;
  if (EX == 0) {
    hipLaunchKernelGGL(k_prep_fold<2>, dim3(cdiv((uint64_t)maxH * E, kBlock), np), dim3(kBlock), 0,
                       st, d, db, E);
    return form;
  }
  const uint32_t ng = cdiv(maxH, (uint64_t)kFoldThreads * kFoldHPT);
  const uint32_t ngb = cdiv(maxH, (uint64_t)kFoldThreads * kFoldHPTBlk);
  auto launch = [&](uint32_t sw, uint32_t w0, uint32_t nsl) {
    const size_t lds = 2ull * (maxCS + 1) * sw * 8;
    const dim3 grid(ngb, nsl, np), blk(kFoldThreads);
    if (sw == 8) hipLaunchKernelGGL(k_prep_fold_blk<8>, grid, blk, lds, st, d, db, zero16, E, w0);
    else if (sw == 4) hipLaunchKernelGGL(k_prep_fold_blk<4>, grid, blk, lds, st, d, db, zero16, E, w0);
    else hipLaunchKernelGGL(k_prep_fold_blk<2>, grid, blk, lds, st, d, db, zero16, E, w0);
  };
  if (form == FOLD_ROT512 || form == FOLD_ROT512P || form == FOLD_ROT1024 || form == FOLD_PIPE) {
    const uint32_t psw = maxCS == 2048 ? 2 : 4, nsl = EX / psw - (form == FOLD_ROT512P ? npk : 0);
    const uint32_t K = clients && np % clients == 0 ? clients : 1, npg = (np / K) * ng;
    const uint32_t lw = 16 / psw, per_pg = K * cdiv(nsl, lw) * lw;
#ifndef PM_FOLD_NB512
#define PM_FOLD_NB512 4
#endif
#ifndef PM_FOLD_D512
#define PM_FOLD_D512 1
#endif
    if (form != FOLD_PIPE) {
      const uint64_t HB = (uint64_t)kFoldThreads * rot_hpl(maxCS);
      const uint32_t ngc = minH >= HB ? 0u : (uint32_t)cdiv(maxH, HB);
      const uint32_t nvg = ngc ? K * ngc : (uint32_t)cdiv((uint64_t)K * maxH, HB), npv = (np / K) * nvg;
      const uint32_t grid = 8 * cdiv((uint64_t)cdiv(npv, PM_ROT_GB) * cdiv(nsl, PM_ROT_SB), 8) * PM_ROT_GB * PM_ROT_SB;
      if (form != FOLD_ROT1024)
        hipLaunchKernelGGL(k_prep_fold_rot<512>, dim3(grid), dim3(kFoldThreads), 0, st, d, E, nvg, nsl, npv,
                           form == FOLD_ROT512P ? npk : 0u, K, ngc);
      else
        hipLaunchKernelGGL(k_prep_fold_rot<1024>, dim3(grid), dim3(kFoldThreads), 0, st, d, E, nvg, nsl, npv, 0u, K, ngc);
      return form;
    }
    const uint32_t nb = maxCS == 512 ? PM_FOLD_NB512 : 3;
    const size_t lds = (size_t)nb * ((maxCS + 1) * psw + kPipeTabWords) * 8;
    const dim3 grid(cdiv(npg, 8) * 8 * per_pg), blk(kFoldThreads);
    if (maxCS == 512)
      hipLaunchKernelGGL((k_prep_fold_pipe<4, 1, PM_FOLD_NB512, PM_FOLD_D512>), grid, blk, lds, st, d, db, zero16, E, ng, nsl,
                         npg, K);
    else if (maxCS == 1024)
      hipLaunchKernelGGL((k_prep_fold_pipe<4, 2, 3>), grid, blk, lds, st, d, db, zero16, E, ng, nsl, npg, K);
    else
      hipLaunchKernelGGL((k_prep_fold_pipe<2, 2, 3>), grid, blk, lds, st, d, db, zero16, E, ng, nsl, npg, K);
    return form;
  }
  if (form == FOLD_GATHER) {
    if (E % 2 == 0)
      hipLaunchKernelGGL(k_prep_fold<2>, dim3(cdiv((uint64_t)maxH * (EX / 2), kBlock), np),
                         dim3(kBlock), 0, st, d, db, E);
    else
      hipLaunchKernelGGL(k_prep_fold<1>, dim3(cdiv((uint64_t)maxH * EX, kBlock), np), dim3(kBlock), 0,
                         st, d, db, E);
    return form;
  }
  const uint32_t sw = fold_blk_sw(maxCS);
  const uint32_t nfull = EX / sw, rem = EX % sw;
  if (nfull) launch(sw, 0, nfull);
  if (rem) launch(rem, nfull * sw, 1);
  return form;
}
void prep_repl(hipStream_t st, const PmPart* d, int np, uint32_t maxRepl, const uint64_t* db,
               uint32_t E) {
  if (E % 2 == 0)
    hipLaunchKernelGGL(k_prep_repl<2>, dim3(cdiv(maxRepl, kReplRows), np), dim3(kBlock), 0, st, d, db, E);
  else
    hipLaunchKernelGGL(k_prep_repl<1>, dim3(cdiv(maxRepl, kReplRows), np), dim3(kBlock), 0, st, d, db, E);
}
void server_answer(hipStream_t st, const PmPart* d, const uint32_t* offs, uint32_t nq, uint32_t SS,
                   const uint64_t* db, uint32_t E, uint64_t* out) {
  if (E % 2 == 0)
    hipLaunchKernelGGL(k_server_answer<2>, dim3(nq), dim3(kBlock), 0, st, d, offs, SS, db, E, out);
  else
    hipLaunchKernelGGL(k_server_answer<1>, dim3(nq), dim3(kBlock), 0, st, d, offs, SS, db, E, out);
}
void server_answer_parts(hipStream_t st, const PmSrvPart* sp, const uint32_t* qpart, const uint32_t* offs,
                         uint32_t nq, uint32_t stride, const uint64_t* db, const uint64_t* dbp, uint32_t pk_nseg,
                         uint32_t pk_cseg, uint32_t E, uint64_t* out) {
  const uint32_t EX = E & ~3u;
  if (dbp)
    hipLaunchKernelGGL((k_server_answer_parts<2, true>), dim3(nq), dim3(kBlock), 0, st, sp, qpart, offs, stride, dbp,
                       2 * pk_nseg, pk_nseg, pk_cseg, E, out);
  else if (E % 2 == 0)
    hipLaunchKernelGGL((k_server_answer_parts<2, false>), dim3(nq), dim3(kBlock), 0, st, sp, qpart, offs, stride, db,
                       E, EX / 2, 0u, E, out);
  else
    hipLaunchKernelGGL((k_server_answer_parts<1, false>), dim3(nq), dim3(kBlock), 0, st, sp, qpart, offs, stride, db,
                       E, EX, 0u, E, out);
}
void l2_rows(hipStream_t st, const float* rows, uint64_t stride, uint64_t nrows, const uint32_t* ids,
             const float* q, uint32_t dim, float* out, uint64_t seglen) {
  if (!nrows) return;
  hipLaunchKernelGGL(k_l2_rows, dim3(cdiv(nrows * 8, kBlock)), dim3(kBlock), 0, st, rows, stride, nrows,
                     ids, q, dim, out, seglen);
}
void ip_rows(hipStream_t st, const uint32_t* rows, uint64_t nrows, const uint32_t* q, uint32_t dim,
             uint32_t* per_row, uint32_t* sum) {
  if (!per_row && dim % 4 == 0 && dim <= 4096) {
    const uint64_t n4 = nrows * dim / 4;
    unsigned grid = cdiv(n4, kBlock);
    if (grid > 256 * 8) grid = 256 * 8;
    if (grid == 0) return;
    hipLaunchKernelGGL(k_ip_scan, dim3(grid), dim3(kBlock), 0, st, (const uint4*)rows, n4, q, dim, sum);
    return;
  }
  if (!nrows) return;
  hipLaunchKernelGGL(k_ip_rows, dim3(cdiv(nrows * 16, kBlock)), dim3(kBlock), 0, st, rows, nrows, q, dim,
                     per_row, sum);
}
void ip_fill(hipStream_t st, uint32_t* rows, uint64_t N, uint32_t D, uint64_t r0) {
  const uint64_t n4 = N * D / 4;
  unsigned grid = cdiv(n4, kBlock);
  if (grid > 256 * 16) grid = 256 * 16;
  if (grid == 0) return;
  hipLaunchKernelGGL(k_ip_fill, dim3(grid), dim3(kBlock), 0, st, (uint4*)rows, n4, D, r0);
}
void db_synth(hipStream_t st, uint64_t* dst, uint64_t r0, uint64_t rows, uint32_t E, uint64_t db_seed) {
  const uint64_t nw = rows * E;
  unsigned grid = cdiv(nw, kBlock);
  if (grid > 256 * 32) grid = 256 * 32;
  if (grid == 0) return;
  hipLaunchKernelGGL(k_db_synth, dim3(grid), dim3(kBlock), 0, st, dst, r0, nw, E, sm64(db_seed + DOM_SYNTH_DB));
}
void gather_rows(hipStream_t st, const uint64_t* const* src, uint64_t n, uint32_t E, uint64_t* out) {
  if (n) hipLaunchKernelGGL(k_gather_rows, dim3((unsigned)n), dim3(kBlock), 0, st, src, E, out);
}
void prf_batch(hipStream_t st, const uint32_t* rk, const uint64_t* tags, const uint64_t* xs, uint64_t n,
               uint64_t* out) {
  unsigned grid = cdiv(n, kBlock * 16);
  if (grid == 0) return;
  if (grid > 2048) grid = 2048;
  hipLaunchKernelGGL(k_prf_batch, dim3(grid), dim3(kBlock), 0, st, rk, tags, xs, n, out);
}
}
```

Baseline: 29200.

## Bit-pack fold image into narrow coordinate and id fields for ROT512 fold

Adds a FOLD_ROT512Q form in which the precomputed fold image stores row words as packed 12/16/20-bit fields, chosen from a device-side OR scan of which bits the database rows actually use. The fold kernel unpacks the fields back to full words before storing, so fewer image slices have to be streamed from HBM during each prep_fold. The scan kernel now reports low-half, coordinate-bit and id-bit usage instead of a single low-zero flag, and the ROT kernel takes its grid blocking as runtime arguments. In exchange the fold does extra shift and mask work per field, and correctness relies on the scan bounding the value ranges exactly.

Measured after the change: 29760, median of 6. 1.9% higher.

```diff
diff --git a/pacmann_amd/csrc/pm_ctx.cpp b/pacmann_amd/csrc/pm_ctx.cpp
--- a/pacmann_amd/csrc/pm_ctx.cpp
+++ b/pacmann_amd/csrc/pm_ctx.cpp
@@ -134,6 +134,11 @@
     pmk::set_fold_pack(value);
     return 0;
   }
+  if (!strcmp(name, "fold_bits")) {
+    if (value < -1 || value > 1) return fail(PM_EINVAL, "fold_bits takes 1, 0 or -1");
+    pmk::set_fold_bits(value);
+    return 0;
+  }
   if (!strcmp(name, "answer_pack")) {
     if (value < -1 || value > 1) return fail(PM_EINVAL, "answer_pack takes 1, 0 or -1");
     pmk::set_answer_pack(value);
diff --git a/pacmann_amd/csrc/pm_engine.cpp b/pacmann_amd/csrc/pm_engine.cpp
--- a/pacmann_amd/csrc/pm_engine.cpp
+++ b/pacmann_amd/csrc/pm_engine.cpp
@@ -134,19 +134,24 @@
   const uint32_t want_npk = !server && fold_img ? pmk::fold_pack_slices(g->minCS, g->maxCS, (uint32_t)g->E, coord_words) : 0;
   const uint32_t want_apk = !server && !remote && !g->owned_list.empty() ? pmk::answer_pack_segs((uint32_t)g->E, coord_words) : 0;
   bool low_zero = false;
+  uint32_t row_bits = 0;
   if (want_npk || want_apk) {
     DevBuf flag;
     CHK(flag.reserve(64));
-    low_zero = pmk::coord_low_zero(ctx->stream, g->db->as<uint64_t>(), off_db, (uint32_t)g->E, coord_words, flag.as<uint32_t>());
+    row_bits = pmk::row_bits_or(ctx->stream, g->db->as<uint64_t>(), off_db, (uint32_t)g->E, coord_words, flag.as<uint32_t>());
+    low_zero = !(row_bits & pmk::kRowLowHalf);
     HIPCHK(hipGetLastError());
   }
   if (fold_img) {
-    if (server) g->img_npk = server->img_npk;
-    else if (low_zero) g->img_npk = want_npk;
+    if (server) { g->img_npk = server->img_npk; g->img_bits = server->img_bits; }
+    else if (low_zero) {
+      g->img_bits = pmk::fold_bits_form((uint32_t)g->E, coord_words, want_npk, row_bits);
+      g->img_npk = g->img_bits ? 0 : want_npk;
+    }
     for (uint32_t i : g->owned_list) {
       PmPart& d = g->parts[i].d;
       d.img = (const uint64_t*)(uintptr_t)off_img;
-      off_img += pmk::fold_image_words(d.SS, (uint32_t)g->E, (uint32_t)g->maxCS, g->img_npk);
+      off_img += pmk::fold_image_words(d.SS, (uint32_t)g->E, (uint32_t)g->maxCS, g->img_npk, g->img_bits);
     }
     size_t free_b = 0, total_b = 0;
     if (!server && hipMemGetInfo(&free_b, &total_b) == hipSuccess && off_img * 8 > free_b / 4) {
@@ -156,7 +161,7 @@
       for (uint32_t i : g->owned_list) g->parts[i].d.img = nullptr;
       off_img = 0;
     }
-    if (!off_img) g->img_npk = 0;
+    if (!off_img) g->img_npk = g->img_bits = 0;
   }
   if (off_img) {
     if (server) {
@@ -166,7 +171,7 @@
       for (uint32_t i : g->owned_list) {
         const PmPart& d = g->parts[i].d;
         pmk::fold_image(ctx->stream, g->img->as<uint64_t>() + (uintptr_t)d.img, g->db->as<uint64_t>() + d.row0 * g->E,
-                        d.N, d.SS, (uint32_t)g->E, (uint32_t)g->maxCS, g->img_npk);
+                        d.N, d.SS, (uint32_t)g->E, (uint32_t)g->maxCS, g->img_npk, g->img_bits);
       }
       HIPCHK(hipGetLastError());
       HIPCHK(hipStreamSynchronize(ctx->stream));
@@ -347,9 +352,11 @@
     int kind = pmk::FOLD_GATHER;
     c->timed("prep_fold", fold, [&] { kind = pmk::prep_fold(st, dp, np, g->maxH, g->db->as<uint64_t>(), (uint32_t)g->E, g->minCS,
                                                       g->maxCS, g->zero16.as<uint64_t>(), clients, g->img->p != nullptr, minH,
-                                                      g->img_npk); });
-    if (kind == pmk::FOLD_ROT512 || kind == pmk::FOLD_ROT512P || kind == pmk::FOLD_ROT1024) {
-      c->host_add(kind == pmk::FOLD_ROT512 ? HT_FOLD_ROT512 : kind == pmk::FOLD_ROT512P ? HT_FOLD_ROT512P : HT_FOLD_ROT1024, 0.0);
+                                                      g->img_npk, g->img_bits); });
+    if (kind == pmk::FOLD_ROT512 || kind == pmk::FOLD_ROT512P || kind == pmk::FOLD_ROT512Q || kind == pmk::FOLD_ROT1024) {
+      c->host_add(kind == pmk::FOLD_ROT512 ? HT_FOLD_ROT512 : kind == pmk::FOLD_ROT512P ? HT_FOLD_ROT512P
+                  : kind == pmk::FOLD_ROT512Q ? HT_FOLD_ROT512Q : HT_FOLD_ROT1024,
+                  kind == pmk::FOLD_ROT512Q ? (double)pmk::fold_bits_slices(g->img_bits, (uint32_t)g->E) : 0.0);
     } else {
       c->host_add(HT_FOLD_OTHER, 0.0);
       c->host_add(kind == pmk::FOLD_PIPE ? HT_FOLD_PIPE : kind == pmk::FOLD_BLK ? HT_FOLD_BLK : HT_FOLD_GATHER, 0.0);
diff --git a/pacmann_amd/csrc/pm_engine.h b/pacmann_amd/csrc/pm_engine.h
--- a/pacmann_amd/csrc/pm_engine.h
+++ b/pacmann_amd/csrc/pm_engine.h
@@ -188,6 +188,7 @@
   std::shared_ptr<DevBuf> db = std::make_shared<DevBuf>();
   std::shared_ptr<DevBuf> img = std::make_shared<DevBuf>();
   uint32_t img_npk = 0;
+  uint32_t img_bits = 0;
   std::shared_ptr<DevBuf> apk = std::make_shared<DevBuf>();
   uint32_t apk_nseg = 0, apk_cseg = 0;
   void step_db(PmStep& S) const {
diff --git a/pacmann_amd/csrc/pm_host.h b/pacmann_amd/csrc/pm_host.h
--- a/pacmann_amd/csrc/pm_host.h
+++ b/pacmann_amd/csrc/pm_host.h
@@ -81,8 +81,8 @@
   template <class T> T* as() const { return (T*)p; }
 };
 
-enum HostTimer : int { HT_STEP_LAUNCH, HT_STEP_WAIT, HT_STEP_POST, HT_BATCH_QUERY, HT_GVI_PARSE, HT_SEARCH_KNN, HT_KNN_INIT, HT_KNN_BATCH, HT_KNN_UPDATE, HT_KNN_FINAL, HT_WAIT_FIRST, HT_WAIT_ALL, HT_ROWS_SEEN, HT_ROWS_TORN, HT_WAIT_DONE, HT_COMBINE, HT_COMBINE_TURN, HT_PATH_MATCH, HT_PATH_MATCH_PART, HT_PATH_MATCH_PART8, HT_PREP_SETS, HT_REC_VERIFIED, HT_REC_BAD, HT_REC_DROPPED, HT_REC_FAILED, HT_REC_PEER, HT_REC_UNEXPLAINED, HT_FOLD_ROT512, HT_FOLD_ROT1024, HT_FOLD_OTHER, HT_FOLD_PIPE, HT_FOLD_BLK, HT_FOLD_GATHER, HT_FOLD_ROT512P, HT_DEV_STEPS, HT_DEV_QUERIES, HT_KNN_BATCH_FALLBACK, HT_PATH_STEP, HT_PATH_RESOLVE_LDS, HT_PATH_RESOLVE_G, HT_PATH_MR_S2, HT_PATH_MR_S4, HT_PATH_MR_GENERAL, HT_PATH_GATHER, HT_PATH_ANSWER_P5, HT_PATH_ANSWER_P, HT_PATH_ANSWER_S, HT_PATH_ANSWER_G, HT_ANSWER_PACKED, HT_GVI_GROUP, HT_GVI_GROUP_STEPS, HT_SERVER_ANSWER_PACKED, HT_CLIENT_BEGIN, HT_CLIENT_FINISH, HT_PREP_STREAM, HT_PREP_STREAM_WINDOWS, HT_COUNT };
-static const char* const kHostTimerName[HT_COUNT] = {"host_step_launch", "host_step_wait", "host_step_post", "host_batch_query", "host_gvi_parse", "host_search_knn", "host_knn_init", "host_knn_batch", "host_knn_update", "host_knn_final", "host_wait_first_token", "host_wait_all_tokens", "host_rows_seen", "host_rows_torn", "host_wait_done", "host_combine", "host_combine_turn", "host_path_match", "host_path_match_part", "host_path_match_part8", "host_prep_sets", "host_records_verified", "host_records_bad", "host_records_dropped", "host_records_failed", "host_records_peer", "host_records_unexplained", "host_fold_rot512", "host_fold_rot1024", "host_fold_other", "host_fold_pipe", "host_fold_blk", "host_fold_gather", "host_fold_rot512p", "host_dev_steps", "host_dev_queries", "host_knn_batch_fallback", "host_path_step", "host_path_resolve_lds", "host_path_resolve_g", "host_path_mr_s2", "host_path_mr_s4", "host_path_mr_general", "host_path_gather", "host_path_answer_p5", "host_path_answer_p", "host_path_answer_s", "host_path_answer_g", "host_answer_packed", "host_gvi_group", "host_gvi_group_steps", "host_server_answer_packed", "host_client_begin", "host_client_finish", "host_prep_stream", "host_prep_stream_windows"};
+enum HostTimer : int { HT_STEP_LAUNCH, HT_STEP_WAIT, HT_STEP_POST, HT_BATCH_QUERY, HT_GVI_PARSE, HT_SEARCH_KNN, HT_KNN_INIT, HT_KNN_BATCH, HT_KNN_UPDATE, HT_KNN_FINAL, HT_WAIT_FIRST, HT_WAIT_ALL, HT_ROWS_SEEN, HT_ROWS_TORN, HT_WAIT_DONE, HT_COMBINE, HT_COMBINE_TURN, HT_PATH_MATCH, HT_PATH_MATCH_PART, HT_PATH_MATCH_PART8, HT_PREP_SETS, HT_REC_VERIFIED, HT_REC_BAD, HT_REC_DROPPED, HT_REC_FAILED, HT_REC_PEER, HT_REC_UNEXPLAINED, HT_FOLD_ROT512, HT_FOLD_ROT1024, HT_FOLD_OTHER, HT_FOLD_PIPE, HT_FOLD_BLK, HT_FOLD_GATHER, HT_FOLD_ROT512P, HT_FOLD_ROT512Q, HT_DEV_STEPS, HT_DEV_QUERIES, HT_KNN_BATCH_FALLBACK, HT_PATH_STEP, HT_PATH_RESOLVE_LDS, HT_PATH_RESOLVE_G, HT_PATH_MR_S2, HT_PATH_MR_S4, HT_PATH_MR_GENERAL, HT_PATH_GATHER, HT_PATH_ANSWER_P5, HT_PATH_ANSWER_P, HT_PATH_ANSWER_S, HT_PATH_ANSWER_G, HT_ANSWER_PACKED, HT_GVI_GROUP, HT_GVI_GROUP_STEPS, HT_SERVER_ANSWER_PACKED, HT_CLIENT_BEGIN, HT_CLIENT_FINISH, HT_PREP_STREAM, HT_PREP_STREAM_WINDOWS, HT_COUNT };
+static const char* const kHostTimerName[HT_COUNT] = {"host_step_launch", "host_step_wait", "host_step_post", "host_batch_query", "host_gvi_parse", "host_search_knn", "host_knn_init", "host_knn_batch", "host_knn_update", "host_knn_final", "host_wait_first_token", "host_wait_all_tokens", "host_rows_seen", "host_rows_torn", "host_wait_done", "host_combine", "host_combine_turn", "host_path_match", "host_path_match_part", "host_path_match_part8", "host_prep_sets", "host_records_verified", "host_records_bad", "host_records_dropped", "host_records_failed", "host_records_peer", "host_records_unexplained", "host_fold_rot512", "host_fold_rot1024", "host_fold_other", "host_fold_pipe", "host_fold_blk", "host_fold_gather", "host_fold_rot512p", "host_fold_rot512q", "host_dev_steps", "host_dev_queries", "host_knn_batch_fallback", "host_path_step", "host_path_resolve_lds", "host_path_resolve_g", "host_path_mr_s2", "host_path_mr_s4", "host_path_mr_general", "host_path_gather", "host_path_answer_p5", "host_path_answer_p", "host_path_answer_s", "host_path_answer_g", "host_answer_packed", "host_gvi_group", "host_gvi_group_steps", "host_server_answer_packed", "host_client_begin", "host_client_finish", "host_prep_stream", "host_prep_stream_windows"};
 static_assert(HT_PATH_ANSWER_G - HT_PATH_STEP + 1 == pmk::FORM_COUNT, "one counter per step form, in the order of pmk::FORM_*");
 
 struct TimedLaunch { std::string name; hipEvent_t a, b; double bytes; };
diff --git a/pacmann_amd/csrc/pm_internal.h b/pacmann_amd/csrc/pm_internal.h
--- a/pacmann_amd/csrc/pm_internal.h
+++ b/pacmann_amd/csrc/pm_internal.h
@@ -234,12 +234,12 @@
                uint32_t E, bool zero_state);
 void prep_offsets(hipStream_t st, const PmPart* dparts, int nparts, uint32_t maxH, uint32_t maxSS);
 void set_aes_bs(int v);
-enum : int { FOLD_GATHER = 0, FOLD_ROT512 = 1, FOLD_ROT1024 = 2, FOLD_PIPE = 3, FOLD_BLK = 4, FOLD_ROT512P = 5 };
-int fold_form(uint32_t minCS, uint32_t maxCS, uint32_t E, bool have_img, uint32_t npk = 0);
+enum : int { FOLD_GATHER = 0, FOLD_ROT512 = 1, FOLD_ROT1024 = 2, FOLD_PIPE = 3, FOLD_BLK = 4, FOLD_ROT512P = 5, FOLD_ROT512Q = 6 };
+int fold_form(uint32_t minCS, uint32_t maxCS, uint32_t E, bool have_img, uint32_t npk = 0, uint32_t qf = 0);
 void set_fold_rot(int v);
 int prep_fold(hipStream_t st, const PmPart* dparts, int nparts, uint32_t maxH, const uint64_t* db,
               uint32_t E, uint32_t minCS, uint32_t maxCS, const uint64_t* zero16, uint32_t clients = 1,
-              bool have_img = false, uint32_t minH = 0, uint32_t npk = 0);
+              bool have_img = false, uint32_t minH = 0, uint32_t npk = 0, uint32_t qf = 0);
 void prep_repl(hipStream_t st, const PmPart* dparts, int nparts, uint32_t maxRepl,
                const uint64_t* db, uint32_t E);
 void stream_fold(hipStream_t st, const PmPart* parts, uint32_t part, uint32_t H, const uint64_t* win, uint32_t c0,
@@ -248,13 +248,17 @@
                  uint32_t nc, uint32_t nrows, uint32_t E);
 bool fold_image_ok(uint32_t minCS, uint32_t maxCS, uint32_t E);
 bool fold_needs_tab(uint32_t minCS, uint32_t maxCS, uint32_t E, bool have_img);
-uint64_t fold_image_words(uint32_t SS, uint32_t E, uint32_t CS, uint32_t npk = 0);
+uint64_t fold_image_words(uint32_t SS, uint32_t E, uint32_t CS, uint32_t npk = 0, uint32_t qf = 0);
 void fold_image(hipStream_t st, uint64_t* img, const uint64_t* part_rows, uint64_t N, uint32_t SS, uint32_t E,
-                uint32_t CS, uint32_t npk = 0);
+                uint32_t CS, uint32_t npk = 0, uint32_t qf = 0);
+enum : uint32_t { kRowLowHalf = 1, kRowCoordBits = 2, kRowIdBits = 4 };
 void set_fold_pack(int v);
+void set_fold_bits(int v);
 uint32_t fold_pack_shape(uint32_t E, uint32_t dim);
 uint32_t fold_pack_slices(uint32_t minCS, uint32_t maxCS, uint32_t E, uint32_t dim);
-bool coord_low_zero(hipStream_t st, const uint64_t* rows, uint64_t nrows, uint32_t E, uint32_t dim, uint32_t* flag);
+uint32_t row_bits_or(hipStream_t st, const uint64_t* rows, uint64_t nrows, uint32_t E, uint32_t dim, uint32_t* flag);
+uint32_t fold_bits_form(uint32_t E, uint32_t dim, uint32_t npk, uint32_t flags);
+uint32_t fold_bits_slices(uint32_t qf, uint32_t E);
 void set_answer_pack(int v);
 uint32_t answer_pack_shape(uint32_t E, uint32_t dim);
 uint32_t answer_pack_segs(uint32_t E, uint32_t dim);
diff --git a/pacmann_amd/csrc/pm_kernels.hip b/pacmann_amd/csrc/pm_kernels.hip
--- a/pacmann_amd/csrc/pm_kernels.hip
+++ b/pacmann_amd/csrc/pm_kernels.hip
@@ -485,6 +485,80 @@
   }
 }
 
+struct FoldBits { uint32_t w1, n1, w2, n2; };
+struct FoldBitsSlice { uint32_t q1, c1, q2, c2; };
+__host__ __device__ inline FoldBits fold_bits_of(uint32_t qf, uint32_t E) {
+  FoldBits f;
+  f.w1 = qf & 0xffu; f.w2 = (qf >> 8) & 0xffu; f.n1 = qf >> 16;
+  f.n2 = (E & ~3u) / 2 - f.n1;
+  return f;
+}
+__host__ __device__ inline FoldBitsSlice fold_bits_slice(const FoldBits& f, uint32_t s) {
+  const uint32_t per1 = 64 / f.w1, per2 = 64 / f.w2, nf1 = f.n1 / per1, r1 = f.n1 % per1;
+  const uint32_t fit = r1 ? (64 - r1 * f.w1) / f.w2 : 0u, cm = fit < f.n2 ? fit : f.n2;
+  FoldBitsSlice o;
+  if (s < nf1) { o.q1 = s * per1; o.c1 = per1; o.q2 = 0; o.c2 = 0; return o; }
+  if (r1 && s == nf1) { o.q1 = nf1 * per1; o.c1 = r1; o.q2 = 0; o.c2 = cm; return o; }
+  o.q1 = f.n1; o.c1 = 0;
+  o.q2 = cm + (s - nf1 - (r1 ? 1 : 0)) * per2;
+  o.c2 = o.q2 >= f.n2 ? 0u : f.n2 - o.q2 < per2 ? f.n2 - o.q2 : per2;
+  return o;
+}
+__host__ __device__ inline uint32_t fold_bits_nsl(const FoldBits& f) {
+  const uint32_t per1 = 64 / f.w1, per2 = 64 / f.w2, nf1 = f.n1 / per1, r1 = f.n1 % per1;
+  const uint32_t fit = r1 ? (64 - r1 * f.w1) / f.w2 : 0u, cm = fit < f.n2 ? fit : f.n2;
+  return nf1 + (r1 ? 1 : 0) + (f.n2 - cm + per2 - 1) / per2;
+}
+template <int W> __host__ __device__ __forceinline__ uint32_t fold_field_pack(uint32_t x) {
+  if constexpr (W == 12) return ((x >> 16) & 0x7ffu) | ((x >> 19) & 0x800u);
+  else if constexpr (W == 16) return x >> 16;
+  else if constexpr (W == 20) return x & 0xfffffu;
+  else return x;
+}
+template <int W> __host__ __device__ __forceinline__ uint32_t fold_field_expand(uint32_t f) {
+  if constexpr (W == 12) return ((f & 0x7ffu) | ((f & 0x400u) * 14u) | ((f & 0x800u) << 3)) << 16;
+  else if constexpr (W == 16) return f << 16;
+  else return f;
+}
+template <int W> __device__ __forceinline__ uint32_t fold_bits_get(const uint32_t (&d)[8], int p) {
+  const int i = p >> 5, sh = p & 31;
+  uint32_t v = d[i] >> sh;
+  if (sh + W > 32) v |= d[i + 1] << (32 - sh);
+  if constexpr (W < 32) v &= (1u << W) - 1u;
+  return v;
+}
+template <int W> __device__ __forceinline__ void fold_bits_put(uint32_t (&d)[8], int p, uint32_t f) {
+  const int i = p >> 5, sh = p & 31;
+  d[i] |= f << sh;
+  if (sh + W > 32) d[i + 1] |= f >> (32 - sh);
+}
+__host__ __device__ constexpr int fold_bits_pos1(int w1, int i, int t) { return (4 * i + t) * w1; }
+__host__ __device__ constexpr int fold_bits_pos2(int w2, int i, int t) { return 256 - 4 * w2 * (i + 1) + t * w2; }
+template <int W1, int W2>
+__device__ __forceinline__ void fold_bits_store(const uint32_t (&d)[8], const FoldBitsSlice& sl, uint32_t n1,
+                                                PM_G uint32_t* par) {
+  typedef uint32_t u32x4 __attribute__((ext_vector_type(4)));
+#pragma unroll
+  for (int i = 0; i < 64 / W1; ++i) {
+    if ((uint32_t)i >= sl.c1) break;
+    u32x4 x;
+#pragma unroll
+    for (int t = 0; t < 4; ++t) x[t] = fold_field_expand<W1>(fold_bits_get<W1>(d, fold_bits_pos1(W1, i, t)));
+    PM_G u32x4* const dst = reinterpret_cast<PM_G u32x4*>(par + (sl.q1 + i) * 4);
+    if (PM_PREP_NT) __builtin_nontemporal_store(x, dst);
+    else *dst = x;
+  }
+#pragma unroll
+  for (int i = 0; i < 64 / W2; ++i) {
+    if ((uint32_t)i >= sl.c2) break;
+    u32x4 x;
+#pragma unroll
+    for (int t = 0; t < 4; ++t) x[t] = fold_field_expand<W2>(fold_bits_get<W2>(d, fold_bits_pos2(W2, i, t)));
+    PM_G u32x4* const dst = reinterpret_cast<PM_G u32x4*>(par + (n1 + sl.q2 + i) * 4);
+    if (PM_PREP_NT) __builtin_nontemporal_store(x, dst);
+    else *dst = x;
+  }
+}
 #ifndef PM_ROT_HPL
 #define PM_ROT_HPL 5
 #endif
@@ -493,6 +567,12 @@
 #endif
 #ifndef PM_ROT_SB
 #define PM_ROT_SB 8
+#endif
+#ifndef PM_ROTQ_GB
+#define PM_ROTQ_GB 4
+#endif
+#ifndef PM_ROTQ_SB
+#define PM_ROTQ_SB 9
 #endif
 #ifndef PM_ROT_HPL2
 #define PM_ROT_HPL2 7
@@ -504,7 +584,8 @@
 template <int CS>
 __global__ void __launch_bounds__(kFoldThreads) k_prep_fold_rot(const PmPart* __restrict__ parts, uint32_t E,
                                                                 uint32_t nvg, uint32_t nsl, uint32_t npv,
-                                                                uint32_t npk_arg, uint32_t K, uint32_t ngc) {
+                                                                uint32_t npk_arg, uint32_t K, uint32_t ngc,
+                                                                uint32_t qf_arg, uint32_t GB, uint32_t SB) {
   constexpr uint32_t NCH = rot_nch(CS), LINE = NCH * 8, BUFW = (CS + 1) * LINE;
   constexpr int HPL = rot_hpl(CS);
   static_assert(CS == 512 || CS == 1024, "4 chunks of 512 rows or 2 of 1,024 per block");
@@ -515,8 +596,8 @@
   constexpr uint32_t G = ITEMS / kFoldThreads;
   constexpr uint32_t HB = kFoldThreads * HPL;
   const uint32_t npk = CS == 512 ? npk_arg : 0u;
+  const uint32_t qf = CS == 512 ? qf_arg : 0u;
   const uint32_t xcd = blockIdx.x % 8, kq = blockIdx.x / 8;
-  constexpr uint32_t GB = PM_ROT_GB, SB = PM_ROT_SB;
   const uint32_t nsb = (nsl + SB - 1) / SB, ngb = (npv + GB - 1) / GB;
   const uint32_t T = (kq / (GB * SB)) * 8 + xcd, wt = kq % (GB * SB);
   if (T >= ngb * nsb) return;
@@ -633,7 +714,20 @@
     const bool inB = v >= vb;
     PM_G uint64_t* const par = (inB ? PB.parity : PA.parity) + (uint64_t)(v - (inB ? vb : hA)) * E;
     PM_G uint32_t* dst = reinterpret_cast<PM_G uint32_t*>(par + w);
-    if (slice < npk) {
+    if (qf) {
+      uint32_t d[8];
+#pragma unroll
+      for (int t = 0; t < 4; ++t) {
+        d[t] = j ? acc[k][4 + t] : acc[k][t];
+        d[4 + t] = j ? acc[k][t] : acc[k][4 + t];
+      }
+      const FoldBits fb = fold_bits_of(qf, E);
+      const FoldBitsSlice sl = fold_bits_slice(fb, slice);
+      PM_G uint32_t* const p32 = reinterpret_cast<PM_G uint32_t*>(par);
+      if (fb.w1 == 12 && fb.w2 == 20) fold_bits_store<12, 20>(d, sl, fb.n1, p32);
+      else if (fb.w1 == 16) fold_bits_store<16, 20>(d, sl, fb.n1, p32);
+      else fold_bits_store<12, 32>(d, sl, fb.n1, p32);
+    } else if (slice < npk) {
       typedef uint32_t u32x4 __attribute__((ext_vector_type(4)));
 #pragma unroll
       for (int t = 0; t < 8; t += 2) {
@@ -650,7 +744,7 @@
         else *d = acc[k][t];
       }
     }
-    if (w == 0)
+    if (slice == 0)
       for (uint32_t t = E & ~3u; t < E; ++t) par[t] = 0;
   }
 }
@@ -682,6 +776,46 @@
       }
     }
     img[x] = v;
+  }
+}
+template <int W1, int W2>
+__device__ __forceinline__ void fold_bits_pack(const uint32_t* __restrict__ row, const FoldBitsSlice& sl, uint32_t n1,
+                                               uint32_t (&d)[8]) {
+#pragma unroll
+  for (int i = 0; i < 64 / W1; ++i) {
+    if ((uint32_t)i >= sl.c1) break;
+    const uint4 v = *reinterpret_cast<const uint4*>(row + (sl.q1 + i) * 4);
+    const uint32_t x[4] = {v.x, v.y, v.z, v.w};
+#pragma unroll
+    for (int t = 0; t < 4; ++t) fold_bits_put<W1>(d, fold_bits_pos1(W1, i, t), fold_field_pack<W1>(x[t]));
+  }
+#pragma unroll
+  for (int i = 0; i < 64 / W2; ++i) {
+    if ((uint32_t)i >= sl.c2) break;
+    const uint4 v = *reinterpret_cast<const uint4*>(row + (n1 + sl.q2 + i) * 4);
+    const uint32_t x[4] = {v.x, v.y, v.z, v.w};
+#pragma unroll
+    for (int t = 0; t < 4; ++t) fold_bits_put<W2>(d, fold_bits_pos2(W2, i, t), fold_field_pack<W2>(x[t]));
+  }
+}
+__global__ void __launch_bounds__(kBlock) k_fold_image_bits(uint4* __restrict__ img, const uint64_t* __restrict__ rows,
+                                                           uint64_t N, uint32_t nbuf, uint32_t E, uint64_t nitems,
+                                                           uint32_t qf) {
+  const FoldBits fb = fold_bits_of(qf, E);
+  for (uint64_t x = (uint64_t)blockIdx.x * kBlock + threadIdx.x; x < nitems; x += (uint64_t)gridDim.x * kBlock) {
+    const uint32_t it = (uint32_t)(x % (kRotBufBytes / 16));
+    const uint64_t blk = x / (kRotBufBytes / 16);
+    const uint32_t b = (uint32_t)(blk % nbuf), s = (uint32_t)(blk / nbuf);
+    const uint64_t r = (uint64_t)(4 * b + ((it >> 1) & 3)) * 512 + (it >> 3);
+    uint32_t d[8] = {0, 0, 0, 0, 0, 0, 0, 0};
+    if (r < N) {
+      const uint32_t* const row = reinterpret_cast<const uint32_t*>(rows + r * E);
+      const FoldBitsSlice sl = fold_bits_slice(fb, s);
+      if (fb.w1 == 12 && fb.w2 == 20) fold_bits_pack<12, 20>(row, sl, fb.n1, d);
+      else if (fb.w1 == 16) fold_bits_pack<16, 20>(row, sl, fb.n1, d);
+      else fold_bits_pack<12, 32>(row, sl, fb.n1, d);
+    }
+    img[x] = (it & 1) ? make_uint4(d[4], d[5], d[6], d[7]) : make_uint4(d[0], d[1], d[2], d[3]);
   }
 }
 __global__ void __launch_bounds__(kBlock) k_answer_pack_image(uint4* __restrict__ img, const uint64_t* __restrict__ rows,
@@ -702,17 +836,28 @@
     img[x] = v;
   }
 }
-__global__ void __launch_bounds__(kBlock) k_coord_low_or(const uint64_t* __restrict__ rows, uint64_t nrows, uint32_t E,
-                                                        uint32_t dim, uint32_t* __restrict__ out) {
-  const uint32_t per = dim / 4;
+__device__ inline uint32_t coord_bits_or(uint32_t x) {
+  const uint32_t e6 = x >> 29;
+  return (x >> 31) | ((((e6 ^ (x >> 28)) | (e6 ^ (x >> 27)) | (e6 ^ (x >> 26))) & 1u));
+}
+__global__ void __launch_bounds__(kBlock) k_row_bits_or(const uint64_t* __restrict__ rows, uint64_t nrows, uint32_t E,
+                                                       uint32_t dim, uint32_t* __restrict__ out) {
+  const uint32_t per = E / 2;
   const uint64_t nitems = nrows * per;
-  uint32_t acc = 0;
+  uint32_t low = 0, cb = 0, ib = 0;
   for (uint64_t x = (uint64_t)blockIdx.x * kBlock + threadIdx.x; x < nitems; x += (uint64_t)gridDim.x * kBlock) {
     const uint64_t r = x / per;
-    const uint4 v = reinterpret_cast<const uint4*>(rows + r * E)[x - r * per];
-    acc |= v.x | v.y | v.z | v.w;
-  }
-  if (acc & 0xffffu) atomicOr(out, 1u);
+    const uint32_t i = (uint32_t)(x - r * per);
+    const uint4 v = reinterpret_cast<const uint4*>(rows + r * E)[i];
+    if (4 * i < dim) {
+      low |= v.x | v.y | v.z | v.w;
+      cb |= coord_bits_or(v.x) | coord_bits_or(v.y) | coord_bits_or(v.z) | coord_bits_or(v.w);
+    } else {
+      ib |= v.x | v.y | v.z | v.w;
+    }
+  }
+  const uint32_t f = ((low & 0xffffu) ? pmk::kRowLowHalf : 0u) | (cb ? pmk::kRowCoordBits : 0u) | ((ib >> 20) ? pmk::kRowIdBits : 0u);
+  if (f) atomicOr(out, f);
 }
 
 constexpr uint32_t kReplRows = 32, kReplIt = (kReplRows * 1024 / 16 + kBlock - 1) / kBlock;
@@ -1064,10 +1209,10 @@
   while (sw > 2 && !fits(sw)) sw /= 2;
   return fits(sw) ? sw : 0;
 }
-int fold_form(uint32_t minCS, uint32_t maxCS, uint32_t E, bool have_img, uint32_t npk) {
+int fold_form(uint32_t minCS, uint32_t maxCS, uint32_t E, bool have_img, uint32_t npk, uint32_t qf) {
   if ((E & ~3u) == 0) return FOLD_GATHER;
   if (have_img && fold_rot_shape(minCS, maxCS, E))
-    return maxCS == 512 ? (npk ? FOLD_ROT512P : FOLD_ROT512) : FOLD_ROT1024;
+    return maxCS == 512 ? (qf ? FOLD_ROT512Q : npk ? FOLD_ROT512P : FOLD_ROT512) : FOLD_ROT1024;
   if (minCS == maxCS && (maxCS == 512 || maxCS == 1024 || maxCS == 2048) && E % 2 == 0) return FOLD_PIPE;
   if (E % 2 || !fold_blk_sw(maxCS)) return FOLD_GATHER;
   return FOLD_BLK;
@@ -1078,12 +1223,33 @@
 }
 static std::atomic<int> g_fold_pack{-1};
 void set_fold_pack(int v) { g_fold_pack.store(v < 0 ? -1 : (v ? 1 : 0)); }
+static std::atomic<int> g_fold_bits{-1};
+void set_fold_bits(int v) { g_fold_bits.store(v < 0 ? -1 : (v ? 1 : 0)); }
+static int fold_pack_level() {
+  static const bool env = [] { const char* e = getenv("PM_FOLD_PACK"); return !e || e[0] != '0'; }();
+  static const bool envb = [] { const char* e = getenv("PM_FOLD_BITS"); return !e || e[0] != '0'; }();
+  const int v = g_fold_pack.load(), b = g_fold_bits.load();
+  if (!(v < 0 ? env : v == 1)) return 0;
+  return (b < 0 ? envb : b == 1) ? 2 : 1;
+}
 uint32_t fold_pack_slices(uint32_t minCS, uint32_t maxCS, uint32_t E, uint32_t dim) {
-  static const bool env = [] { const char* e = getenv("PM_FOLD_PACK"); return !e || e[0] != '0'; }();
-  const int v = g_fold_pack.load();
-  if (!(v < 0 ? env : v == 1) || fold_form(minCS, maxCS, E, true) != FOLD_ROT512) return 0;
+  if (fold_pack_level() < 1 || fold_form(minCS, maxCS, E, true) != FOLD_ROT512) return 0;
   return fold_pack_shape(E, dim);
 }
+uint32_t fold_bits_form(uint32_t E, uint32_t dim, uint32_t npk, uint32_t flags) {
+  if (fold_pack_level() < 2 || !npk || (flags & kRowLowHalf)) return 0;
+  const bool cq = !(flags & kRowCoordBits), iq = !(flags & kRowIdBits);
+  uint32_t best = 0, best_nsl = (E & ~3u) / 4 - npk;
+  auto offer = [&](uint32_t w1, uint32_t w2) {
+    const uint32_t qf = w1 | (w2 << 8) | ((dim / 4) << 16), nsl = fold_bits_nsl(fold_bits_of(qf, E));
+    if (nsl < best_nsl) { best = qf; best_nsl = nsl; }
+  };
+  if (iq) offer(16, 20);
+  if (cq) offer(12, 32);
+  if (cq && iq) offer(12, 20);
+  return best;
+}
+uint32_t fold_bits_slices(uint32_t qf, uint32_t E) { return qf ? fold_bits_nsl(fold_bits_of(qf, E)) : 0; }
 uint32_t fold_pack_shape(uint32_t E, uint32_t dim) {
   return dim && dim % 16 == 0 && dim / 8 <= E / 4 ? dim / 16 : 0;
 }
@@ -1106,26 +1272,31 @@
   if (grid > 256 * 32) grid = 256 * 32;
   if (grid) hipLaunchKernelGGL(k_answer_pack_image, dim3(grid), dim3(kBlock), 0, st, (uint4*)img, rows, nitems, E, nseg, dim / 8);
 }
-bool coord_low_zero(hipStream_t st, const uint64_t* rows, uint64_t nrows, uint32_t E, uint32_t dim, uint32_t* flag) {
-  if (hipMemsetAsync(flag, 0, 4, st) != hipSuccess) return false;
-  unsigned grid = cdiv(nrows * (dim / 4), kBlock);
+uint32_t row_bits_or(hipStream_t st, const uint64_t* rows, uint64_t nrows, uint32_t E, uint32_t dim, uint32_t* flag) {
+  const uint32_t all = kRowLowHalf | kRowCoordBits | kRowIdBits;
+  if (hipMemsetAsync(flag, 0, 4, st) != hipSuccess) return all;
+  unsigned grid = cdiv(nrows * (E / 2), kBlock);
   if (grid > 256 * 32) grid = 256 * 32;
-  if (grid) hipLaunchKernelGGL(k_coord_low_or, dim3(grid), dim3(kBlock), 0, st, rows, nrows, E, dim, flag);
-  uint32_t h = 1;
+  if (grid) hipLaunchKernelGGL(k_row_bits_or, dim3(grid), dim3(kBlock), 0, st, rows, nrows, E, dim, flag);
+  uint32_t h = all;
   if (hipMemcpyAsync(&h, flag, 4, hipMemcpyDeviceToHost, st) != hipSuccess || hipStreamSynchronize(st) != hipSuccess)
-    return false;
-  return h == 0;
-}
-uint64_t fold_image_words(uint32_t SS, uint32_t E, uint32_t CS, uint32_t npk) {
-  return (uint64_t)(E / 4 - npk) * (SS / rot_nch(CS)) * (kRotBufBytes / 8);
+    return all;
+  return h;
+}
+uint64_t fold_image_words(uint32_t SS, uint32_t E, uint32_t CS, uint32_t npk, uint32_t qf) {
+  const uint32_t nsl = qf ? fold_bits_slices(qf, E) : E / 4 - npk;
+  return (uint64_t)nsl * (SS / rot_nch(CS)) * (kRotBufBytes / 8);
 }
 void fold_image(hipStream_t st, uint64_t* img, const uint64_t* rows, uint64_t N, uint32_t SS, uint32_t E, uint32_t CS,
-                uint32_t npk) {
-  const uint64_t nitems = fold_image_words(SS, E, CS, npk) / 2;
+                uint32_t npk, uint32_t qf) {
+  const uint64_t nitems = fold_image_words(SS, E, CS, npk, qf) / 2;
   unsigned grid = cdiv(nitems, kBlock);
   if (grid > 256 * 32) grid = 256 * 32;
-  hipLaunchKernelGGL(k_fold_image, dim3(grid), dim3(kBlock), 0, st, (uint4*)img, rows, N, SS / rot_nch(CS), E, nitems,
-                     CS, npk);
+  if (qf)
+    hipLaunchKernelGGL(k_fold_image_bits, dim3(grid), dim3(kBlock), 0, st, (uint4*)img, rows, N, SS / rot_nch(CS), E, nitems, qf);
+  else
+    hipLaunchKernelGGL(k_fold_image, dim3(grid), dim3(kBlock), 0, st, (uint4*)img, rows, N, SS / rot_nch(CS), E, nitems,
+                       CS, npk);
 }
 void fold_image_map(uint32_t CS, uint32_t SS, uint32_t npk, uint64_t x0, uint64_t n, uint64_t* row, uint32_t* word,
                     uint8_t* packed) {
@@ -1136,8 +1307,8 @@
 }
 int prep_fold(hipStream_t st, const PmPart* d, int np, uint32_t maxH, const uint64_t* db, uint32_t E,
               uint32_t minCS, uint32_t maxCS, const uint64_t* zero16, uint32_t clients, bool have_img,
-               uint32_t minH, uint32_t npk) {
-  const int form = fold_form(minCS, maxCS, E, have_img, npk);
+               uint32_t minH, uint32_t npk, uint32_t qf) {
+  const int form = fold_form(minCS, maxCS, E, have_img, npk, qf);
   const uint32_t EX = E & ~3u;
   if (EX == 0) {
     hipLaunchKernelGGL(k_prep_fold<2>, dim3(cdiv((uint64_t)maxH * E, kBlock), np), dim3(kBlock), 0,
@@ -1153,8 +1324,9 @@
     else if (sw == 4) hipLaunchKernelGGL(k_prep_fold_blk<4>, grid, blk, lds, st, d, db, zero16, E, w0);
     else hipLaunchKernelGGL(k_prep_fold_blk<2>, grid, blk, lds, st, d, db, zero16, E, w0);
   };
-  if (form == FOLD_ROT512 || form == FOLD_ROT512P || form == FOLD_ROT1024 || form == FOLD_PIPE) {
-    const uint32_t psw = maxCS == 2048 ? 2 : 4, nsl = EX / psw - (form == FOLD_ROT512P ? npk : 0);
+  if (form == FOLD_ROT512 || form == FOLD_ROT512P || form == FOLD_ROT512Q || form == FOLD_ROT1024 || form == FOLD_PIPE) {
+    const uint32_t psw = maxCS == 2048 ? 2 : 4;
+    const uint32_t nsl = form == FOLD_ROT512Q ? fold_bits_slices(qf, E) : EX / psw - (form == FOLD_ROT512P ? npk : 0);
     const uint32_t K = clients && np % clients == 0 ? clients : 1, npg = (np / K) * ng;
     const uint32_t lw = 16 / psw, per_pg = K * cdiv(nsl, lw) * lw;
 #ifndef PM_FOLD_NB512
@@ -1167,12 +1339,14 @@
       const uint64_t HB = (uint64_t)kFoldThreads * rot_hpl(maxCS);
       const uint32_t ngc = minH >= HB ? 0u : (uint32_t)cdiv(maxH, HB);
       const uint32_t nvg = ngc ? K * ngc : (uint32_t)cdiv((uint64_t)K * maxH, HB), npv = (np / K) * nvg;
-      const uint32_t grid = 8 * cdiv((uint64_t)cdiv(npv, PM_ROT_GB) * cdiv(nsl, PM_ROT_SB), 8) * PM_ROT_GB * PM_ROT_SB;
+      const uint32_t GB = form == FOLD_ROT512Q ? PM_ROTQ_GB : PM_ROT_GB, SB = form == FOLD_ROT512Q ? PM_ROTQ_SB : PM_ROT_SB;
+      const uint32_t grid = 8 * cdiv((uint64_t)cdiv(npv, GB) * cdiv(nsl, SB), 8) * GB * SB;
       if (form != FOLD_ROT1024)
         hipLaunchKernelGGL(k_prep_fold_rot<512>, dim3(grid), dim3(kFoldThreads), 0, st, d, E, nvg, nsl, npv,
-                           form == FOLD_ROT512P ? npk : 0u, K, ngc);
+                           form == FOLD_ROT512P ? npk : 0u, K, ngc, form == FOLD_ROT512Q ? qf : 0u, GB, SB);
       else
-        hipLaunchKernelGGL(k_prep_fold_rot<1024>, dim3(grid), dim3(kFoldThreads), 0, st, d, E, nvg, nsl, npv, 0u, K, ngc);
+        hipLaunchKernelGGL(k_prep_fold_rot<1024>, dim3(grid), dim3(kFoldThreads), 0, st, d, E, nvg, nsl, npv, 0u, K, ngc,
+                           0u, GB, SB);
       return form;
     }
     const uint32_t nb = maxCS == 512 ? PM_FOLD_NB512 : 3;
```
